# tanderson92/Fast_solver_Lippmann_Schwinger

Measured on AMD Instinct MI355X. Metric: fastconv applies/sec, 3D n=512^3 fp64 (FastM3D apply), higher is better.
Workload: dtype f64; 1 GPU; 3D n=512^3 complex fp64 operator apply y = x + w^2 G*(nu.*x), Greengard-Vico truncated-kernel symbol, omega=1/h=512, sum-of-8-Gaussians contrast, vectors resident in HBM; n=512, pipeline=pruned-hip, parallelism=single GPU

## Files before the change

fast_solver_lippmann_schwinger_amd/_lib.py:

```python
from __future__ import annotations

import ctypes as C
import os

_HERE = os.path.dirname(os.path.abspath(__file__))
LIB_PATH = os.environ.get("LSFC_LIBRARY") or os.path.join(_HERE, "liblsfc.so")

LSFC_QUAD_TRAPEZOIDAL, LSFC_QUAD_GREENGARD_VICO = 0, 1
LSFC_MEM_HOST, LSFC_MEM_DEVICE = 0, 1
LSFC_PRECOND_INV_F64, LSFC_PRECOND_INV_F32 = 0, 1
LSFC_PRECOND_PIVOT_NONE, LSFC_PRECOND_PIVOT_PARTIAL, LSFC_PRECOND_PIVOT_AUTO = 0, 1, 2
LSFC_FLAG_DEFAULT, LSFC_FLAG_LITERAL_PAD, LSFC_FLAG_FORCE_ROCFFT, LSFC_FLAG_PATCH_SINGULAR = 0, 1, 2, 4
LSFC_ORTH_MGS, LSFC_ORTH_CGS, LSFC_ORTH_DGKS = 0, 1, 2
LSFC_EINVAL, LSFC_ENODEV, LSFC_ENOMEM, LSFC_ENOTCONV = -1, -2, -3, -5
LSFC_UNIQUE_ID_BYTES = 128

PRECOND_FN = C.CFUNCTYPE(C.c_int, C.c_void_p, C.POINTER(C.c_double), C.c_int64)


class GmresOpts(C.Structure):
    _fields_ = [("restart", C.c_int), ("maxiter", C.c_int64), ("reltol", C.c_double), ("abstol", C.c_double),
                ("orth", C.c_int), ("initially_zero", C.c_int), ("precond", PRECOND_FN), ("precond_user", C.c_void_p),
                ("precond_on_device", C.c_int)]


class GmresResult(C.Structure):
    _fields_ = [("iters", C.c_int64), ("mvps", C.c_int64), ("converged", C.c_int), ("final_resnorm", C.c_double)]


class BicgstablOpts(C.Structure):
    _fields_ = [("l", C.c_int), ("max_mv_products", C.c_int64), ("reltol", C.c_double), ("abstol", C.c_double),
                ("initially_zero", C.c_int), ("precond", PRECOND_FN), ("precond_user", C.c_void_p),
                ("precond_on_device", C.c_int), ("r_shadow", C.c_void_p), ("reserved", C.c_int * 4)]


class BlocktriOpts(C.Structure):
    _fields_ = [("inverse_precision", C.c_int), ("pivoting", C.c_int), ("reserved", C.c_int * 6)]


class LsfcError(RuntimeError):
    def __init__(self, code, msg):
        super().__init__(f"lsfc error {code}: {msg}")
        self.code = code


_P, _I, _L, _D, _U = C.c_void_p, C.c_int, C.c_int64, C.c_double, C.c_uint
_PP = C.POINTER(C.c_void_p)
SIGNATURES = {
    "lsfc_plan_create_2d": (_I, [_PP, _L, _L, _L, _L, _P, _P, _D, _I, _U, _I]),
    "lsfc_plan_create_3d": (_I, [_PP, _L, _L, _L, _L, _L, _L, _P, _P, _D, _I, _U, _I]),
    "lsfc_plan_create_gv2d": (_I, [_PP, _L, _L, _D, _D, _P, _U, _I]),
    "lsfc_plan_create_trap2d": (_I, [_PP, _L, _L, _D, _D, _D, _D, _D, _D, _P, _U, _I]),
    "lsfc_plan_create_gv3d": (_I, [_PP, _L, _L, _L, _D, _D, _P, _U, _I]),
    "lsfc_plan_destroy": (_I, [_P]),
    "lsfc_plan_size": (_L, [_P]),
    "lsfc_plan_dims": (_I, [_P, C.POINTER(_L), C.POINTER(_L)]),
    "lsfc_plan_pipeline": (C.c_char_p, [_P]),
    "lsfc_plan_set_nu": (_I, [_P, _P, _I]),
    "lsfc_plan_get_symbol": (_I, [_P, _P, _L, C.POINTER(_L)]),
    "lsfc_apply": (_I, [_P, _P, _P, _I]),
    "lsfc_convolve": (_I, [_P, _P, _P, _I, _I]),
    "lsfc_apply_batch": (_I, [_P, _P, _P, _L, _I, _I]),
    "lsfc_sample_sources": (_I, [_P, _P, _L, _P, _I]),
    "lsfc_gmres": (_I, [_P, _P, _P, C.POINTER(GmresOpts), _P, _L, C.POINTER(GmresResult), _I]),
    "lsfc_gmres_batch": (_I, [_P, _P, _P, _L, C.POINTER(GmresOpts), _P, _L, C.POINTER(GmresResult), _I]),
    "lsfc_bicgstabl": (_I, [_P, _P, _P, C.POINTER(BicgstablOpts), _P, _L, C.POINTER(GmresResult), _I]),
    "lsfc_precond_create": (_I, [_PP, _L, _P, _P, _P, _P, _P, _P, _P, _P, _P, _P, _P, _P, _I]),
    "lsfc_precond_destroy": (_I, [_P]),
    "lsfc_precond_set_stream": (_I, [_P, _P]),
    "lsfc_precond_apply": (_I, [_P, _P, _I]),
    "lsfc_precond_apply_batch": (_I, [_P, _P, _L, _I]),
    "lsfc_precond_batch_info": (_I, [_P, C.POINTER(_L)]),
    "lsfc_precond_callback": (_I, [_P, _P, _L]),
    "lsfc_precond_stats": (_I, [_P, C.POINTER(_L), C.POINTER(_L), C.POINTER(_L)]),
    "lsfc_precond_schedule": (_I, [_P, _I, C.POINTER(_L)]),
    "lsfc_precond_create_blocktri": (_I, [_PP, _L, _L, _P, _P, _P, _P, _I, _I]),
    "lsfc_precond_create_from_plan": (_I, [_PP, _P]),
    "lsfc_precond_create_blocktri_prec": (_I, [_PP, _L, _L, _P, _P, _P, _P, _I, _I, _I]),
    "lsfc_precond_create_from_plan_prec": (_I, [_PP, _P, _I]),
    "lsfc_precond_create_blocktri_opts": (_I, [_PP, _L, _L, _P, _P, _P, _P, _I, _I, _P]),
    "lsfc_precond_create_from_plan_opts": (_I, [_PP, _P, _P]),
    "lsfc_precond_blocktri_get_pivots": (_I, [_P, _L, _P, _L]),
    "lsfc_precond_inverse_precision": (_I, [_P, C.POINTER(_I)]),
    "lsfc_precond_blocktri_info": (_I, [_P, C.POINTER(_L), C.POINTER(_D)]),
    "lsfc_precond_blocktri_get_block": (_I, [_P, _L, _P, _L]),
    "lsfc_sparsify_pattern": (_I, [_L, _L, _L, C.POINTER(_L), _P, _P, _P]),
    "lsfc_sparsify_build": (_I, [_P, _P, _P, _P, _P, _P, _P, _I]),
    "lsfc_plan_set_stream": (_I, [_P, _P]),
    "lsfc_plan_synchronize": (_I, [_P]),
    "lsfc_plan_set_tuning": (_I, [_P, C.c_char_p, _I]),
    "lsfc_time_apply": (_I, [_P, _P, _P, _I, C.POINTER(_D)]),
    "lsfc_profile_apply": (_I, [_P, _P, _P, _I, _I, C.POINTER(C.c_char_p), C.POINTER(_D), C.POINTER(_D), C.POINTER(_I)]),
    "lsfc_device_count": (_I, [C.POINTER(_I)]),
    "lsfc_malloc": (_I, [_PP, C.c_size_t, _I]),
    "lsfc_free": (_I, [_P]),
    "lsfc_memcpy_h2d": (_I, [_P, _P, C.c_size_t]),
    "lsfc_memcpy_d2h": (_I, [_P, _P, C.c_size_t]),
    "lsfc_host_register": (_I, [_P, C.c_size_t]),
    "lsfc_host_unregister": (_I, [_P]),
    "lsfc_host_alloc": (_I, [_PP, C.c_size_t]),
    "lsfc_host_free": (_I, [_P]),
    "lsfc_dist_unique_id": (_I, [_P]),
    "lsfc_dist_plan_create_gv3d": (_I, [_PP, _L, _L, _L, _D, _D, _P, _U, _I, _I, _I, _P]),
    "lsfc_dist_sim_plan_create_gv3d": (_I, [_PP, _L, _L, _L, _D, _D, _P, _U, _I, _I, _I]),
    "lsfc_dist_sim_apply": (_I, [_PP, _I, _PP, _PP, _I]),
    "lsfc_plan_create_gv3d_multi": (_I, [_PP, _L, _L, _L, _D, _D, _P, _U, C.POINTER(_I), _I]),
    "lsfc_multi_info": (_I, [_P, C.POINTER(_I), C.POINTER(_I), C.POINTER(_L), C.POINTER(C.c_char_p)]),
    "lsfc_multi_apply_dev": (_I, [_P, _PP, _PP, _I]),
    "lsfc_last_error": (C.c_char_p, []),
    "lsfc_padded_length": (_I, [C.c_int64]),
    "lsfc_version": (C.c_char_p, []),
}

_lib = None


def load():
    global _lib
    if _lib is None:
        if not os.path.exists(LIB_PATH):
            raise ImportError(f"{LIB_PATH} is missing: build it with `make -C {os.path.join(_HERE, 'csrc')}` "
                              "(hipcc --offload-arch=gfx950); there is no CPU fallback for the lsfc operator")
        try:
            import torch
        except ImportError:
            pass
        lib = C.CDLL(LIB_PATH)
        for name, (res, args) in SIGNATURES.items():
            fn = getattr(lib, name)
            fn.restype, fn.argtypes = res, args
        _lib = lib
    return _lib


def check(rc):
    if rc != 0:
        raise LsfcError(rc, load().lsfc_last_error().decode(errors="replace"))
    return rc


def host_register(a):
    check(load().lsfc_host_register(a.ctypes.data_as(C.c_void_p), a.nbytes))


def host_unregister(a):
    check(load().lsfc_host_unregister(a.ctypes.data_as(C.c_void_p)))


class _PinnedBlock:

    def __init__(self, nbytes):
        self.ptr = C.c_void_p()
        check(load().lsfc_host_alloc(C.byref(self.ptr), max(int(nbytes), 1)))
        self.nbytes = int(nbytes)

    def __del__(self):
        try:
            if self.ptr:
                load().lsfc_host_free(self.ptr)
                self.ptr = C.c_void_p()
        except Exception:
            pass


def host_empty(shape, dtype="complex128"):
    import numpy as np
    dt = np.dtype(dtype)
    count = int(np.prod(shape)) if np.ndim(shape) else int(shape)
    blk = _PinnedBlock(count * dt.itemsize)
    buf = (C.c_char * max(blk.nbytes, 1)).from_address(blk.ptr.value)
    buf._owner = blk
    return np.frombuffer(buf, dtype=dt, count=count).reshape(shape)


def device_count():
    n = C.c_int(0)
    load().lsfc_device_count(C.byref(n))
    return n.value
```

fast_solver_lippmann_schwinger_amd/csrc/fft_kernels.hip:

```cpp
#include "common.hpp"
#include "fft_configs.hpp"
#include "pruned.hpp"
#include <cstdlib>
#include <mutex>
#include <set>
#include <map>
#include <utility>

#ifndef LSFC_FAMILY
#error "compile with -DLSFC_FAMILY=2, 3 or 5"
#endif
#define LSFC_CAT2(a, b) a##b
#define LSFC_CAT(a, b) LSFC_CAT2(a, b)
#define FAM(name) LSFC_CAT(LSFC_CAT(name, _f), LSFC_FAMILY)

namespace lsfc {
using namespace fft;

static constexpr int XB = 8;

template <class C, int LPW, bool SPLIT, bool EXACT>
__global__ __launch_bounds__(C::T * LPW)
void k_xfwd(const VecBatch vb, int64_t obatch, const double* __restrict__ nu, cplx* __restrict__ out,
            const cplx* __restrict__ tw, int64_t nlines, int wmagic, int W, int Wp, int n, int64_t bstride) {
    const cplx* __restrict__ x = vb.x[blockIdx.y];
    out += (int64_t)blockIdx.y * obatch;
    using LL = LdsLayout<1, 3, SPLIT>;
    extern __shared__ __attribute__((aligned(16))) char smem[];
    constexpr int T = C::T, E = C::E;
    const int t = threadIdx.x % T, ll = threadIdx.x / T;
    const int64_t line = (int64_t)blockIdx.x * LPW + ll;
    const bool valid = line < nlines;
    const int64_t lc = valid ? line : nlines - 1;
    const cplx* xin = x + lc * n;
    cplx v[E];
#pragma unroll
    for (int e = 0; e < E / 2; ++e) v[e] = (EXACT || t + T * e < n) ? xin[t + T * e] : make_double2(0.0, 0.0);
    if (nu) {
        const double* nin = nu + lc * n;
#pragma unroll
        for (int e = 0; e < E / 2; ++e) { const double s = (EXACT || t + T * e < n) ? nin[t + T * e] : 0.0; v[e].x *= s; v[e].y *= s; }
    }
#pragma unroll
    for (int e = E / 2; e < E; ++e) v[e] = make_double2(0.0, 0.0);
    fft_forward<C, LL, true>(v, t, tw, smem, ll * LL::line_elems(C::L), 0);
    if (valid) {
#pragma unroll
        for (int e = 0; e < E; ++e) {
            const int s = t + T * e;
            const int c = (int)(((unsigned)s * (unsigned)wmagic) >> 22);
            out[(int64_t)c * bstride + line * Wp + (s - c * W)] = v[e];
        }
    }
}

template <class C, int LPW, bool SPLIT, bool EXACT>
__global__ __launch_bounds__(C::T * LPW)
void k_xinv(const cplx* __restrict__ in, const VecBatch vb, int64_t ibatch, double alpha, double beta,
            const cplx* __restrict__ tw, int64_t nlines, int wmagic, int W, int Wp, int n, int64_t bstride) {
    const cplx* xorig = vb.x[blockIdx.y];
    cplx* y = vb.y[blockIdx.y];
    in += (int64_t)blockIdx.y * ibatch;
    using LL = LdsLayout<1, 3, SPLIT>;
    extern __shared__ __attribute__((aligned(16))) char smem[];
    constexpr int T = C::T, E = C::E;
    const int t = threadIdx.x % T, ll = threadIdx.x / T;
    const int64_t line = (int64_t)blockIdx.x * LPW + ll;
    const bool valid = line < nlines;
    const int64_t lc = valid ? line : nlines - 1;
    cplx v[E];
#pragma unroll
    for (int e = 0; e < E; ++e) {
        const int s = t + T * e;
        const int c = (int)(((unsigned)s * (unsigned)wmagic) >> 22);
        v[e] = in[(int64_t)c * bstride + lc * Wp + (s - c * W)];
    }
    fft_inverse<C, LL, true>(v, t, tw, smem, ll * LL::line_elems(C::L), 0);
    if (valid) {
#pragma unroll
        for (int e = 0; e < E / 2; ++e) {
            if (EXACT || t + T * e < n) {
                const int64_t idx = line * n + t + T * e;
                cplx r = make_double2(beta * v[e].x, beta * v[e].y);
                if (alpha != 0.0) { const cplx xo = xorig[idx]; r.x = fma(alpha, xo.x, r.x); r.y = fma(alpha, xo.y, r.y); }
                y[idx] = r;
            }
        }
    }
}

template <class C, int LINES, bool SPLIT, int WPE, bool EXACT>
__global__ __launch_bounds__(C::T * LINES, WPE)
void k_yfwd(const cplx* __restrict__ a1, cplx* __restrict__ a2, const cplx* __restrict__ tw, int Lx, int m, int l, int TG, int TZ, int p1, int p2,
            int64_t batch1, int64_t batch2) {
    using LL = LdsLayout<LINES, 3, SPLIT>;
    a1 += (int64_t)blockIdx.y * batch1; a2 += (int64_t)blockIdx.y * batch2;
    extern __shared__ __attribute__((aligned(16))) char smem[];
    constexpr int T = C::T, E = C::E, Ly = C::L;
    const int xi = threadIdx.x % LINES, t = threadIdx.x / LINES;
    const int ngrp = Lx / LINES;
    const int within = blockIdx.x % (TG * TZ), tile = blockIdx.x / (TG * TZ);
    const int ntg = ngrp / TG;
    const int g = (tile % ntg) * TG + within % TG, z = (tile / ntg) * TZ + within / TG;
    const int xp = g * LINES + xi;
    const cplx* src = a1 + xp + (int64_t)p1 * m * z;
    cplx v[E];
#pragma unroll
    for (int e = 0; e < E / 2; ++e) v[e] = (EXACT || t + T * e < m) ? src[(int64_t)p1 * (t + T * e)] : make_double2(0.0, 0.0);
#pragma unroll
    for (int e = E / 2; e < E; ++e) v[e] = make_double2(0.0, 0.0);
    fft_forward<C, LL, true, false, (C::T * LINES > 512)>(v, t, tw, smem, 0, xi);
    const int xb = xp / XB, xq = xp % XB;
    cplx* dst = a2 + xq + (int64_t)XB * z + (int64_t)p2 * ((int64_t)Ly * xb);
#pragma unroll
    for (int e = 0; e < E; ++e) dst[(int64_t)p2 * (t + T * e)] = v[e];
}

template <class C, int LINES, bool SPLIT, int WPE, bool EXACT>
__global__ __launch_bounds__(C::T * LINES, WPE)
void k_yinv(const cplx* __restrict__ a2, cplx* __restrict__ a1, const cplx* __restrict__ tw, int Lx, int m, int l, int TG, int TZ, int p1, int p2,
            int64_t batch1, int64_t batch2) {
    using LL = LdsLayout<LINES, 3, SPLIT>;
    a1 += (int64_t)blockIdx.y * batch1; a2 += (int64_t)blockIdx.y * batch2;
    extern __shared__ __attribute__((aligned(16))) char smem[];
    constexpr int T = C::T, E = C::E, Ly = C::L;
    const int xi = threadIdx.x % LINES, t = threadIdx.x / LINES;
    const int ngrp = Lx / LINES;
    const int within = blockIdx.x % (TG * TZ), tile = blockIdx.x / (TG * TZ);
    const int ntg = ngrp / TG;
    const int g = (tile % ntg) * TG + within % TG, z = (tile / ntg) * TZ + within / TG;
    const int xp = g * LINES + xi;
    const int xb = xp / XB, xq = xp % XB;
    const cplx* src = a2 + xq + (int64_t)XB * z + (int64_t)p2 * ((int64_t)Ly * xb);
    cplx v[E];
#pragma unroll
    for (int e = 0; e < E; ++e) v[e] = src[(int64_t)p2 * (t + T * e)];
    fft_inverse<C, LL, true, false, (C::T * LINES > 512)>(v, t, tw, smem, 0, xi);
    cplx* dst = a1 + xp + (int64_t)p1 * m * z;
#pragma unroll
    for (int e = 0; e < E / 2; ++e) if (EXACT || t + T * e < m) dst[(int64_t)p1 * (t + T * e)] = v[e];
}

template <class C, int LINES, bool SPLIT, bool PREFETCH, int WPE, bool HALF, bool ZE, bool EXACT, bool TWL, bool MULTI = false>
__global__ __launch_bounds__(C::T * LINES, WPE)
void k_zfused(cplx* __restrict__ data, const cplx* __restrict__ sym, const cplx* __restrict__ tw,
              int nouter, int64_t dGrp, int64_t dOuter, int64_t dLine, int64_t sGrp, int64_t sOuter, int64_t sLine,
              const int2* __restrict__ ytab, const int* __restrict__ zm, int nin, int nrhs, int64_t dBatch, int sibling_pairs) {
    using LL = LdsLayout<LINES, 3, SPLIT>;
    extern __shared__ __attribute__((aligned(16))) char smem[];
    constexpr int T = C::T, E = C::E;
    int xi = threadIdx.x % LINES; const int t = threadIdx.x / LINES;
    unsigned tile = blockIdx.x;
    if constexpr (HALF) {
        constexpr int PARTS = XB / LINES, SH = PARTS == 4 ? 5 : 4;
        const unsigned b = blockIdx.x;
        tile = (b >> SH) * 8 + (b & 7);
        xi += (int)((b >> 3) & (PARTS - 1)) * LINES;
    } else if (sibling_pairs) {
        const unsigned b = blockIdx.x;
        tile = (((b >> 4) * 8 + (b & 7)) << 1) | ((b >> 3) & 1);
    }
    const int o = tile % nouter, g = tile / nouter;
    int outer = o, srow = o;
    if (ytab) { const int2 e = ytab[o]; outer = e.x; srow = e.y; }
    cplx* d = data + g * dGrp + outer * dOuter + xi;
    const cplx* s = sym + g * sGrp + srow * sOuter + xi;
    const int li = threadIdx.x % LINES;
    if constexpr (TWL) {
        cplx* tl = reinterpret_cast<cplx*>(smem + (size_t)LL::line_elems(C::L) * LINES * LL::elem_bytes());
        for (int i = threadIdx.x; i < C::TWLEN; i += C::T * LINES) tl[i] = tw[i];
        __syncthreads();
        tw = tl;
    }
#ifdef LSFC_NO_XLANE_ONE_TILE
    constexpr bool XL1 = false;
#else
    constexpr bool XL1 = !SPLIT && xlane_ok<C, LL>() && (C::T * LINES) % 64 == 0;
#endif
    auto fwd = [&](cplx (&w)[E]) {
        if constexpr (!SPLIT) fft_forward_ws<C, LL, true, TWL, false, XL1>(w, t, tw, smem, 0, li, [] {});
        else fft_forward<C, LL, true, TWL>(w, t, tw, smem, 0, li);
    };
    auto inv = [&](cplx (&w)[E]) {
        if constexpr (!SPLIT) fft_inverse_ws<C, LL, true, TWL, false, XL1>(w, t, tw, smem, 0, li);
        else fft_inverse<C, LL, true, TWL>(w, t, tw, smem, 0, li);
    };
    cplx v[E];
    if constexpr (MULTI) {
        constexpr int H = ZE ? E / 2 : E;
        cplx sv[H];
#pragma unroll
        for (int e = 0; e < H; ++e) sv[e] = s[sLine * (t + T * e)];
        int part[ZE ? H : 1];
        cplx smid = make_double2(0.0, 0.0);
        if constexpr (ZE) {
#pragma unroll
            for (int e = 0; e < H; ++e) part[e] = zm[t + T * e];
            if (t == 0) smid = s[sLine * (C::L / 2)];
        }
        for (int r = 0; r < nrhs; ++r) {
            cplx* dr = d + (int64_t)r * dBatch;
#pragma unroll
            for (int e = 0; e < E / 2; ++e) v[e] = (EXACT || t + T * e < nin) ? dr[dLine * (t + T * e)] : make_double2(0.0, 0.0);
#pragma unroll
            for (int e = E / 2; e < E; ++e) v[e] = make_double2(0.0, 0.0);
            fwd(v);
            if constexpr (ZE) {
                cplx* stage = reinterpret_cast<cplx*>(smem);
                if constexpr (forward_ends_local<C, LL>()) LSFC_BARRIER();
#pragma unroll
                for (int e = 0; e < H; ++e) stage[(t + T * e) * LINES + li] = sv[e];
                if (t == 0) stage[(C::L / 2) * LINES + li] = smid;
                LSFC_BARRIER();
#pragma unroll
                for (int e = 0; e < H; ++e) {
                    v[e] = cmul(v[e], sv[e]);
                    v[e + H] = cmul(v[e + H], stage[part[e] * LINES + li]);
                }
                LSFC_BARRIER();
            } else {
#pragma unroll
                for (int e = 0; e < E; ++e) v[e] = cmul(v[e], sv[e]);
            }
            inv(v);
#pragma unroll
            for (int e = 0; e < E / 2; ++e) if (EXACT || t + T * e < nin) dr[dLine * (t + T * e)] = v[e];
        }
        return;
    }
#pragma unroll
    for (int e = 0; e < E / 2; ++e) v[e] = (EXACT || t + T * e < nin) ? d[dLine * (t + T * e)] : make_double2(0.0, 0.0);
#pragma unroll
    for (int e = E / 2; e < E; ++e) v[e] = make_double2(0.0, 0.0);
    if constexpr (ZE) {
        constexpr int H = E / 2;
        int part[H];
#pragma unroll
        for (int e = 0; e < H; ++e) part[e] = zm[t + T * e];
        cplx sv[H];
        if constexpr (PREFETCH) {
#pragma unroll
            for (int e = 0; e < H; ++e) sv[e] = s[sLine * (t + T * e)];
        }
        fwd(v);
        if constexpr (!PREFETCH) {
#pragma unroll
            for (int e = 0; e < H; ++e) sv[e] = s[sLine * (t + T * e)];
        }
        cplx* stage = reinterpret_cast<cplx*>(smem);
        if constexpr (forward_ends_local<C, LL>()) LSFC_BARRIER();
#pragma unroll
        for (int e = 0; e < H; ++e) stage[(t + T * e) * LINES + li] = sv[e];
        if (t == 0) stage[(C::L / 2) * LINES + li] = s[sLine * (C::L / 2)];
        LSFC_BARRIER();
#pragma unroll
        for (int e = 0; e < H; ++e) {
            v[e] = cmul(v[e], sv[e]);
            v[e + H] = cmul(v[e + H], stage[part[e] * LINES + li]);
        }
        LSFC_BARRIER();
    } else if constexpr (PREFETCH) {
        cplx sv[E];
#pragma unroll
        for (int e = 0; e < E; ++e) sv[e] = s[sLine * (t + T * e)];
        fwd(v);
#pragma unroll
        for (int e = 0; e < E; ++e) v[e] = cmul(v[e], sv[e]);
    } else {
        fwd(v);
#pragma unroll
        for (int e = 0; e < E; ++e) v[e] = cmul(v[e], s[sLine * (t + T * e)]);
    }
    inv(v);
#pragma unroll
    for (int e = 0; e < E / 2; ++e) if (EXACT || t + T * e < nin) d[dLine * (t + T * e)] = v[e];
}

__device__ __forceinline__ unsigned xcc_id() {
    unsigned v;
    asm volatile("s_getreg_b32 %0, hwreg(HW_REG_XCC_ID, 0, 4)" : "=s"(v));
    return v & 7u;
}
template <class V> __device__ __forceinline__ V launder_v(V x) { asm volatile("" : "+v"(x)); return x; }
template <class P> __device__ __forceinline__ P launder_s(P x) { asm volatile("" : "+s"(x)); return x; }

template <class C, int LINES, bool SPLIT, bool HALF> constexpr size_t persist_xbuf_bytes() {
    using LL = LdsLayout<LINES, HALF ? -1 : 3, SPLIT>;
    constexpr size_t ex = (size_t)LL::line_elems(C::L) * LINES * LL::elem_bytes(), stg = (size_t)(C::L / 2 + 1) * LINES * sizeof(cplx);
    return ex > stg ? ex : stg;
}
template <class C, int LINES, bool SPLIT, bool TWL, bool HALF> constexpr size_t persist_lds_bytes() {
    return persist_xbuf_bytes<C, LINES, SPLIT, HALF>() + (TWL ? (size_t)C::TWLEN * sizeof(cplx) : 0);
}
template <class C, int LINES, bool SPLIT, bool EXACT, bool TWL, bool LATE_SYM = false, bool HALF = false, bool TICKETS = HALF, int XL = 0>
__global__ __launch_bounds__(C::T * LINES, (HALF && 2 * persist_lds_bytes<C, LINES, SPLIT, TWL, HALF>() <= (size_t)160 * 1024) ? 2 : 1)
void k_zfused_persist(cplx* __restrict__ data, const cplx* __restrict__ sym, const cplx* __restrict__ tw,
                      int nouter, int64_t dGrp, int64_t dOuter, int64_t dLine, int64_t sGrp, int64_t sOuter, int64_t sLine,
                      const int2* __restrict__ ytab, const int* __restrict__ zm, int nin, unsigned ntiles, unsigned* __restrict__ tickets) {
    using LL = LdsLayout<LINES, HALF ? -1 : 3, SPLIT>;
    extern __shared__ __attribute__((aligned(16))) char smem[];
    constexpr int T = C::T, E = C::E, H = E / 2;
#ifdef LSFC_NO_STAGE_STORES
    constexpr bool WS = false;
#else
    constexpr bool WS = true;
#endif
#ifdef LSFC_DEFERRED_BARRIERS
    constexpr bool DEFER = true;
#else
    constexpr bool DEFER = false;
#endif
    const int li = threadIdx.x % LINES, t = threadIdx.x / LINES;
    constexpr bool PAIR = (XL & 4) != 0 && TICKETS && !HALF;
    constexpr unsigned DONE = 0xFFFFFFFFu;
    unsigned cur = blockIdx.x, nwork = ntiles;
    unsigned* slot = nullptr;
    unsigned queue = 0, queues_left = 8;
    [[maybe_unused]] unsigned parity = 1u;
    auto draw = [&]() -> unsigned {
        while (queues_left > 0) {
            const unsigned c = atomicAdd(tickets + queue, 1u);
            if (c < nwork) return (c << 3) | queue;
            queue = (queue + 1) & 7u; --queues_left;
        }
        return DONE;
    };
    if constexpr (TICKETS) {
        queue = xcc_id();
        nwork = HALF ? ntiles / 4 : (PAIR ? ntiles / 16 : ntiles / 8);
        slot = reinterpret_cast<unsigned*>(smem + persist_lds_bytes<C, LINES, SPLIT, TWL, HALF>());
        if (threadIdx.x == 0) *slot = draw();
        __syncthreads();
        cur = __builtin_amdgcn_readfirstlane(*slot);
        __syncthreads();
        if (cur == DONE) return;
    } else if (cur >= nwork) return;
    if constexpr (TWL) {
        cplx* tl = reinterpret_cast<cplx*>(smem + persist_xbuf_bytes<C, LINES, SPLIT, HALF>());
        for (int i = threadIdx.x; i < C::TWLEN; i += C::T * LINES) tl[i] = tw[i];
        __syncthreads();
        tw = tl;
    }
    auto locate = [&](unsigned w, cplx*& dbase, const cplx*& sbase, unsigned sub = 0) {
        unsigned tl_ = w; int half = 0;
        if constexpr (PAIR) tl_ = ticket_decode_pair(w, sub);
        else if constexpr (TICKETS) { unsigned hf; ticket_decode<HALF>(w, tl_, hf); half = (int)hf * LINES; }
        const int o = (int)(tl_ % (unsigned)nouter), g = (int)(tl_ / (unsigned)nouter);
        int outer = o, srow = o;
        if (ytab) { const int2 e2 = ytab[o]; outer = e2.x; srow = e2.y; }
        dbase = data + g * dGrp + outer * dOuter + half;
        sbase = sym + g * sGrp + srow * sOuter + half;
    };
    const unsigned doff = (unsigned)(li + (int)dLine * t), dstep = (unsigned)((int)dLine * T);
    const unsigned soff = (unsigned)(li + (int)sLine * t), sstep = (unsigned)((int)sLine * T);
    constexpr bool MIRG = (XL & 2) != 0;
    [[maybe_unused]] unsigned moff[MIRG ? H : 1];
    if constexpr (MIRG) {
#pragma unroll
        for (int e = 0; e < H; ++e) moff[e] = (unsigned)(li + (int)sLine * zm[t + T * e]);
    }
    cplx nd[H];
    {
        cplx* d; const cplx* s;
        locate(cur, d, s);
#pragma unroll
        for (int e = 0; e < H; ++e) nd[e] = (EXACT || t + T * e < nin) ? d[doff + dstep * e] : make_double2(0.0, 0.0);
    }
    [[maybe_unused]] unsigned sub = 0;
    [[maybe_unused]] const cplx* sheld = nullptr;
    [[maybe_unused]] cplx sv_pair[PAIR ? H : 1];
    [[maybe_unused]] cplx smid_pair = make_double2(0.0, 0.0);
    for (;;) {
        unsigned drawn = 0;
        if constexpr (TICKETS) { if (threadIdx.x == 0 && (!PAIR || sub == 0)) drawn = draw(); }
        cplx v[E];
#pragma unroll
        for (int e = 0; e < H; ++e) { v[e] = nd[e]; v[e + H] = make_double2(0.0, 0.0); }
        cplx sv_tile[PAIR ? 1 : H];
        cplx (&sv)[H] = *reinterpret_cast<cplx (*)[H]>(PAIR ? &sv_pair[0] : &sv_tile[0]);
        [[maybe_unused]] cplx smr[MIRG ? H : 1];
        cplx smid_tile = make_double2(0.0, 0.0);
        cplx& smid = PAIR ? smid_pair : smid_tile;
        auto load_symbol = [&] {
            cplx* d; const cplx* s;
            locate(cur, d, s, sub);
            if constexpr (PAIR) {
                if (s == sheld) return;
                sheld = s;
            }
            const unsigned so = launder_v(soff);
#pragma unroll
            for (int e = 0; e < H; ++e) sv[e] = s[so + sstep * e];
            if constexpr (MIRG) {
#pragma unroll
                for (int e = 0; e < H; ++e) smr[e] = s[moff[e]];
            } else {
                if (t == 0) smid = s[so - (unsigned)((int)sLine * t) + (unsigned)((int)sLine * (C::L / 2))];
            }
        };
        if constexpr (!SPLIT && WS) {
            if constexpr (!LATE_SYM) load_symbol();
            fft_forward_ws<C, LL, true, TWL, DEFER, (XL > 0)>(v, t, tw, smem, 0, li, [&] { if constexpr (LATE_SYM) load_symbol(); });
        } else if constexpr (LATE_SYM) {
            stage<C, 0, +1, 1, TWL>(v, t, tw);
            load_symbol();
            exchange<C, 0, 1, LL>(v, t, smem, 0, li);
            stage<C, 1, +1, 0, TWL>(v, t, tw);
            if constexpr (C::NS >= 3) { exchange<C, 1, 2, LL>(v, t, smem, 0, li); stage<C, 2, +1, 0, TWL>(v, t, tw); }
            if constexpr (C::NS >= 4) { exchange<C, 2, 3, LL>(v, t, smem, 0, li); stage<C, 3, +1, 0, TWL>(v, t, tw); }
        } else {
            load_symbol();
            fft_forward<C, LL, true, TWL>(v, t, tw, smem, 0, li);
        }
        cplx* stage = reinterpret_cast<cplx*>(smem);
        unsigned next = cur + gridDim.x;
        if constexpr (MIRG) {
#pragma unroll
            for (int e = 0; e < H; ++e) { v[e] = cmul(v[e], sv[e]); v[e + H] = cmul(v[e + H], smr[e]); }
            if constexpr (TICKETS) {
                if (threadIdx.x == 0) slot[parity] = drawn;
                LSFC_BARRIER();
                next = __builtin_amdgcn_readfirstlane(slot[parity]);
                parity ^= 1u;
            }
        } else {
        if constexpr (forward_ends_local<C, LL>() || (!SPLIT && WS && DEFER)) LSFC_BARRIER();
#pragma unroll
        for (int e = 0; e < H; ++e) stage[(t + T * e) * LINES + li] = sv[e];
        if (t == 0) stage[(C::L / 2) * LINES + li] = smid;
        if constexpr (TICKETS) { if (threadIdx.x == 0 && (!PAIR || sub == 0)) *slot = drawn; }
        LSFC_BARRIER();
        {
            const int* zmt = launder_s(zm) + t;
#pragma unroll
            for (int e = 0; e < H; ++e) {
                v[e] = cmul(v[e], sv[e]);
                v[e + H] = cmul(v[e + H], stage[zmt[T * e] * LINES + li]);
            }
        }
        if constexpr (TICKETS) next = __builtin_amdgcn_readfirstlane(*slot);
        LSFC_BARRIER();
        }
        const bool more = PAIR ? (sub == 0 || next != DONE) : (TICKETS ? next != DONE : next < nwork);
        if (more) {
            cplx* dn; const cplx* sn;
            if (PAIR && sub == 0) locate(cur, dn, sn, 1u); else locate(next, dn, sn, 0u);
            const unsigned dof = launder_v(doff);
#pragma unroll
            for (int e = 0; e < H; ++e) nd[e] = (EXACT || t + T * e < nin) ? dn[dof + dstep * e] : make_double2(0.0, 0.0);
        }
        if constexpr (!SPLIT && WS) fft_inverse_ws<C, LL, true, TWL, DEFER, (XL > 0)>(v, t, tw, smem, 0, li);
        else fft_inverse<C, LL, true, TWL>(v, t, tw, smem, 0, li);
        {
            cplx* d; const cplx* s;
            locate(cur, d, s, sub);
            const unsigned dof = launder_v(doff);
#pragma unroll
            for (int e = 0; e < H; ++e) if (EXACT || t + T * e < nin) d[dof + dstep * e] = v[e];
        }
        if (!more) break;
        if constexpr (PAIR) { if (sub == 0) sub = 1; else { sub = 0; cur = next; } }
        else cur = next;
    }
}

template <class K> static void allow_lds(K kernel, size_t bytes) {
    if (bytes <= 48 * 1024) return;
    static std::mutex mu;
    static std::set<std::pair<const void*, int>> done;
    int dev = 0; LSFC_HIP(hipGetDevice(&dev));
    const std::pair<const void*, int> key(reinterpret_cast<const void*>(kernel), dev);
    std::lock_guard<std::mutex> lock(mu);
    if (done.count(key)) return;
    LSFC_HIP(hipFuncSetAttribute(key.first, hipFuncAttributeMaxDynamicSharedMemorySize, (int)bytes));
    done.insert(key);
}

static bool env_flag_no_sibling_pairs() { static const bool v = getenv("LSFC_NO_SIBLING_PAIRS") != nullptr; return v; }
static bool env_flag_z_quarter() { static const bool v = [] { const char* e = getenv("LSFC_Z_QUARTER"); return e && e[0] == '1'; }(); return v; }

template <class C> struct Tune {
    static constexpr int LPW = (256 / C::T) > 0 ? (256 / C::T) : 1;
    static constexpr int LINES = (C::T * XB <= 512 || (C::E <= 8 && C::T * XB <= 1024)) ? XB : 512 / C::T;
#ifdef LSFC_Y2048_HALF
    static constexpr int YLINES = LINES;
#else
    static constexpr int YLINES = (C::L == 2048 && C::T * XB <= 1024) ? XB : LINES;
#endif
};

template <class C, bool SPLIT> static void xfwd_t(const VecBatch& vb, int nrhs, int64_t obatch, const double* nu, cplx* out, const cplx* tw, int64_t nlines, int wmagic, int W, int Wp, int n, int64_t bstride, hipStream_t st) {
    constexpr int LPW = Tune<C>::LPW;
    using LL = LdsLayout<1, 3, SPLIT>;
    const size_t lds = (size_t)LL::line_elems(C::L) * LPW * LL::elem_bytes();
    auto k = (n == C::L / 2) ? k_xfwd<C, LPW, SPLIT, true> : k_xfwd<C, LPW, SPLIT, false>;
    allow_lds(k, lds);
    hipLaunchKernelGGL(k, dim3((unsigned)((nlines + LPW - 1) / LPW), (unsigned)nrhs), dim3(C::T * LPW), lds, st, vb, obatch, nu, out, tw, nlines, wmagic, W, Wp, n, bstride);
}
template <class C, bool SPLIT> static void xinv_t(const cplx* in, const VecBatch& vb, int nrhs, int64_t ibatch, double alpha, double beta, const cplx* tw, int64_t nlines, int wmagic, int W, int Wp, int n, int64_t bstride, hipStream_t st) {
    constexpr int LPW = Tune<C>::LPW;
    using LL = LdsLayout<1, 3, SPLIT>;
    const size_t lds = (size_t)LL::line_elems(C::L) * LPW * LL::elem_bytes();
    auto k = (n == C::L / 2) ? k_xinv<C, LPW, SPLIT, true> : k_xinv<C, LPW, SPLIT, false>;
    allow_lds(k, lds);
    hipLaunchKernelGGL(k, dim3((unsigned)((nlines + LPW - 1) / LPW), (unsigned)nrhs), dim3(C::T * LPW), lds, st, in, vb, ibatch, alpha, beta, tw, nlines, wmagic, W, Wp, n, bstride);
}
static void ytile(const PrunedTuning& tn, int L, int ngrp, int l, int& TG, int& TZ) {
    const int ag = (L >= 1024) ? 32 : ngrp, az = (L >= 1024) ? 8 : 1;
    TG = tn.ytile_g > 0 ? tn.ytile_g : ag; if (TG > ngrp) TG = ngrp; while (ngrp % TG) --TG;
    TZ = tn.ytile_z > 0 ? tn.ytile_z : az; if (TZ > l) TZ = l;       while (l % TZ) --TZ;
}
template <class C, bool SPLIT, int WPE> static void yfwd_t(const PrunedTuning& tn, const cplx* a1, cplx* a2, const cplx* tw, int Lx, int m, int l, int p1, int p2, hipStream_t st, int nrhs, int64_t b1, int64_t b2) {
    constexpr int LINES = Tune<C>::YLINES;
    using LL = LdsLayout<LINES, 3, SPLIT>;
    const size_t lds = (size_t)LL::line_elems(C::L) * LINES * LL::elem_bytes();
    auto k = (m == C::L / 2) ? k_yfwd<C, LINES, SPLIT, WPE, true> : k_yfwd<C, LINES, SPLIT, WPE, false>;
    allow_lds(k, lds);
    int TG, TZ; ytile(tn, C::L, Lx / LINES, l, TG, TZ);
    hipLaunchKernelGGL(k, dim3((unsigned)((Lx / LINES) * l), (unsigned)nrhs), dim3(C::T * LINES), lds, st, a1, a2, tw, Lx, m, l, TG, TZ, p1, p2, b1, b2);
}
template <class C, bool SPLIT, int WPE> static void yinv_t(const PrunedTuning& tn, const cplx* a2, cplx* a1, const cplx* tw, int Lx, int m, int l, int p1, int p2, hipStream_t st, int nrhs, int64_t b1, int64_t b2) {
    constexpr int LINES = Tune<C>::YLINES;
    using LL = LdsLayout<LINES, 3, SPLIT>;
    const size_t lds = (size_t)LL::line_elems(C::L) * LINES * LL::elem_bytes();
    auto k = (m == C::L / 2) ? k_yinv<C, LINES, SPLIT, WPE, true> : k_yinv<C, LINES, SPLIT, WPE, false>;
    allow_lds(k, lds);
    int TG, TZ; ytile(tn, C::L, Lx / LINES, l, TG, TZ);
    hipLaunchKernelGGL(k, dim3((unsigned)((Lx / LINES) * l), (unsigned)nrhs), dim3(C::T * LINES), lds, st, a2, a1, tw, Lx, m, l, TG, TZ, p1, p2, b1, b2);
}
template <class C, bool SPLIT, bool PREFETCH, int WPE, bool ZE = false> static void zfused_t(cplx* data, const cplx* sym, const cplx* tw, const cplx* twl,
                                                    const FusedGeom& g, hipStream_t st, int nrhs, int64_t dBatch) {
    constexpr int LINES = Tune<C>::LINES;
    static_assert(XB % LINES == 0, "LINES must divide XB");
    using LL = LdsLayout<LINES, 3, SPLIT>;
    size_t lds = (size_t)LL::line_elems(C::L) * LINES * LL::elem_bytes();
    auto k = (g.nin == C::L / 2) ? k_zfused<C, LINES, SPLIT, PREFETCH, WPE, false, ZE, true, false> : k_zfused<C, LINES, SPLIT, PREFETCH, WPE, false, ZE, false, false>;
    if (twl && lds + (size_t)C::TWLEN * sizeof(cplx) > (size_t)160 * 1024) twl = nullptr;
    if (twl) {
        k = (g.nin == C::L / 2) ? k_zfused<C, LINES, SPLIT, PREFETCH, WPE, false, ZE, true, true> : k_zfused<C, LINES, SPLIT, PREFETCH, WPE, false, ZE, false, true>;
        lds += (size_t)C::TWLEN * sizeof(cplx);
        tw = twl;
    }
    if (nrhs > 1) {
        if (twl) k = (g.nin == C::L / 2) ? k_zfused<C, LINES, SPLIT, false, WPE, false, ZE, true, true, true> : k_zfused<C, LINES, SPLIT, false, WPE, false, ZE, false, true, true>;
        else     k = (g.nin == C::L / 2) ? k_zfused<C, LINES, SPLIT, false, WPE, false, ZE, true, false, true> : k_zfused<C, LINES, SPLIT, false, WPE, false, ZE, false, false, true>;
    }
    allow_lds(k, lds);
    if (LINES == XB) {
        hipLaunchKernelGGL(k, dim3((unsigned)((g.Lx / XB) * g.nouter)), dim3(C::T * LINES), lds, st, data, sym, tw, g.nouter,
                           g.dTile, g.dOuter, g.dLine, g.sTile, g.sOuter, g.sLine, g.ytab, g.zm, g.nin, nrhs, dBatch,
                           0);
    } else {
        LSFC_REQUIRE(g.dTile == XB && g.sTile == XB, "sub-tile groups need the natural (2D) layout");
        hipLaunchKernelGGL(k, dim3((unsigned)((g.Lx / LINES) * g.nouter)), dim3(C::T * LINES), lds, st, data, sym, tw, g.nouter,
                           (int64_t)LINES, g.dOuter, g.dLine, (int64_t)LINES, g.sOuter, g.sLine, g.ytab, g.zm, g.nin, nrhs, dBatch,
                           (XB / LINES == 2 && g.nouter == 1 && (g.Lx / LINES) % 16 == 0 && !env_flag_no_sibling_pairs()) ? 1 : 0);
    }
}

static int cu_count() {
    static int cus = 0;
    if (!cus) { int dev = 0; LSFC_HIP(hipGetDevice(&dev)); hipDeviceProp_t pr; LSFC_HIP(hipGetDeviceProperties(&pr, dev)); cus = pr.multiProcessorCount > 0 ? pr.multiProcessorCount : 256; }
    return cus;
}
static unsigned* ticket_set(hipStream_t st);
template <class C, bool SPLIT, bool LATE_SYM = false, bool TICKETS = false> static void zfused_persist_t(cplx* data, const cplx* sym, const cplx* tw, const cplx* twl,
                                                            const FusedGeom& g, hipStream_t st, int xl = 0) {
    constexpr int LINES = XB;
    using LL = LdsLayout<LINES, 3, SPLIT>;
    size_t lds = persist_xbuf_bytes<C, LINES, SPLIT, false>();
    if (twl && lds + (size_t)C::TWLEN * sizeof(cplx) > (size_t)160 * 1024) twl = nullptr;
    auto k = (g.nin == C::L / 2) ? k_zfused_persist<C, LINES, SPLIT, true, false, LATE_SYM, false, TICKETS> : k_zfused_persist<C, LINES, SPLIT, false, false, LATE_SYM, false, TICKETS>;
    if (twl) {
        k = (g.nin == C::L / 2) ? k_zfused_persist<C, LINES, SPLIT, true, true, LATE_SYM, false, TICKETS> : k_zfused_persist<C, LINES, SPLIT, false, true, LATE_SYM, false, TICKETS>;
        lds += (size_t)C::TWLEN * sizeof(cplx);
        tw = twl;
    }
    if constexpr (xlane_ok<C, LL>() && !SPLIT && LATE_SYM) {
        if (xl == 1) {
            if (twl) k = (g.nin == C::L / 2) ? k_zfused_persist<C, LINES, SPLIT, true, true, LATE_SYM, false, TICKETS, 1> : k_zfused_persist<C, LINES, SPLIT, false, true, LATE_SYM, false, TICKETS, 1>;
            else     k = (g.nin == C::L / 2) ? k_zfused_persist<C, LINES, SPLIT, true, false, LATE_SYM, false, TICKETS, 1> : k_zfused_persist<C, LINES, SPLIT, false, false, LATE_SYM, false, TICKETS, 1>;
        } else if (xl >= 2 && twl) {
            if (xl == 5 && TICKETS) k = (g.nin == C::L / 2) ? k_zfused_persist<C, LINES, SPLIT, true, true, LATE_SYM, false, TICKETS, 5> : k_zfused_persist<C, LINES, SPLIT, false, true, LATE_SYM, false, TICKETS, 5>;
            else if (xl == 3) k = (g.nin == C::L / 2) ? k_zfused_persist<C, LINES, SPLIT, true, true, LATE_SYM, false, TICKETS, 3> : k_zfused_persist<C, LINES, SPLIT, false, true, LATE_SYM, false, TICKETS, 3>;
            else k = (g.nin == C::L / 2) ? k_zfused_persist<C, LINES, SPLIT, true, true, LATE_SYM, false, TICKETS, 1> : k_zfused_persist<C, LINES, SPLIT, false, true, LATE_SYM, false, TICKETS, 1>;
        }
    }
    if (TICKETS) lds += 16;
    allow_lds(k, lds);
    const int cus = cu_count();
    const unsigned ntiles = (unsigned)((g.Lx / XB) * g.nouter);
    const int per_cu = (int)std::max<size_t>(1, std::min<size_t>(4, ((size_t)160 * 1024) / lds));
    const unsigned grid = std::min<unsigned>(ntiles, (unsigned)(cus * per_cu));
    hipLaunchKernelGGL(k, dim3(grid), dim3(C::T * LINES), lds, st, data, sym, tw, g.nouter,
                       g.dTile, g.dOuter, g.dLine, g.sTile, g.sOuter, g.sLine, g.ytab, g.zm, g.nin, ntiles, TICKETS ? ticket_set(st) : (unsigned*)nullptr);
}
static unsigned* ticket_set(hipStream_t st) {
    static std::mutex mu;
    static std::map<int, std::pair<unsigned*, unsigned>> ring;
    int dev = 0; LSFC_HIP(hipGetDevice(&dev));
    unsigned* base; unsigned idx;
    {
        std::lock_guard<std::mutex> lock(mu);
        auto it = ring.find(dev);
        if (it == ring.end()) {
            unsigned* p = nullptr;
            LSFC_HIP(hipMalloc(&p, 64 * 8 * sizeof(unsigned)));
            it = ring.emplace(dev, std::make_pair(p, 0u)).first;
        }
        base = it->second.first; idx = it->second.second++ % 64u;
    }
    unsigned* set = base + 8 * idx;
    LSFC_HIP(hipMemsetAsync(set, 0, 8 * sizeof(unsigned), st));
    return set;
}
template <class C> static void zfused_persist_half_t(cplx* data, const cplx* sym, const cplx* twl, const FusedGeom& g, hipStream_t st, int xl = 0) {
    if constexpr (C::L >= 1024) {
        constexpr int LINES = XB / 2;
        constexpr size_t lds = persist_lds_bytes<C, LINES, false, true, true>() + 16;
        static_assert(lds <= (size_t)160 * 1024, "half-tile persistent pass: exchange buffer exceeds the LDS");
        auto k = (g.nin == C::L / 2) ? k_zfused_persist<C, LINES, false, true, true, true, true> : k_zfused_persist<C, LINES, false, false, true, true, true>;
        if constexpr (xlane_ok<C, LdsLayout<LINES, -1, false>>()) {
            if (xl) k = (g.nin == C::L / 2) ? k_zfused_persist<C, LINES, false, true, true, true, true, true, 1> : k_zfused_persist<C, LINES, false, false, true, true, true, true, 1>;
        }
        LSFC_REQUIRE(twl != nullptr, "half-tile persistent pass: twiddle table missing");
        allow_lds(k, lds);
        const unsigned ntiles = (unsigned)((g.Lx / XB) * g.nouter);
        LSFC_REQUIRE(ntiles % 16 == 0 && (g.nouter % 2 == 0 || !g.ytab), "ticketed half-tile z pass needs a multiple of 16 tiles in row pairs");
        const int per_cu = (int)std::max<size_t>(1, std::min<size_t>(2, ((size_t)160 * 1024) / lds));
        const unsigned grid = std::min<unsigned>(2 * ntiles, (unsigned)(cu_count() * per_cu));
        unsigned* tickets = ticket_set(st);
        hipLaunchKernelGGL(k, dim3(grid), dim3(C::T * LINES), lds, st, data, sym, twl, g.nouter,
                           g.dTile, g.dOuter, g.dLine, g.sTile, g.sOuter, g.sLine, g.ytab, g.zm, g.nin, ntiles, tickets);
    } else {
        fail(LSFC_EINVAL, "half-tile persistent pass: lines of %d points run as whole tiles", (int)C::L);
    }
}

template <class C, bool SPLIT, bool PREFETCH, int WPE, bool ZE = false, int LINES = 4> static void zfused_half_t(cplx* data, const cplx* sym, const cplx* tw,
                                                         const FusedGeom& g, hipStream_t st) {
    using LL = LdsLayout<LINES, 3, SPLIT>;
    const size_t lds = (size_t)LL::line_elems(C::L) * LINES * LL::elem_bytes();
    auto k = (g.nin == C::L / 2) ? k_zfused<C, LINES, SPLIT, PREFETCH, WPE, true, ZE, true, false> : k_zfused<C, LINES, SPLIT, PREFETCH, WPE, true, ZE, false, false>;
    allow_lds(k, lds);
    const int64_t ntiles = (int64_t)(g.Lx / XB) * g.nouter;
    LSFC_REQUIRE(ntiles % 8 == 0, "half-tile z pass needs a multiple of 8 tiles");
    hipLaunchKernelGGL(k, dim3((unsigned)((XB / LINES) * ntiles)), dim3(C::T * LINES), lds, st, data, sym, tw, g.nouter,
                       g.dTile, g.dOuter, g.dLine, g.sTile, g.sOuter, g.sLine, g.ytab, g.zm, g.nin, 1, (int64_t)0, 0);
}

#if LSFC_FAMILY == 2
#define LSFC_DISPATCH_L(L, CALL)                                           \
    switch (L) {                                                           \
    case 32:   { using C = Cfg32;   CALL; } break;                         \
    case 64:   { using C = Cfg64;   CALL; } break;                         \
    case 128:  { using C = Cfg128;  CALL; } break;                         \
    case 256:  { using C = Cfg256;  CALL; } break;                         \
    case 512:  { using C = Cfg512;  CALL; } break;                         \
    case 1024: { using C = Cfg1024; CALL; } break;                         \
    case 2048: { using C = Cfg2048; CALL; } break;                         \
    default: fail(LSFC_EINVAL, "pruned pipeline: unsupported padded length %d", (int)(L)); }
#elif LSFC_FAMILY == 3
#define LSFC_DISPATCH_L(L, CALL)                                           \
    switch (L) {                                                           \
    case 48:   { using C = Cfg48;   CALL; } break;                         \
    case 96:   { using C = Cfg96;   CALL; } break;                         \
    case 192:  { using C = Cfg192;  CALL; } break;                         \
    case 384:  { using C = Cfg384;  CALL; } break;                         \
    case 768:  { using C = Cfg768;  CALL; } break;                         \
    case 1536: { using C = Cfg1536; CALL; } break;                         \
    default: fail(LSFC_EINVAL, "pruned pipeline: unsupported padded length %d", (int)(L)); }
#else
#define LSFC_DISPATCH_L(L, CALL)                                           \
    switch (L) {                                                           \
    case 80:   { using C = Cfg80;   CALL; } break;                         \
    case 160:  { using C = Cfg160;  CALL; } break;                         \
    case 320:  { using C = Cfg320;  CALL; } break;                         \
    case 640:  { using C = Cfg640;  CALL; } break;                         \
    case 1280: { using C = Cfg1280; CALL; } break;                         \
    default: fail(LSFC_EINVAL, "pruned pipeline: unsupported padded length %d", (int)(L)); }
#endif

__global__ void FAM(k_warmup)(int* p) { if (p) *p = 0; }
void FAM(pruned_warmup)() {
    hipLaunchKernelGGL(FAM(k_warmup), dim3(1), dim3(64), 0, 0, (int*)nullptr);
    LSFC_HIP(hipGetLastError());
}

void FAM(pruned_perm)(int L, int* freq_of_storage) {
    LSFC_DISPATCH_L(L, perm_table<C>(freq_of_storage));
}

static int chunk_magic(int L, int W) {
    LSFC_REQUIRE(W >= 8 && W <= L && L % W == 0 && L <= 2048, "chunk width %d does not divide the line length %d", W, L);
    return (1 << 22) / W + 1;
}
void FAM(pruned_xfwd)(int L, const PrunedTuning& tn, const VecBatch& vb, int nrhs, int64_t obatch, const double* nu, cplx* out, const cplx* tw, int64_t nlines, int W, int Wp, int n, hipStream_t st, int64_t bstride) {
    const int wmagic = chunk_magic(L, W);
    if (bstride <= 0) bstride = (int64_t)Wp * nlines;
    if (tn.split_x) { LSFC_DISPATCH_L(L, (xfwd_t<C, true>(vb, nrhs, obatch, nu, out, tw, nlines, wmagic, W, Wp, n, bstride, st))); }
    else            { LSFC_DISPATCH_L(L, (xfwd_t<C, false>(vb, nrhs, obatch, nu, out, tw, nlines, wmagic, W, Wp, n, bstride, st))); }
    LSFC_HIP(hipGetLastError());
}
void FAM(pruned_xinv)(int L, const PrunedTuning& tn, const cplx* in, const VecBatch& vb, int nrhs, int64_t ibatch, double alpha, double beta, const cplx* tw, int64_t nlines, int W, int Wp, int n, hipStream_t st, int64_t bstride) {
    const int wmagic = chunk_magic(L, W);
    if (bstride <= 0) bstride = (int64_t)Wp * nlines;
    if (tn.split_x) { LSFC_DISPATCH_L(L, (xinv_t<C, true>(in, vb, nrhs, ibatch, alpha, beta, tw, nlines, wmagic, W, Wp, n, bstride, st))); }
    else            { LSFC_DISPATCH_L(L, (xinv_t<C, false>(in, vb, nrhs, ibatch, alpha, beta, tw, nlines, wmagic, W, Wp, n, bstride, st))); }
    LSFC_HIP(hipGetLastError());
}
void FAM(pruned_yfwd)(int L, const PrunedTuning& tn, const cplx* a1, cplx* a2, const cplx* tw, int Lx, int m, int l, int p1, int p2, hipStream_t st, int nrhs, int64_t b1, int64_t b2) {
    size_t full_lds = 0;
    LSFC_DISPATCH_L(L, (full_lds = (size_t)LdsLayout<Tune<C>::YLINES, 3, false>::line_elems(C::L) * Tune<C>::YLINES * 16));
    if (tn.split_s || full_lds > (size_t)160 * 1024) { LSFC_DISPATCH_L(L, (yfwd_t<C, true, 1>(tn, a1, a2, tw, Lx, m, l, p1, p2, st, nrhs, b1, b2))); }
    else            { LSFC_DISPATCH_L(L, (yfwd_t<C, false, 1>(tn, a1, a2, tw, Lx, m, l, p1, p2, st, nrhs, b1, b2))); }
    LSFC_HIP(hipGetLastError());
}
void FAM(pruned_yinv)(int L, const PrunedTuning& tn, const cplx* a2, cplx* a1, const cplx* tw, int Lx, int m, int l, int p1, int p2, hipStream_t st, int nrhs, int64_t b1, int64_t b2) {
    size_t full_lds = 0;
    LSFC_DISPATCH_L(L, (full_lds = (size_t)LdsLayout<Tune<C>::YLINES, 3, false>::line_elems(C::L) * Tune<C>::YLINES * 16));
    if (tn.split_s || full_lds > (size_t)160 * 1024) { LSFC_DISPATCH_L(L, (yinv_t<C, true, 1>(tn, a2, a1, tw, Lx, m, l, p1, p2, st, nrhs, b1, b2))); }
    else            { LSFC_DISPATCH_L(L, (yinv_t<C, false, 1>(tn, a2, a1, tw, Lx, m, l, p1, p2, st, nrhs, b1, b2))); }
    LSFC_HIP(hipGetLastError());
}
int FAM(pruned_twfull_len)(int L) {
    int len = 0;
    LSFC_DISPATCH_L(L, len = C::TWLEN);
    return len;
}
void FAM(pruned_twfull)(int L, const cplx* tw, cplx* out) {
    LSFC_DISPATCH_L(L, twfull_table<C>(out, tw));
}

void FAM(pruned_zfused)(int L, const PrunedTuning& tn, cplx* data, const cplx* sym, const cplx* tw, const cplx* twl, const FusedGeom& g, hipStream_t st,
                        int nrhs, int64_t dBatch) {
    const bool tiled = g.dLine == 8 && ((int64_t)(g.Lx / XB) * g.nouter) % 8 == 0;
    const bool half_form = (LSFC_FAMILY == 2 && ((L == 1024 && (tn.z_half >= 0 ? tn.z_half : (g.zm ? 0 : 2)) > 0 && tiled) || (L == 2048 && g.dLine == 8)))
                        || (LSFC_FAMILY == 3 && L == 1536 && (tn.z_half >= 0 ? tn.z_half : 1) > 0 && tiled);
    {
        const int zp = tn.z_persist >= 0 ? tn.z_persist : ((L == 1536 || L == 1280 || L == 2048) ? 5 : (L >= 1024 ? 6 : 3));
        bool eight_lines = false;
        LSFC_DISPATCH_L(L, (eight_lines = Tune<C>::LINES == XB));
        const bool enough_tiles = tn.z_persist > 0 || (int64_t)(g.Lx / XB) * g.nouter >= (int64_t)4096;
        const bool half5 = zp == 5 && tiled && twl && L >= 1024 && ((int64_t)(g.Lx / XB) * g.nouter) % 16 == 0 && (g.nouter % 2 == 0 || !g.ytab);
        if (zp > 0 && g.zm && g.dLine == 8 && nrhs == 1 && (eight_lines || half5) && (!half_form || half5) && enough_tiles) {
            size_t full_lds = 0;
            LSFC_DISPATCH_L(L, (full_lds = (size_t)LdsLayout<XB, 3, false>::line_elems(C::L) * XB * 16));
            const bool split = zp == 2 || zp == 4 || full_lds > (size_t)160 * 1024;
            if (half5) {
                LSFC_DISPATCH_L(L, (zfused_persist_half_t<C>(data, sym, twl, g, st, tn.xlane != 0 ? 1 : 0)));
                LSFC_HIP(hipGetLastError());
                return;
            }
            if (zp == 6 && !split && ((int64_t)(g.Lx / XB) * g.nouter) % 16 == 0 && g.nouter % 2 == 0) {
                LSFC_DISPATCH_L(L, (zfused_persist_t<C, false, true, true>(data, sym, tw, tn.tw_lds ? twl : nullptr, g, st, tn.xlane < 0 ? 5 : tn.xlane)));
                LSFC_HIP(hipGetLastError());
                return;
            }
            if ((zp == 3 || zp == 6) && !split) { LSFC_DISPATCH_L(L, (zfused_persist_t<C, false, true>(data, sym, tw, tn.tw_lds ? twl : nullptr, g, st, tn.xlane < 0 ? 1 : tn.xlane))); }
            else if (zp >= 3) { LSFC_DISPATCH_L(L, (zfused_persist_t<C, true, true>(data, sym, tw, tn.tw_lds ? twl : nullptr, g, st))); }
            else if (split) { LSFC_DISPATCH_L(L, (zfused_persist_t<C, true>(data, sym, tw, tn.tw_lds ? twl : nullptr, g, st))); }
            else       { LSFC_DISPATCH_L(L, (zfused_persist_t<C, false>(data, sym, tw, tn.tw_lds ? twl : nullptr, g, st))); }
            LSFC_HIP(hipGetLastError());
            return;
        }
    }
    if (nrhs > 1 && half_form) {
        for (int r = 0; r < nrhs; ++r)
            FAM(pruned_zfused)(L, tn, data + (int64_t)r * dBatch, sym, tw, twl, g, st, 1, 0);
        return;
    }
#define LSFC_ZF(SP, PF) do { if (g.zm) { LSFC_DISPATCH_L(L, (zfused_t<C, SP, PF, 1, true>(data, sym, tw, tn.tw_lds ? twl : nullptr, g, st, nrhs, dBatch))); } \
                             else    { LSFC_DISPATCH_L(L, (zfused_t<C, SP, PF, 1, false>(data, sym, tw, tn.tw_lds ? twl : nullptr, g, st, nrhs, dBatch))); } } while (0)
#if LSFC_FAMILY == 2
    const int zh = tn.z_half >= 0 ? tn.z_half : (g.zm ? 0 : 2);
    if (L == 1024 && zh > 0 && g.dLine == 8 && ((int64_t)(g.Lx / XB) * g.nouter) % 8 == 0) {
        using C = Cfg1024;
#define LSFC_ZH(SP, PF, W) do { if (g.zm) zfused_half_t<C, SP, PF, W, true>(data, sym, tw, g, st); \
                                else zfused_half_t<C, SP, PF, W, false>(data, sym, tw, g, st); } while (0)
        switch (zh) {
        case 1: LSFC_ZH(false, true, 2); break;
        case 2: LSFC_ZH(true, true, 2); break;
        case 3: LSFC_ZH(true, false, 3); break;
        default: LSFC_ZH(false, false, 2); break;
        }
#undef LSFC_ZH
        LSFC_HIP(hipGetLastError());
        return;
    }
    if (L == 2048 && g.dLine == 8) {
        LSFC_REQUIRE(((int64_t)(g.Lx / XB) * g.nouter) % 8 == 0, "half-tile z pass needs a multiple of 8 tiles");
        using C = Cfg2048;
        const bool quarter = g.zm && env_flag_z_quarter();
        if (quarter) zfused_half_t<C, false, false, 2, true, 2>(data, sym, tw, g, st);
        else if (g.zm) zfused_half_t<C, false, false, 2, true>(data, sym, tw, g, st);
        else zfused_half_t<C, false, false, 2, false>(data, sym, tw, g, st);
        LSFC_HIP(hipGetLastError());
        return;
    }
#elif LSFC_FAMILY == 3
    const int zh = tn.z_half >= 0 ? tn.z_half : 1;
    if (L == 1536 && zh > 0 && g.dLine == 8 && ((int64_t)(g.Lx / XB) * g.nouter) % 8 == 0) {
        using C = Cfg1536;
#define LSFC_ZH(SP, PF) do { if (g.zm) zfused_half_t<C, SP, PF, 1, true>(data, sym, tw, g, st); \
                             else zfused_half_t<C, SP, PF, 1, false>(data, sym, tw, g, st); } while (0)
        switch (zh) {
        case 1: LSFC_ZH(false, true); break;
        case 2: LSFC_ZH(true, true); break;
        case 3: LSFC_ZH(true, false); break;
        default: LSFC_ZH(false, false); break;
        }
#undef LSFC_ZH
        LSFC_HIP(hipGetLastError());
        return;
    }
#endif
#if LSFC_FAMILY == 2
    const bool e16 = L == 1024, full = L >= 1024;
#elif LSFC_FAMILY == 3
    const bool e16 = L >= 384 && L < 1536, full = L >= 384;
#else
    const bool e16 = L >= 320, full = false;
#endif
    bool sp = tn.split_z >= 0 ? tn.split_z != 0 : !full;
    const bool pf = tn.sym_prefetch >= 0 ? tn.sym_prefetch != 0 : e16;
    size_t full_lds = 0;
    LSFC_DISPATCH_L(L, (full_lds = (size_t)LdsLayout<Tune<C>::LINES, 3, false>::line_elems(C::L) * Tune<C>::LINES * 16));
    if (full_lds > (size_t)160 * 1024) sp = true;
    if (sp) { if (pf) { LSFC_ZF(true, true); } else { LSFC_ZF(true, false); } }
    else    { if (pf) { LSFC_ZF(false, true); } else { LSFC_ZF(false, false); } }
#undef LSFC_ZF
    LSFC_HIP(hipGetLastError());
}

}
```

fast_solver_lippmann_schwinger_amd/csrc/plan.hip:

```cpp
#include "plan.hpp"
#include "pointwise.hpp"
#include <cmath>
#include <cstring>
#include <condition_variable>
#include <deque>
#include <thread>
#include <functional>
#include <mutex>

namespace lsfc {

static thread_local char g_last_error[1024] = "";
void set_last_error(const char* fmt, ...) {
    va_list ap; va_start(ap, fmt); vsnprintf(g_last_error, sizeof g_last_error, fmt, ap); va_end(ap);
}

#define LSFC_ROCFFT(expr) do { rocfft_status s_ = (expr); if (s_ != rocfft_status_success) \
    ::lsfc::fail(LSFC_EHIP, "%s failed with rocfft_status %d (%s:%d)", #expr, (int)s_, __FILE__, __LINE__); } while (0)

void rocfft_global_setup() {
    static std::once_flag once;
    std::call_once(once, [] { rocfft_setup(); });
}

RocFft::~RocFft() { release(); }
void RocFft::release() {
    if (info) { rocfft_execution_info_destroy(info); info = nullptr; }
    if (plan) { rocfft_plan_destroy(plan); plan = nullptr; }
    work.release();
}
void RocFft::finish_create() {
    size_t wsz = 0;
    LSFC_ROCFFT(rocfft_plan_get_work_buffer_size(plan, &wsz));
    LSFC_ROCFFT(rocfft_execution_info_create(&info));
    if (wsz) { work.alloc(wsz); LSFC_ROCFFT(rocfft_execution_info_set_work_buffer(info, work.p, wsz)); }
}
void RocFft::create(int ndim, const size_t* lengths, bool forward, size_t batch, bool lazy_work) {
    rocfft_global_setup();
    size_t len[3]; int nd = 0;
    for (int d = 0; d < ndim; ++d) if (lengths[d] > 1) len[nd++] = lengths[d];
    if (nd == 0) { len[0] = 1; nd = 1; }
    LSFC_ROCFFT(rocfft_plan_create(&plan, rocfft_placement_inplace,
                                   forward ? rocfft_transform_type_complex_forward : rocfft_transform_type_complex_inverse,
                                   rocfft_precision_double, nd, len, batch, nullptr));
    if (!lazy_work) finish_create();
}
void RocFft::create_strided_1d(size_t length, size_t stride, size_t dist, size_t batch, bool forward, bool lazy_work) {
    rocfft_global_setup();
    rocfft_plan_description desc = nullptr;
    LSFC_ROCFFT(rocfft_plan_description_create(&desc));
    const size_t strides[1] = { stride };
    rocfft_status s = rocfft_plan_description_set_data_layout(desc, rocfft_array_type_complex_interleaved, rocfft_array_type_complex_interleaved,
                                                              nullptr, nullptr, 1, strides, dist, 1, strides, dist);
    if (s == rocfft_status_success)
        s = rocfft_plan_create(&plan, rocfft_placement_inplace,
                               forward ? rocfft_transform_type_complex_forward : rocfft_transform_type_complex_inverse,
                               rocfft_precision_double, 1, &length, batch, desc);
    rocfft_plan_description_destroy(desc);
    LSFC_ROCFFT(s);
    if (!lazy_work) finish_create();
}
void RocFft::exec(void* buf, hipStream_t stream) {
    if (!info) finish_create();
    LSFC_ROCFFT(rocfft_execution_info_set_stream(info, stream));
    void* in[1] = { buf };
    LSFC_ROCFFT(rocfft_execute(plan, in, nullptr, info));
}

static int env_switch(const char* name) { const char* e = getenv(name); return e ? (unsigned char)e[0] : -1; }
static bool sym_even_y_enabled() { return env_switch("LSFC_SYM_EVEN_Y") != '0'; }
static bool sym_even_z_enabled() { return env_switch("LSFC_SYM_EVEN_Z") != '0'; }

static void select_device(int device) {
    int count = 0;
    hipError_t e = hipGetDeviceCount(&count);
    if (e != hipSuccess || count <= 0) fail(LSFC_ENODEV, "no HIP device available (%s): the lsfc operator has no CPU fallback",
                                            e == hipSuccess ? "device count is 0" : hipGetErrorString(e));
    LSFC_REQUIRE(device >= 0 && device < count, "device %d out of range (have %d)", device, count);
    LSFC_HIP(hipSetDevice(device));
}

void plan_common_init(lsfc_plan* p, int ndim, int64_t n, int64_t m, int64_t l, const double* nu_host, double omega,
                      int quad_rule, unsigned flags, int device) {
    LSFC_REQUIRE(n >= 1 && m >= 1 && l >= 1 && n <= 8192 && m <= 8192 && l <= 8192, "grid size out of range");
    LSFC_REQUIRE(quad_rule == LSFC_QUAD_TRAPEZOIDAL || quad_rule == LSFC_QUAD_GREENGARD_VICO,
                 "unknown quadRule %d (the reference leaves B undefined, src/FastConvolution.jl:106)", quad_rule);
    LSFC_REQUIRE(nu_host != nullptr, "nu is NULL");
    select_device(device);
    pruned_warmup(device);
    p->device = device; p->ndim = ndim;
    p->dims[0] = (int)n; p->dims[1] = (int)m; p->dims[2] = (int)l;
    p->N = n * m * l; p->omega = omega; p->quad_rule = quad_rule; p->flags = flags;
    p->nu.alloc((size_t)p->N);
    LSFC_HIP(hipMemcpy(p->nu.p, nu_host, p->N * sizeof(double), hipMemcpyHostToDevice));
    p->tuning = pruned_default_tuning();
}

void plan_make_twiddles(lsfc_plan* p, int axis, int L) {
    std::vector<cplx> tw((size_t)L);
    for (int j = 0; j < L; ++j) {
        const long double a = -2.0L * 3.14159265358979323846264338327950288L * (long double)j / (long double)L;
        tw[j] = make_double2((double)cosl(a), (double)sinl(a));
    }
    p->tw[axis].alloc((size_t)L);
    LSFC_HIP(hipMemcpy(p->tw[axis].p, tw.data(), (size_t)L * sizeof(cplx), hipMemcpyHostToDevice));
    std::vector<cplx> full((size_t)pruned_twfull_len(L) + 1);
    pruned_twfull(L, tw.data(), full.data());
    p->twl[axis].alloc(full.size());
    LSFC_HIP(hipMemcpy(p->twl[axis].p, full.data(), full.size() * sizeof(cplx), hipMemcpyHostToDevice));
}

static bool pruned_eligible(const lsfc_plan* p) {
    if (p->flags & (LSFC_FLAG_FORCE_ROCFFT | LSFC_FLAG_LITERAL_PAD)) return false;
    double ratio = 1.0;
    for (int d = 0; d < p->ndim; ++d) {
        const int L = pruned_best_length(p->dims[d]);
        if (L == 0) return false;
        if (p->ndim == 3 && L > 4 * p->dims[d]) return false;
        ratio *= (double)L / (2.0 * (double)p->dims[d]);
    }
    return ratio <= 4.0;
}

static void plan_choose_reduced_grid(lsfc_plan* p) {
    const bool pr = pruned_eligible(p);
    for (int d = 0; d < 3; ++d) {
        p->crop[d] = 0;
        if (d >= p->ndim) p->pads[d] = 1;
        else p->pads[d] = pr ? pruned_best_length(p->dims[d]) : 2 * p->dims[d];
    }
    p->pipeline = pr ? lsfc_plan::PRUNED : lsfc_plan::ROCFFT_REDUCED;
}

static void setup_rocfft_pipeline(lsfc_plan* p) {
    const size_t len[3] = { (size_t)p->pads[0], (size_t)p->pads[1], (size_t)p->pads[2] };
    p->fwd.reset(new RocFft()); p->fwd->create(3, len, true);
    p->inv.reset(new RocFft()); p->inv->create(3, len, false);
    p->W.alloc(len[0] * len[1] * len[2]);
}

static void plan_finish_literal(lsfc_plan* p, const cplx* Gd, bool centred) {
    const int64_t total = (int64_t)p->pads[0] * p->pads[1] * p->pads[2];
    p->sym.alloc((size_t)total);
    int shift[3];
    for (int d = 0; d < 3; ++d) shift[d] = centred ? p->pads[d] / 2 : 0;
    pw_roll_scale(Gd, p->sym.p, p->pads, shift, 1.0 / (double)total, p->stream);
    p->pipeline = lsfc_plan::ROCFFT_LITERAL;
    setup_rocfft_pipeline(p);
    LSFC_HIP(hipStreamSynchronize(p->stream));
}

static bool mirror_slots(const std::vector<int>& perm, std::vector<int>* zm) {
    const int L = (int)perm.size();
    for (int s = 0; s < L; ++s) if ((perm[(size_t)s] < L / 2) != (s < L / 2)) return false;
    if (!zm) return true;
    std::vector<int> inv((size_t)L);
    for (int s = 0; s < L; ++s) inv[(size_t)perm[(size_t)s]] = s;
    zm->resize((size_t)L / 2);
    for (int s = L / 2; s < L; ++s) {
        const int km = (L - perm[(size_t)s]) % L;
        (*zm)[(size_t)(s - L / 2)] = (km == L / 2) ? L / 2 : inv[(size_t)km];
    }
    return true;
}
static void upload_mirror_slots(lsfc_plan* p, const std::vector<int>& zm) {
    p->zmirror.alloc(zm.size());
    LSFC_HIP(hipMemcpy(p->zmirror.p, zm.data(), zm.size() * sizeof(int), hipMemcpyHostToDevice));
}

void plan_setup_symbol_rows(lsfc_plan* p, const cplx* G2, const std::vector<int>& perm_y, const std::vector<int>& perm_z, DevBuf<int>& pyrow) {
    const int Ly = p->pads[1], Lz = p->pads[2];
    bool even = false;
    if (sym_even_y_enabled() && p->ndim == 3 && Ly >= 4) even = !G2 || pw_mirror_deviation(G2, p->pads, 1, p->stream) < 1e-13;
    std::vector<int> inv((size_t)Ly), rowky;
    for (int s = 0; s < Ly; ++s) inv[perm_y[s]] = s;
    std::vector<int2> tab;
    if (even) {
        std::vector<int> rowof((size_t)Ly, -1);
        for (int s = 0; s < Ly; ++s) if (perm_y[s] <= Ly / 2) { rowof[s] = (int)rowky.size(); rowky.push_back(perm_y[s]); }
        for (int s = 0; s < Ly; ++s)
            if (rowof[s] >= 0 && inv[(Ly - perm_y[s]) % Ly] == s) tab.push_back(make_int2(s, rowof[s]));
        for (int s = 0; s < Ly; ++s) {
            if (rowof[s] < 0) continue;
            const int mirror = inv[(Ly - perm_y[s]) % Ly];
            if (mirror == s) continue;
            tab.push_back(make_int2(s, rowof[s]));
            tab.push_back(make_int2(mirror, rowof[s]));
        }
    } else {
        for (int s = 0; s < Ly; ++s) { rowky.push_back(perm_y[s]); tab.push_back(make_int2(s, s)); }
    }
    LSFC_REQUIRE((int)tab.size() == Ly, "internal: row table has %d entries for %d rows", (int)tab.size(), Ly);
    p->sym_rows = (int)rowky.size();
    p->ytab.alloc(tab.size());
    LSFC_HIP(hipMemcpy(p->ytab.p, tab.data(), tab.size() * sizeof(int2), hipMemcpyHostToDevice));
    pyrow.alloc(rowky.size());
    LSFC_HIP(hipMemcpy(pyrow.p, rowky.data(), rowky.size() * sizeof(int), hipMemcpyHostToDevice));

    std::vector<int> zm;
    bool zeven = false;
    if (sym_even_z_enabled() && p->ndim == 3 && Lz >= 32 && mirror_slots(perm_z, &zm))
        zeven = !G2 || pw_mirror_deviation(G2, p->pads, 2, p->stream) < 1e-13;
    if (zeven) {
        p->sym_hz = Lz / 2 + 8;
        upload_mirror_slots(p, zm);
    } else {
        p->sym_hz = Lz;
        p->zmirror.release();
    }
}

bool plan_quarter_symbol_ok(const lsfc_plan* p) {
    if (p->ndim != 3) return false;
    if (!sym_even_y_enabled() || !sym_even_z_enabled() || env_switch("LSFC_SYMBOL_FULL") == '1') return false;
    const int Ly = p->pads[1], Lz = p->pads[2];
    if (Ly < 4 || Lz < 32 || p->pads[0] % 2 || Ly % 2 || Lz % 2) return false;
    std::vector<int> pz((size_t)Lz);
    pruned_perm(Lz, pz.data());
    return mirror_slots(pz, nullptr);
}

static void plan_finish_symbol(lsfc_plan* p, DevBuf<cplx>& G2, bool quarter) {
    const int64_t total = (int64_t)p->pads[0] * p->pads[1] * p->pads[2];
    const int64_t have = quarter ? (int64_t)p->pads[0] * (p->pads[1] / 2 + 1) * (p->pads[2] / 2 + 1) : total;
    LSFC_REQUIRE((int64_t)G2.n == have, "internal: reduced symbol has %lld entries, expected %lld", (long long)G2.n, (long long)have);
    LSFC_REQUIRE(!quarter || (p->pipeline == lsfc_plan::PRUNED && p->ndim == 3), "internal: quarter symbol outside the 3D pruned pipeline");
    const double scale = 1.0 / (double)total;
    if (p->pipeline == lsfc_plan::PRUNED) {
        std::vector<int> perm[3];
        DevBuf<int> dperm[3], pyrow, zero, drow;
        for (int d = 0; d < p->ndim; ++d) {
            perm[d].resize((size_t)p->pads[d]);
            pruned_perm(p->pads[d], perm[d].data());
            dperm[d].alloc(perm[d].size());
            LSFC_HIP(hipMemcpy(dperm[d].p, perm[d].data(), perm[d].size() * sizeof(int), hipMemcpyHostToDevice));
            plan_make_twiddles(p, d, p->pads[d]);
        }
        if (p->ndim == 3) {
            plan_setup_symbol_rows(p, quarter ? nullptr : G2.p, perm[1], perm[2], pyrow);
            LSFC_REQUIRE(!quarter || (p->sym_rows == p->pads[1] / 2 + 1 && p->sym_hz == p->pads[2] / 2 + 8), "internal: quarter symbol but full storage");
            p->sym.alloc((size_t)p->pads[0] * p->sym_rows * p->sym_hz);
            pw_permute_symbol(G2.p, p->sym.p, dperm[0].p, pyrow.p, dperm[2].p, p->pads, p->sym_rows, p->sym_hz, 0, p->pads[0] / 8, scale, p->stream,
                              quarter ? p->pads[1] / 2 + 1 : 0);
        } else {
            const int Ly = p->pads[1];
            std::vector<int> zm;
            bool even = false;
            if (sym_even_z_enabled() && Ly >= 32 && mirror_slots(perm[1], &zm)) even = pw_mirror_deviation(G2.p, p->pads, 1, p->stream) < 1e-13;
            if (even) {
                upload_mirror_slots(p, zm);
                const int t2 = env_switch("LSFC_2D_TILED");
                const bool tiled = t2 >= 0 ? t2 == '1' : Ly >= 2048;
                if (tiled && p->pads[0] % 8 == 0 && (p->pads[0] / 8) % 8 == 0 && p->pads[0] <= 2048) {
                    p->sym_hz = Ly / 2 + 8; p->sym_rows = 1;
                    zero.alloc(1);
                    LSFC_HIP(hipMemset(zero.p, 0, sizeof(int)));
                    const int L3[3] = { p->pads[0], 1, Ly };
                    p->sym.alloc((size_t)p->pads[0] * p->sym_hz);
                    pw_permute_symbol(G2.p, p->sym.p, dperm[0].p, zero.p, dperm[1].p, L3, 1, p->sym_hz, 0, p->pads[0] / 8, scale, p->stream);
                    p->tile2d = (int64_t)8 * p->dims[1] + (Ly >= 1024 ? 72 : 0);
                } else {
                    std::vector<int> rowk(perm[1].begin(), perm[1].begin() + Ly / 2);
                    rowk.push_back(Ly / 2);
                    drow.alloc(rowk.size());
                    LSFC_HIP(hipMemcpy(drow.p, rowk.data(), rowk.size() * sizeof(int), hipMemcpyHostToDevice));
                    p->sym.alloc((size_t)p->pads[0] * rowk.size());
                    pw_permute_symbol(G2.p, p->sym.p, dperm[0].p, drow.p, dperm[2].p, p->pads, (int)rowk.size(), 1, 0, p->pads[0] / 8, scale, p->stream);
                }
            } else {
                p->zmirror.release();
                p->sym.alloc((size_t)total);
                pw_permute_symbol(G2.p, p->sym.p, dperm[0].p, dperm[1].p, dperm[2].p, p->pads, p->pads[1], 1, 0, p->pads[0] / 8, scale, p->stream);
            }
        }
        LSFC_HIP(hipStreamSynchronize(p->stream));
        G2.release();
        const bool big = p->ndim == 3 && p->pads[1] >= 1024;
        const int pad1 = p->tuning.pad1 >= 0 ? p->tuning.pad1 : (big ? 40 : 0);
        const int pad2 = p->tuning.pad2 >= 0 ? p->tuning.pad2 : (big ? 72 : 0);
        p->pitch1 = p->pads[0] + ((p->ndim == 3) ? pad1 / 8 * 8 : 0);
        p->pitch2 = 8 * p->dims[2] + pad2 / 8 * 8;
        p->a1_elems = (int64_t)p->pitch1 * p->dims[1] * p->dims[2];
        if (p->tile2d) p->a1_elems = std::max<int64_t>(p->a1_elems, p->tile2d * (p->pads[0] / 8));
        p->a2_elems = (p->ndim == 3) ? (int64_t)p->pitch2 * p->pads[1] * (p->pads[0] / 8) : 0;
        p->A1.alloc((size_t)p->a1_elems);
        if (p->ndim == 3) p->A2.alloc((size_t)p->a2_elems);
        p->batch_cap = 1;
    } else {
        pw_scale(G2.p, scale, total, p->stream);
        LSFC_HIP(hipStreamSynchronize(p->stream));
        p->sym = std::move(G2);
        setup_rocfft_pipeline(p);
    }
}

static void plan_finish_reduce(lsfc_plan* p, DevBuf<cplx>& Gd, const int lit[3], bool centred, const int kernel_origin[3]) {
    plan_choose_reduced_grid(p);
    const int* q = p->pads;
    for (int d = 0; d < p->ndim; ++d)
        LSFC_REQUIRE(lit[d] >= 2 * p->dims[d] - 1, "padded size %d along axis %d is smaller than 2n-1=%d", lit[d], d, 2 * p->dims[d] - 1);
    const int64_t ltotal = (int64_t)lit[0] * lit[1] * lit[2];
    const int64_t qtotal = (int64_t)q[0] * q[1] * q[2];
    {
        DevBuf<cplx> tmp; tmp.alloc((size_t)ltotal);
        int shift[3]; for (int d = 0; d < 3; ++d) shift[d] = centred ? lit[d] / 2 : 0;
        pw_roll_scale(Gd.p, tmp.p, lit, shift, 1.0, p->stream);
        LSFC_HIP(hipStreamSynchronize(p->stream));
        Gd.release();
        const size_t len[3] = { (size_t)lit[0], (size_t)lit[1], (size_t)lit[2] };
        RocFft inv; inv.create(3, len, false);
        inv.exec(tmp.p, p->stream);
        Gd.alloc((size_t)qtotal);
        int nmax[3]; for (int d = 0; d < 3; ++d) nmax[d] = (d < p->ndim) ? p->dims[d] - 1 : 0;
        pw_resample_kernel(tmp.p, Gd.p, lit, q, kernel_origin, nmax, 1.0 / (double)ltotal, p->stream);
        LSFC_HIP(hipStreamSynchronize(p->stream));
    }
    {
        const size_t len[3] = { (size_t)q[0], (size_t)q[1], (size_t)q[2] };
        RocFft fwd; fwd.create(3, len, true);
        fwd.exec(Gd.p, p->stream);
        LSFC_HIP(hipStreamSynchronize(p->stream));
    }
    plan_finish_symbol(p, Gd, false);
}

struct Slab { int z0, nz; };
static Slab whole_grid(const lsfc_plan* p) { return Slab{0, p->dims[2]}; }
static VecBatch slab_vectors(const lsfc_plan* p, const VecBatch& vb, int nrhs, Slab s) {
    const int64_t off = (int64_t)s.z0 * p->dims[0] * p->dims[1];
    VecBatch v = vb;
    for (int j = 0; j < nrhs; ++j) { v.x[j] += off; v.y[j] += off; }
    return v;
}
static cplx* slab_a1(const lsfc_plan* p, Slab s) { return p->A1.p + (int64_t)s.z0 * p->dims[1] * p->pitch1; }
static cplx* slab_a2(const lsfc_plan* p, Slab s) { return p->A2.p + (int64_t)8 * s.z0; }

static void pass_xfwd(lsfc_plan* p, const VecBatch& vb, int nrhs, const double* nu, Slab s, hipStream_t st) {
    const int Lx = p->pads[0], n = p->dims[0];
    const int64_t nlines = (int64_t)p->dims[1] * s.nz;
    const VecBatch v = slab_vectors(p, vb, nrhs, s);
    if (nu) nu += (int64_t)s.z0 * n * p->dims[1];
    if (p->tile2d) pruned_xfwd(Lx, p->tuning, v, nrhs, p->a1_elems, nu, p->A1.p, p->tw[0].p, nlines, 8, 8, n, st, p->tile2d);
    else pruned_xfwd(Lx, p->tuning, v, nrhs, p->a1_elems, nu, slab_a1(p, s), p->tw[0].p, nlines, Lx, p->pitch1, n, st);
}
static void pass_yfwd(lsfc_plan* p, int nrhs, Slab s, hipStream_t st) {
    pruned_yfwd(p->pads[1], p->tuning, slab_a1(p, s), slab_a2(p, s), p->tw[1].p, p->pads[0], p->dims[1], s.nz, p->pitch1, p->pitch2, st,
                nrhs, p->a1_elems, p->a2_elems);
}
static void pass_yinv(lsfc_plan* p, int nrhs, Slab s, hipStream_t st) {
    pruned_yinv(p->pads[1], p->tuning, slab_a2(p, s), slab_a1(p, s), p->tw[1].p, p->pads[0], p->dims[1], s.nz, p->pitch1, p->pitch2, st,
                nrhs, p->a1_elems, p->a2_elems);
}
static void pass_xinv(lsfc_plan* p, const VecBatch& vb, int nrhs, double alpha, double beta, Slab s, hipStream_t st) {
    const int Lx = p->pads[0], n = p->dims[0];
    const int64_t nlines = (int64_t)p->dims[1] * s.nz;
    const VecBatch v = slab_vectors(p, vb, nrhs, s);
    if (p->tile2d) pruned_xinv(Lx, p->tuning, p->A1.p, v, nrhs, p->a1_elems, alpha, beta, p->tw[0].p, nlines, 8, 8, n, st, p->tile2d);
    else pruned_xinv(Lx, p->tuning, slab_a1(p, s), v, nrhs, p->a1_elems, alpha, beta, p->tw[0].p, nlines, Lx, p->pitch1, n, st);
}

void plan_zfused_3d(lsfc_plan* p, int Wc, int64_t a2_off, int64_t sym_off, int nrhs, hipStream_t st) {
    const int Ly = p->pads[1];
    const FusedGeom g{Wc, Ly, (int64_t)p->pitch2 * Ly, (int64_t)p->pitch2, 8, (int64_t)8 * p->sym_hz * p->sym_rows, (int64_t)8 * p->sym_hz, 8,
                      p->ytab.p, p->zmirror.p, p->dims[2]};
    pruned_zfused(p->pads[2], p->tuning, p->A2.p + a2_off, p->sym.p + sym_off, p->tw[2].p, p->twl[2].p, g, st, nrhs, p->a2_elems);
}
static FusedGeom geom_2d_rows(const lsfc_plan* p) {
    return FusedGeom{p->pads[0], 1, 8, 0, (int64_t)p->pitch1, 8, 0, (int64_t)p->pads[0], nullptr, p->zmirror.p, p->dims[1]};
}
static FusedGeom geom_2d_tiles(const lsfc_plan* p) {
    return FusedGeom{p->pads[0], 1, p->tile2d, 0, 8, (int64_t)8 * p->sym_hz, 0, 8, nullptr, p->zmirror.p, p->dims[1]};
}
static void pass_fused(lsfc_plan* p, int nrhs, hipStream_t st) {
    if (p->ndim == 3) { plan_zfused_3d(p, p->pads[0], 0, 0, nrhs, st); return; }
    pruned_zfused(p->pads[1], p->tuning, p->A1.p, p->sym.p, p->tw[1].p, p->twl[1].p, p->tile2d ? geom_2d_tiles(p) : geom_2d_rows(p), st, nrhs, p->a1_elems);
}

static void pruned_convolve(lsfc_plan* p, int nrhs, const VecBatch& vb, bool use_nu, double alpha, double beta) {
    hipStream_t st = p->stream;
    const Slab all = whole_grid(p);
    pass_xfwd(p, vb, nrhs, use_nu ? p->nu.p : nullptr, all, st);
    if (p->ndim == 3) pass_yfwd(p, nrhs, all, st);
    pass_fused(p, nrhs, st);
    if (p->ndim == 3) pass_yinv(p, nrhs, all, st);
    pass_xinv(p, vb, nrhs, alpha, beta, all, st);
}

void plan_convolve_dev(lsfc_plan* p, const cplx* x, cplx* y, bool use_nu, double alpha, double beta) {
    if (p->dist) { dist_convolve_dev(p, x, y, use_nu, alpha, beta); return; }
    if (p->pipeline == lsfc_plan::PRUNED) {
        VecBatch vb{}; vb.x[0] = x; vb.y[0] = y;
        pruned_convolve(p, 1, vb, use_nu, alpha, beta);
    } else {
        const double* nu = use_nu ? p->nu.p : nullptr;
        hipStream_t st = p->stream;
        const int64_t total = (int64_t)p->pads[0] * p->pads[1] * p->pads[2];
        pw_embed(x, nu, p->W.p, p->dims, p->pads, st);
        p->fwd->exec(p->W.p, st);
        pw_mul_inplace(p->W.p, p->sym.p, total, st);
        p->inv->exec(p->W.p, st);
        pw_crop_axpy(p->W.p, x, y, alpha, beta, p->dims, p->pads, p->crop, st);
    }
}

void plan_convolve_batch_dev(lsfc_plan* p, int nrhs, const VecBatch& vb, bool use_nu, double alpha, double beta) {
    LSFC_REQUIRE(nrhs >= 1 && nrhs <= LSFC_MAX_BATCH, "batch of %d right-hand sides (1..%d per pass)", nrhs, LSFC_MAX_BATCH);
    const bool fuse = p->tuning.batch_fuse > 0 ||
                      (p->tuning.batch_fuse < 0 && (int64_t)p->pads[0] * p->pads[1] * p->pads[2] <= ((int64_t)1 << 24));
    if (nrhs == 1 || p->dist || p->multi || p->pipeline != lsfc_plan::PRUNED || !fuse) {
        for (int j = 0; j < nrhs; ++j) plan_convolve_dev(p, vb.x[j], vb.y[j], use_nu, alpha, beta);
        return;
    }
    if (nrhs > p->batch_cap) {
        LSFC_HIP(hipStreamSynchronize(p->stream));
        p->A1.alloc((size_t)(p->a1_elems * nrhs));
        if (p->ndim == 3) p->A2.alloc((size_t)(p->a2_elems * nrhs));
        p->batch_cap = nrhs;
    }
    pruned_convolve(p, nrhs, vb, use_nu, alpha, beta);
}

static void ensure_staging(lsfc_plan* p, int64_t count) {
    if (p->xs.n < (size_t)count) { p->xs.alloc((size_t)count); p->ys.alloc((size_t)count); }
}

HostPipe::~HostPipe() {
    for (hipEvent_t e : ev_up) (void)hipEventDestroy(e);
    for (hipEvent_t e : ev_down) (void)hipEventDestroy(e);
    if (ev_free) (void)hipEventDestroy(ev_free);
    for (hipEvent_t e : { ev_xfree[0], ev_xfree[1], ev_yfree[0], ev_yfree[1] }) if (e) (void)hipEventDestroy(e);
    if (up) (void)hipStreamDestroy(up);
    if (down) (void)hipStreamDestroy(down);
}

static int host_pipeline_chunks(const lsfc_plan* p) {
    const char* e = getenv("LSFC_HOST_PIPELINE");
    const int forced = e ? atoi(e) : -1;
    if (forced == 0 || forced == 1) return 1;
    if (p->pipeline != lsfc_plan::PRUNED || p->ndim != 3 || p->dist || p->multi) return 1;
    if (forced < 0 && p->N * (int64_t)sizeof(cplx) < ((int64_t)64 << 20)) return 1;
    const int l = p->dims[2];
    for (int K = forced > 1 ? forced : 8; K >= 2; --K) if (l % K == 0) return K;
    return 1;
}

static void host_pipelined_convolve(lsfc_plan* p, const cplx* x, cplx* y, int64_t nrhs, bool use_nu, double alpha, double beta, int K) {
    if (!p->hostpipe) {
        std::unique_ptr<HostPipe> hp(new HostPipe());
        LSFC_HIP(hipStreamCreateWithFlags(&hp->up, hipStreamNonBlocking));
        LSFC_HIP(hipStreamCreateWithFlags(&hp->down, hipStreamNonBlocking));
        LSFC_HIP(hipEventCreateWithFlags(&hp->ev_free, hipEventDisableTiming));
        for (hipEvent_t* e : { &hp->ev_xfree[0], &hp->ev_xfree[1], &hp->ev_yfree[0], &hp->ev_yfree[1] }) LSFC_HIP(hipEventCreateWithFlags(e, hipEventDisableTiming));
        p->hostpipe = std::move(hp);
    }
    HostPipe* hp = p->hostpipe.get();
    while ((int)hp->ev_up.size() < 2 * K) {
        hipEvent_t a, b;
        LSFC_HIP(hipEventCreateWithFlags(&a, hipEventDisableTiming)); hp->ev_up.push_back(a);
        LSFC_HIP(hipEventCreateWithFlags(&b, hipEventDisableTiming)); hp->ev_down.push_back(b);
    }
    const int slots = nrhs > 1 ? 2 : 1;
    if (p->xs.n < (size_t)(slots * p->N)) { LSFC_HIP(hipStreamSynchronize(p->stream)); p->xs.alloc((size_t)(slots * p->N)); p->ys.alloc((size_t)(slots * p->N)); }
    const double* nu = use_nu ? p->nu.p : nullptr;
    hipStream_t st = p->stream;
    const int lz = p->dims[2] / K;
    const int64_t chunk = (int64_t)p->dims[0] * p->dims[1] * lz;
    LSFC_HIP(hipEventRecord(hp->ev_free, st));
    LSFC_HIP(hipStreamWaitEvent(hp->up, hp->ev_free, 0));
    struct Down { hipEvent_t ev; cplx* dst; const cplx* src; int slot; bool last; int64_t rhs; };
    std::mutex dmu; std::condition_variable dcv; std::deque<Down> dq; bool ddone = false; std::exception_ptr derr;
    int64_t yfree_recorded[2] = { 0, 0 };
    std::thread dthread;
    const bool helper = nrhs > 1;
    if (helper) dthread = std::thread([&] {
        try {
            LSFC_HIP(hipSetDevice(p->device));
            for (;;) {
                Down d;
                { std::unique_lock<std::mutex> lk(dmu); dcv.wait(lk, [&] { return !dq.empty() || ddone; }); if (dq.empty()) return; d = dq.front(); dq.pop_front(); }
                LSFC_HIP(hipStreamWaitEvent(hp->down, d.ev, 0));
                LSFC_HIP(hipMemcpyAsync(d.dst, d.src, (size_t)chunk * sizeof(cplx), hipMemcpyDeviceToHost, hp->down));
                if (d.last) {
                    LSFC_HIP(hipEventRecord(hp->ev_yfree[d.slot], hp->down));
                    { std::lock_guard<std::mutex> lk(dmu); yfree_recorded[d.slot] = d.rhs + 1; }
                    dcv.notify_all();
                }
            }
        } catch (...) { { std::lock_guard<std::mutex> lk(dmu); derr = std::current_exception(); } dcv.notify_all(); }
    });
    struct Join { std::thread& t; std::mutex& mu; std::condition_variable& cv; bool& done;
                  ~Join() { if (t.joinable()) { { std::lock_guard<std::mutex> lk(mu); done = true; } cv.notify_all(); t.join(); } } } join{dthread, dmu, dcv, ddone};
    for (int64_t j = 0; j < nrhs; ++j) {
        const int sl = (int)(j % slots);
        const cplx* xj = x + j * p->N; cplx* yj = y + j * p->N;
        cplx* xs = p->xs.p + (int64_t)sl * p->N; cplx* ys = p->ys.p + (int64_t)sl * p->N;
        VecBatch sv{}; sv.x[0] = xs; sv.y[0] = ys;
        if (j >= slots) {
            LSFC_HIP(hipStreamWaitEvent(hp->up, hp->ev_xfree[sl], 0));
            if (helper) {
                std::unique_lock<std::mutex> lk(dmu);
                dcv.wait(lk, [&] { return yfree_recorded[sl] >= j - slots + 1 || derr; });
                if (derr) std::rethrow_exception(derr);
            }
            LSFC_HIP(hipStreamWaitEvent(st, hp->ev_yfree[sl], 0));
        }
        for (int c = 0; c < K; ++c) {
            const int64_t off = c * chunk;
            hipEvent_t ev = hp->ev_up[(size_t)(sl * K + c)];
            LSFC_HIP(hipMemcpyAsync(xs + off, xj + off, (size_t)chunk * sizeof(cplx), hipMemcpyHostToDevice, hp->up));
            LSFC_HIP(hipEventRecord(ev, hp->up));
            LSFC_HIP(hipStreamWaitEvent(st, ev, 0));
            pass_xfwd(p, sv, 1, nu, Slab{c * lz, lz}, st);
            pass_yfwd(p, 1, Slab{c * lz, lz}, st);
        }
        pass_fused(p, 1, st);
        for (int c = 0; c < K; ++c) {
            const int64_t off = c * chunk;
            hipEvent_t ev = hp->ev_down[(size_t)(sl * K + c)];
            pass_yinv(p, 1, Slab{c * lz, lz}, st);
            pass_xinv(p, sv, 1, alpha, beta, Slab{c * lz, lz}, st);
            LSFC_HIP(hipEventRecord(ev, st));
            if (helper) {
                { std::lock_guard<std::mutex> lk(dmu); dq.push_back(Down{ev, yj + off, ys + off, sl, c == K - 1, j}); }
                dcv.notify_all();
            } else {
                LSFC_HIP(hipStreamWaitEvent(hp->down, ev, 0));
                LSFC_HIP(hipMemcpyAsync(yj + off, ys + off, (size_t)chunk * sizeof(cplx), hipMemcpyDeviceToHost, hp->down));
            }
        }
        LSFC_HIP(hipEventRecord(hp->ev_xfree[sl], st));
        if (!helper) LSFC_HIP(hipEventRecord(hp->ev_yfree[sl], hp->down));
    }
    if (helper) {
        { std::lock_guard<std::mutex> lk(dmu); ddone = true; }
        dcv.notify_all();
        dthread.join();
        if (derr) std::rethrow_exception(derr);
    }
    LSFC_HIP(hipStreamSynchronize(hp->down));
    LSFC_HIP(hipStreamSynchronize(st));
}

static void convolve_any(lsfc_plan* p, const double* x, double* y, int64_t nrhs, bool use_nu, double alpha, double beta, int memspace) {
    LSFC_REQUIRE(p && x && y, "NULL argument");
    LSFC_REQUIRE(nrhs >= 1, "nrhs must be >= 1");
    if (p->multi) {
        LSFC_REQUIRE(memspace == LSFC_MEM_HOST, "a multi-device plan takes host vectors here; per-device slabs go through lsfc_multi_apply_dev");
        for (int64_t j = 0; j < nrhs; ++j) multi_convolve_host(p, (const cplx*)x + j * p->N, (cplx*)y + j * p->N, use_nu, alpha, beta);
        return;
    }
    LSFC_HIP(hipSetDevice(p->device));
    if (memspace == LSFC_MEM_DEVICE) {
        for (int64_t j0 = 0; j0 < nrhs; j0 += LSFC_MAX_BATCH) {
            const int cnt = (int)std::min<int64_t>(LSFC_MAX_BATCH, nrhs - j0);
            VecBatch vb{};
            for (int j = 0; j < cnt; ++j) { vb.x[j] = (const cplx*)x + (j0 + j) * p->N; vb.y[j] = (cplx*)y + (j0 + j) * p->N; }
            plan_convolve_batch_dev(p, cnt, vb, use_nu, alpha, beta);
        }
        return;
    }
    LSFC_REQUIRE(memspace == LSFC_MEM_HOST, "unknown memspace %d", memspace);
    const int group = (int)std::min<int64_t>(LSFC_MAX_BATCH, nrhs);
    const int K = host_pipeline_chunks(p);
    if (K <= 1) ensure_staging(p, p->N * group);
    if (K > 1) {
        host_pipelined_convolve(p, (const cplx*)x, (cplx*)y, nrhs, use_nu, alpha, beta, K);
        return;
    }
    static const bool sync_copy = env_switch("LSFC_HOST_COPY") == 's';
    for (int64_t j0 = 0; j0 < nrhs; j0 += group) {
        const int cnt = (int)std::min<int64_t>(group, nrhs - j0);
        const size_t bytes = (size_t)cnt * p->N * sizeof(cplx);
        if (sync_copy) {
            LSFC_HIP(hipStreamSynchronize(p->stream));
            LSFC_HIP(hipMemcpy(p->xs.p, (const cplx*)x + j0 * p->N, bytes, hipMemcpyHostToDevice));
        } else LSFC_HIP(hipMemcpyAsync(p->xs.p, (const cplx*)x + j0 * p->N, bytes, hipMemcpyHostToDevice, p->stream));
        VecBatch vb{};
        for (int j = 0; j < cnt; ++j) { vb.x[j] = p->xs.p + (int64_t)j * p->N; vb.y[j] = p->ys.p + (int64_t)j * p->N; }
        plan_convolve_batch_dev(p, cnt, vb, use_nu, alpha, beta);
        LSFC_HIP(hipMemcpyAsync((cplx*)y + j0 * p->N, p->ys.p, bytes, hipMemcpyDeviceToHost, p->stream));
        LSFC_HIP(hipStreamSynchronize(p->stream));
    }
}

void plan_kernel0(lsfc_plan* p) {
    const int64_t N = p->N;
    if (p->kernel0.n == (size_t)N) return;
    p->kernel0.alloc((size_t)N);
    DevBuf<cplx> e; e.alloc((size_t)N);
    LSFC_HIP(hipMemsetAsync(e.p, 0, (size_t)N * sizeof(cplx), p->stream));
    const cplx one = make_double2(1.0, 0.0);
    LSFC_HIP(hipMemcpyAsync(e.p, &one, sizeof one, hipMemcpyHostToDevice, p->stream));
    plan_convolve_dev(p, e.p, p->kernel0.p, false, 0.0, 1.0);
    LSFC_HIP(hipStreamSynchronize(p->stream));
}
}

using namespace lsfc;

lsfc_plan::lsfc_plan() {}
lsfc_plan::~lsfc_plan() {}

extern "C" {

const char* lsfc_last_error(void) { return g_last_error; }
int lsfc_padded_length(int64_t n) { return (n >= 1 && n <= 1024) ? lsfc::pruned_best_length(n) : 0; }

const char* lsfc_version(void) { return "lsfc 0.1 (gfx950, rocFFT + hand-written pruned FFT passes)"; }

static int create_from_literal(lsfc_plan** out, int ndim, int64_t n, int64_t m, int64_t l, int64_t ne, int64_t me, int64_t le,
                               const double* nu, const double* gfft, double omega, int quad_rule, unsigned flags, int device) {
    return guarded([&] {
        LSFC_REQUIRE(out && gfft, "NULL argument");
        *out = nullptr;
        std::unique_ptr<lsfc_plan> p(new lsfc_plan());
        plan_common_init(p.get(), ndim, n, m, l, nu, omega, quad_rule, flags, device);
        LSFC_REQUIRE(ne >= 1 && me >= 1 && le >= 1 && ne <= 16384 && me <= 16384 && le <= 16384, "padded size out of range");
        const int lit[3] = { (int)ne, (int)me, (int)le };
        const int64_t ltotal = ne * me * le;
        DevBuf<cplx> Gd; Gd.alloc((size_t)ltotal);
        LSFC_HIP(hipMemcpy(Gd.p, gfft, (size_t)ltotal * sizeof(cplx), hipMemcpyHostToDevice));
        const bool trap = quad_rule == LSFC_QUAD_TRAPEZOIDAL;
        for (int d = 0; d < ndim; ++d)
            LSFC_REQUIRE(lit[d] >= (trap ? 2 * p->dims[d] - 1 : p->dims[d]), "padded size %d too small along axis %d", lit[d], d);
        int origin[3]; for (int d = 0; d < 3; ++d) origin[d] = (trap && d < ndim) ? p->dims[d] - 1 : 0;
        if (flags & LSFC_FLAG_LITERAL_PAD) {
            for (int d = 0; d < 3; ++d) { p->pads[d] = lit[d]; p->crop[d] = origin[d]; }
            plan_finish_literal(p.get(), Gd.p, !trap);
        } else {
            plan_finish_reduce(p.get(), Gd, lit, !trap, origin);
        }
        *out = p.release();
    });
}

int lsfc_plan_create_2d(lsfc_plan** out, int64_t n, int64_t m, int64_t ne, int64_t me, const double* nu, const double* gfft,
                        double omega, int quad_rule, unsigned flags, int device) {
    return create_from_literal(out, 2, n, m, 1, ne, me, 1, nu, gfft, omega, quad_rule, flags, device);
}
int lsfc_plan_create_3d(lsfc_plan** out, int64_t n, int64_t m, int64_t l, int64_t ne, int64_t me, int64_t le, const double* nu,
                        const double* gfft, double omega, int quad_rule, unsigned flags, int device) {
    return create_from_literal(out, 3, n, m, l, ne, me, le, nu, gfft, omega, quad_rule, flags, device);
}

int lsfc_plan_create_gv3d(lsfc_plan** out, int64_t n, int64_t m, int64_t l, double box, double omega, const double* nu,
                          unsigned flags, int device) {
    return guarded([&] {
        LSFC_REQUIRE(out, "NULL argument"); *out = nullptr;
        LSFC_REQUIRE(n % 2 == 0 && m % 2 == 0 && l % 2 == 0, "buildFastConvolution3D: even n only (the reference's odd branch is broken)");
        LSFC_REQUIRE(box > 0, "box must be positive");
        PhaseTimer pt;
        std::unique_ptr<lsfc_plan> p(new lsfc_plan());
        plan_common_init(p.get(), 3, n, m, l, nu, omega, LSFC_QUAD_GREENGARD_VICO, flags & ~LSFC_FLAG_LITERAL_PAD, device);
        pt.mark("init + nu upload");
        DevBuf<cplx> G2;
        plan_choose_reduced_grid(p.get());
        if (p->pipeline == lsfc_plan::PRUNED && plan_quarter_symbol_ok(p.get())) {
            symbol_gv3d_quarter(p.get(), box, G2);
            pt.mark("symbol (total; through its symmetry)");
            plan_finish_symbol(p.get(), G2, true);
        } else {
            symbol_gv3d_reduced(p.get(), box, G2);
            pt.mark("symbol (total)");
            plan_finish_symbol(p.get(), G2, false);
        }
        pt.mark("tables, symbol permutation, work arrays");
        *out = p.release();
    });
}

int lsfc_plan_create_gv2d(lsfc_plan** out, int64_t n, int64_t m, double box, double omega, const double* nu, unsigned flags, int device) {
    return guarded([&] {
        LSFC_REQUIRE(out, "NULL argument"); *out = nullptr;
        LSFC_REQUIRE(box > 0, "box must be positive");
        std::unique_ptr<lsfc_plan> p(new lsfc_plan());
        plan_common_init(p.get(), 2, n, m, 1, nu, omega, LSFC_QUAD_GREENGARD_VICO, flags, device);
        DevBuf<cplx> G; int lit[3];
        symbol_gv2d_literal(p.get(), box, G, lit);
        const int origin[3] = { 0, 0, 0 };
        if (flags & LSFC_FLAG_LITERAL_PAD) {
            for (int d = 0; d < 3; ++d) { p->pads[d] = lit[d]; p->crop[d] = 0; }
            plan_finish_literal(p.get(), G.p, true);
        } else plan_finish_reduce(p.get(), G, lit, true, origin);
        *out = p.release();
    });
}

int lsfc_plan_create_trap2d(lsfc_plan** out, int64_t n, int64_t m, double x0, double y0, double h, double omega,
                            double d0_re, double d0_im, const double* nu, unsigned flags, int device) {
    return guarded([&] {
        LSFC_REQUIRE(out, "NULL argument"); *out = nullptr;
        LSFC_REQUIRE(n % 2 == 1 && m % 2 == 1, "so far only works for n odd (src/FastConvolution.jl:455)");
        std::unique_ptr<lsfc_plan> p(new lsfc_plan());
        plan_common_init(p.get(), 2, n, m, 1, nu, omega, LSFC_QUAD_TRAPEZOIDAL, flags, device);
        DevBuf<cplx> G;
        symbol_trap2d_literal(p.get(), x0, y0, h, make_double2(d0_re, d0_im), G);
        const int lit[3] = { 2 * (int)n - 1, 2 * (int)m - 1, 1 };
        const int origin[3] = { (int)n - 1, (int)m - 1, 0 };
        if (flags & LSFC_FLAG_LITERAL_PAD) {
            for (int d = 0; d < 3; ++d) { p->pads[d] = lit[d]; p->crop[d] = origin[d]; }
            plan_finish_literal(p.get(), G.p, false);
        } else plan_finish_reduce(p.get(), G, lit, false, origin);
        *out = p.release();
    });
}

int lsfc_plan_destroy(lsfc_plan* plan) {
    return guarded([&] {
        if (!plan) return;
        if (plan->multi) multi_synchronize(plan);
        else { (void)hipSetDevice(plan->device); (void)hipStreamSynchronize(plan->stream); }
        delete plan;
    });
}

int64_t lsfc_plan_size(const lsfc_plan* plan) { return plan ? plan->N : -1; }

int lsfc_plan_dims(const lsfc_plan* plan, int64_t dims[3], int64_t pads[3]) {
    return guarded([&] {
        LSFC_REQUIRE(plan, "NULL plan");
        for (int d = 0; d < 3; ++d) { if (dims) dims[d] = plan->dims[d]; if (pads) pads[d] = plan->pads[d]; }
    });
}

const char* lsfc_plan_pipeline(const lsfc_plan* plan) {
    if (!plan) return "";
    switch (plan->pipeline) {
    case lsfc_plan::PRUNED: return "pruned-hip";
    case lsfc_plan::ROCFFT_REDUCED: return "rocfft-reduced";
    default: return "rocfft-literal";
    }
}

int lsfc_plan_set_nu(lsfc_plan* plan, const double* nu, int memspace) {
    return guarded([&] {
        LSFC_REQUIRE(plan && nu, "NULL argument");
        if (plan->multi) {
            LSFC_REQUIRE(memspace == LSFC_MEM_HOST, "a multi-device plan takes nu from the host");
            int64_t off = 0;
            for (auto& sp : plan->multi->sub) {
                LSFC_HIP(hipSetDevice(sp->device));
                LSFC_HIP(hipMemcpy(sp->nu.p, nu + off, sp->N * sizeof(double), hipMemcpyHostToDevice));
                off += sp->N;
            }
            return;
        }
        LSFC_HIP(hipSetDevice(plan->device));
        LSFC_HIP(hipMemcpyAsync(plan->nu.p, nu, plan->N * sizeof(double),
                                memspace == LSFC_MEM_DEVICE ? hipMemcpyDeviceToDevice : hipMemcpyHostToDevice, plan->stream));
        LSFC_HIP(hipStreamSynchronize(plan->stream));
    });
}

int lsfc_plan_get_symbol(const lsfc_plan* plan, double* out, int64_t capacity_complex, int64_t* count) {
    return guarded([&] {
        LSFC_REQUIRE(plan && count, "NULL argument");
        LSFC_REQUIRE(!plan->multi, "not available on a multi-device plan");
        *count = (int64_t)plan->sym.n;
        if (out) {
            LSFC_REQUIRE(capacity_complex >= (int64_t)plan->sym.n, "buffer too small");
            LSFC_HIP(hipMemcpy(out, plan->sym.p, plan->sym.bytes(), hipMemcpyDeviceToHost));
        }
    });
}

int lsfc_apply(lsfc_plan* plan, const double* x, double* y, int memspace) {
    return guarded([&] { LSFC_REQUIRE(plan, "NULL plan"); convolve_any(plan, x, y, 1, true, 1.0, plan->omega * plan->omega, memspace); });
}
int lsfc_convolve(lsfc_plan* plan, const double* x, double* y, int apply_nu, int memspace) {
    return guarded([&] { convolve_any(plan, x, y, 1, apply_nu != 0, 0.0, 1.0, memspace); });
}
int lsfc_apply_batch(lsfc_plan* plan, const double* x, double* y, int64_t nrhs, int mode, int memspace) {
    return guarded([&] {
        LSFC_REQUIRE(plan, "NULL plan");
        LSFC_REQUIRE(mode >= 0 && mode <= 2, "mode must be 0 (apply), 1 (convolve) or 2 (convolve with nu)");
        if (mode == 0) convolve_any(plan, x, y, nrhs, true, 1.0, plan->omega * plan->omega, memspace);
        else convolve_any(plan, x, y, nrhs, mode == 2, 0.0, 1.0, memspace);
    });
}

int lsfc_sample_sources(lsfc_plan* plan, const int64_t* sources, int64_t nsrc, double* out, int memspace) {
    return guarded([&] {
        LSFC_REQUIRE(plan && sources && out && nsrc >= 1, "bad argument");
        LSFC_REQUIRE(!plan->dist && !plan->multi, "not available on a distributed plan");
        LSFC_HIP(hipSetDevice(plan->device));
        lsfc_plan* p = plan;
        const int64_t N = p->N;
        for (int64_t s = 0; s < nsrc; ++s) LSFC_REQUIRE(sources[s] >= 0 && sources[s] < N, "source index %lld out of range", (long long)sources[s]);
        plan_kernel0(p);
        DevBuf<int64_t> dsrc; dsrc.alloc((size_t)nsrc);
        LSFC_HIP(hipMemcpyAsync(dsrc.p, sources, (size_t)nsrc * sizeof(int64_t), hipMemcpyHostToDevice, p->stream));
        if (memspace == LSFC_MEM_DEVICE) {
            pw_gather_sources(p->kernel0.p, (cplx*)out, dsrc.p, (int)nsrc, p->dims, p->stream);
            LSFC_HIP(hipStreamSynchronize(p->stream));
        } else {
            const int64_t per = std::max<int64_t>(1, ((int64_t)1 << 24) / N);
            DevBuf<cplx> buf; buf.alloc((size_t)(std::min(per, nsrc) * N));
            for (int64_t s0 = 0; s0 < nsrc; s0 += per) {
                const int64_t cnt = std::min(per, nsrc - s0);
                pw_gather_sources(p->kernel0.p, buf.p, dsrc.p + s0, (int)cnt, p->dims, p->stream);
                LSFC_HIP(hipMemcpyAsync((cplx*)out + s0 * N, buf.p, (size_t)(cnt * N) * sizeof(cplx), hipMemcpyDeviceToHost, p->stream));
                LSFC_HIP(hipStreamSynchronize(p->stream));
            }
        }
    });
}

int lsfc_gmres(lsfc_plan* plan, double* x, const double* b, const lsfc_gmres_opts* opts, double* resnorm, int64_t resnorm_cap,
               lsfc_gmres_result* result, int memspace) {
    int conv_code = LSFC_OK;
    int rc = guarded([&] {
        LSFC_REQUIRE(plan && x && b, "NULL argument");
        LSFC_HIP(hipSetDevice(plan->device));
        lsfc_gmres_result local; lsfc_gmres_result* res = result ? result : &local;
        if (plan->multi) {
            LSFC_REQUIRE(memspace == LSFC_MEM_HOST, "a multi-device plan takes host vectors");
            gmres_run_multi(plan, (cplx*)x, (const cplx*)b, opts, resnorm, resnorm_cap, res);
        } else if (memspace == LSFC_MEM_DEVICE) {
            gmres_run(plan, (cplx*)x, (const cplx*)b, opts, resnorm, resnorm_cap, res);
        } else {
            LSFC_REQUIRE(memspace == LSFC_MEM_HOST, "unknown memspace %d", memspace);
            ensure_staging(plan, plan->N);
            LSFC_HIP(hipMemcpy(plan->xs.p, x, plan->N * sizeof(cplx), hipMemcpyHostToDevice));
            LSFC_HIP(hipMemcpy(plan->ys.p, b, plan->N * sizeof(cplx), hipMemcpyHostToDevice));
            gmres_run(plan, plan->xs.p, plan->ys.p, opts, resnorm, resnorm_cap, res);
            LSFC_HIP(hipMemcpy(x, plan->xs.p, plan->N * sizeof(cplx), hipMemcpyDeviceToHost));
        }
        if (!res->converged) conv_code = LSFC_ENOTCONV;
    });
    if (rc == LSFC_OK && conv_code != LSFC_OK) { set_last_error("gmres: maxiter reached without convergence"); return conv_code; }
    return rc;
}

int lsfc_gmres_batch(lsfc_plan* plan, double* x, const double* b, int64_t nrhs, const lsfc_gmres_opts* opts, double* resnorm,
                     int64_t resnorm_cap, lsfc_gmres_result* results, int memspace) {
    return guarded([&] {
        LSFC_REQUIRE(plan && x && b && results, "NULL argument");
        LSFC_REQUIRE(nrhs >= 1 && nrhs <= 64, "nrhs must be in 1..64");
        LSFC_REQUIRE(!plan->multi && !plan->dist, "batched GMRES runs on a single-device plan");
        LSFC_HIP(hipSetDevice(plan->device));
        if (memspace == LSFC_MEM_DEVICE) {
            gmres_run_batch(plan, (cplx*)x, (const cplx*)b, (int)nrhs, opts, resnorm, resnorm_cap, results);
        } else {
            LSFC_REQUIRE(memspace == LSFC_MEM_HOST, "unknown memspace %d", memspace);
            const size_t bytes = (size_t)nrhs * plan->N * sizeof(cplx);
            DevBuf<cplx> xd, bd; xd.alloc((size_t)nrhs * plan->N); bd.alloc((size_t)nrhs * plan->N);
            LSFC_HIP(hipMemcpy(xd.p, x, bytes, hipMemcpyHostToDevice));
            LSFC_HIP(hipMemcpy(bd.p, b, bytes, hipMemcpyHostToDevice));
            gmres_run_batch(plan, xd.p, bd.p, (int)nrhs, opts, resnorm, resnorm_cap, results);
            LSFC_HIP(hipMemcpy(x, xd.p, bytes, hipMemcpyDeviceToHost));
        }
    });
}

int lsfc_plan_set_stream(lsfc_plan* plan, void* hip_stream) {
    return guarded([&] {
        LSFC_REQUIRE(plan, "NULL plan");
        LSFC_REQUIRE(!plan->multi, "a multi-device plan runs on the streams of its ranks");
        plan->stream = (hipStream_t)hip_stream;
    });
}
int lsfc_plan_synchronize(lsfc_plan* plan) {
    return guarded([&] {
        LSFC_REQUIRE(plan, "NULL plan");
        if (plan->multi) { multi_synchronize(plan); return; }
        LSFC_HIP(hipSetDevice(plan->device)); LSFC_HIP(hipStreamSynchronize(plan->stream));
    });
}

int lsfc_plan_set_tuning(lsfc_plan* plan, const char* key, int value) {
    return guarded([&] {
        LSFC_REQUIRE(plan && key, "NULL argument");
        if (plan->multi) { for (auto& sp : plan->multi->sub) { const int rc = lsfc_plan_set_tuning(sp.get(), key, value); if (rc != LSFC_OK) fail(rc, "%s", lsfc_last_error()); } return; }
        const std::string k(key);
        if (k == "split_x") plan->tuning.split_x = value != 0;
        else if (k == "split_s") plan->tuning.split_s = value != 0;
        else if (k == "split_z") plan->tuning.split_z = value;
        else if (k == "z_half") plan->tuning.z_half = value;
        else if (k == "tw_lds") plan->tuning.tw_lds = value;
        else if (k == "sym_prefetch") plan->tuning.sym_prefetch = value;
        else if (k == "ytile_g") plan->tuning.ytile_g = value;
        else if (k == "ytile_z") plan->tuning.ytile_z = value;
        else if (k == "batch_fuse") plan->tuning.batch_fuse = value;
        else if (k == "z_persist") plan->tuning.z_persist = value;
        else if (k == "xlane") plan->tuning.xlane = value;
        else fail(LSFC_EINVAL, "unknown tuning key '%s'", key);
    });
}

int lsfc_time_apply(lsfc_plan* plan, const double* x_dev, double* y_dev, int reps, double* ms_total) {
    return guarded([&] {
        LSFC_REQUIRE(plan && x_dev && y_dev && ms_total && reps >= 1, "bad argument");
        LSFC_REQUIRE(!plan->multi, "time a multi-device plan from the host around lsfc_multi_apply_dev + lsfc_plan_synchronize");
        LSFC_HIP(hipSetDevice(plan->device));
        hipEvent_t e0, e1;
        LSFC_HIP(hipEventCreate(&e0)); LSFC_HIP(hipEventCreate(&e1));
        LSFC_HIP(hipEventRecord(e0, plan->stream));
        for (int r = 0; r < reps; ++r) plan_apply_dev(plan, (const cplx*)x_dev, (cplx*)y_dev);
        LSFC_HIP(hipEventRecord(e1, plan->stream));
        LSFC_HIP(hipEventSynchronize(e1));
        float ms = 0; LSFC_HIP(hipEventElapsedTime(&ms, e0, e1));
        *ms_total = ms;
        (void)hipEventDestroy(e0); (void)hipEventDestroy(e1);
    });
}

int lsfc_profile_apply(lsfc_plan* plan, const double* x_dev, double* y_dev, int reps, int max_stages, const char** names,
                       double* ms, double* bytes, int* nstages) {
    return guarded([&] {
        LSFC_REQUIRE(plan && names && ms && bytes && nstages && reps >= 1, "bad argument");
        if (plan->multi) { multi_profile(plan, reps, max_stages, names, ms, bytes, nstages); return; }
        LSFC_REQUIRE(x_dev && y_dev, "bad argument");
        LSFC_HIP(hipSetDevice(plan->device));
        lsfc_plan* p = plan;
        const cplx* x = (const cplx*)x_dev; cplx* y = (cplx*)y_dev;
        hipStream_t st = p->stream;
        const double N = (double)p->N, C = 16.0;
        struct Stage { const char* name; double bytes; std::function<void()> run; };
        std::vector<Stage> stages;
        auto stages_add_fn = [](std::vector<Stage>& v) {
            return [&v](const char* name, double bytes, std::function<void()> run) { v.push_back({name, bytes, std::move(run)}); };
        };
        const double om2 = p->omega * p->omega;
        if (p->dist) {
            dist_profile_stages(p, x, y, stages_add_fn(stages));
        } else if (p->pipeline == lsfc_plan::PRUNED) {
            VecBatch vb{}; vb.x[0] = x; vb.y[0] = y;
            const Slab all = whole_grid(p);
            const bool d3 = p->ndim == 3;
            stages.push_back({"xfwd", N * (C + 8) + 2 * N * C, [=] { pass_xfwd(p, vb, 1, p->nu.p, all, st); }});
            if (d3) stages.push_back({"yfwd", (2 + 4) * N * C, [=] { pass_yfwd(p, 1, all, st); }});
            stages.push_back({d3 ? "zfused" : "yfused", d3 ? (4 + 8 + 4) * N * C : (2 + 4 + 2) * N * C, [=] { pass_fused(p, 1, st); }});
            if (d3) stages.push_back({"yinv", (4 + 2) * N * C, [=] { pass_yinv(p, 1, all, st); }});
            stages.push_back({"xinv", (2 + 1 + 1) * N * C, [=] { pass_xinv(p, vb, 1, 1.0, om2, all, st); }});
        } else {
            const int64_t total = (int64_t)p->pads[0] * p->pads[1] * p->pads[2];
            const double P = (double)total;
            stages.push_back({"embed", N * (C + 8) + P * C, [=] { pw_embed(x, p->nu.p, p->W.p, p->dims, p->pads, st); }});
            stages.push_back({"rocfft_fwd", 2 * P * C, [=] { p->fwd->exec(p->W.p, st); }});
            stages.push_back({"symbol_mul", 3 * P * C, [=] { pw_mul_inplace(p->W.p, p->sym.p, total, st); }});
            stages.push_back({"rocfft_inv", 2 * P * C, [=] { p->inv->exec(p->W.p, st); }});
            stages.push_back({"crop_axpy", 3 * N * C, [=] { pw_crop_axpy(p->W.p, x, y, 1.0, om2, p->dims, p->pads, p->crop, st); }});
        }
        LSFC_REQUIRE((int)stages.size() <= max_stages, "max_stages too small (need %d)", (int)stages.size());
        *nstages = (int)stages.size();
        std::vector<hipEvent_t> ev(stages.size() + 1);
        for (auto& e : ev) LSFC_HIP(hipEventCreate(&e));
        for (size_t i = 0; i < stages.size(); ++i) { names[i] = stages[i].name; bytes[i] = stages[i].bytes; ms[i] = 0.0; }
        for (int r = 0; r < reps; ++r) {
            LSFC_HIP(hipEventRecord(ev[0], st));
            for (size_t i = 0; i < stages.size(); ++i) { stages[i].run(); LSFC_HIP(hipEventRecord(ev[i + 1], st)); }
            LSFC_HIP(hipEventSynchronize(ev[stages.size()]));
            for (size_t i = 0; i < stages.size(); ++i) { float t = 0; LSFC_HIP(hipEventElapsedTime(&t, ev[i], ev[i + 1])); ms[i] += t; }
        }
        for (size_t i = 0; i < stages.size(); ++i) ms[i] /= reps;
        for (auto& e : ev) (void)hipEventDestroy(e);
    });
}

int lsfc_device_count(int* count) {
    return guarded([&] { LSFC_REQUIRE(count, "NULL argument"); int c = 0; hipError_t e = hipGetDeviceCount(&c); *count = (e == hipSuccess) ? c : 0; });
}
int lsfc_malloc(void** dptr, size_t bytes, int device) {
    return guarded([&] { LSFC_REQUIRE(dptr, "NULL argument"); select_device(device); LSFC_HIP(hipMalloc(dptr, bytes)); });
}
int lsfc_free(void* dptr) { return guarded([&] { if (dptr) LSFC_HIP(hipFree(dptr)); }); }
int lsfc_memcpy_h2d(void* dst, const void* src, size_t bytes) { return guarded([&] { LSFC_HIP(hipMemcpy(dst, src, bytes, hipMemcpyHostToDevice)); }); }
int lsfc_memcpy_d2h(void* dst, const void* src, size_t bytes) { return guarded([&] { LSFC_HIP(hipMemcpy(dst, src, bytes, hipMemcpyDeviceToHost)); }); }
int lsfc_host_register(void* ptr, size_t bytes) {
    return guarded([&] { LSFC_REQUIRE(ptr && bytes, "NULL argument"); LSFC_HIP(hipHostRegister(ptr, bytes, hipHostRegisterDefault)); });
}
int lsfc_host_unregister(void* ptr) { return guarded([&] { LSFC_REQUIRE(ptr, "NULL argument"); LSFC_HIP(hipHostUnregister(ptr)); }); }
int lsfc_host_alloc(void** ptr, size_t bytes) {
    return guarded([&] { LSFC_REQUIRE(ptr && bytes, "NULL argument"); *ptr = nullptr; LSFC_HIP(hipHostMalloc(ptr, bytes, hipHostMallocDefault)); });
}
int lsfc_host_free(void* ptr) { return guarded([&] { if (ptr) LSFC_HIP(hipHostFree(ptr)); }); }

}
```

fast_solver_lippmann_schwinger_amd/csrc/plan.hpp:

```cpp
#pragma once
#include "common.hpp"
#include "pruned.hpp"
#include <rocfft/rocfft.h>
#include <functional>
#include <memory>
#include <vector>

namespace lsfc {

struct RocFft {
    rocfft_plan plan = nullptr;
    rocfft_execution_info info = nullptr;
    DevBuf<char> work;
    RocFft() = default;
    RocFft(const RocFft&) = delete; RocFft& operator=(const RocFft&) = delete;
    ~RocFft();
    void create(int ndim, const size_t* lengths, bool forward, size_t batch = 1, bool lazy_work = false);
    void create_strided_1d(size_t length, size_t stride, size_t dist, size_t batch, bool forward, bool lazy_work = false);
    void exec(void* buf, hipStream_t stream);
    void release();
private:
    void finish_create();
};

void rocfft_global_setup();

struct GmresWorkspace {
    int restart = 0;
    DevBuf<cplx> V;
    DevBuf<cplx> hdev;
    DevBuf<cplx> ydev;
    DevBuf<cplx> partial;
    DevBuf<cplx> ax;
    cplx* hpin = nullptr;
    cplx* vpin = nullptr;
    hipEvent_t fetched[2] = { nullptr, nullptr };
    ~GmresWorkspace();
};

struct HostPipe {
    hipStream_t up = nullptr, down = nullptr;
    std::vector<hipEvent_t> ev_up, ev_down;
    hipEvent_t ev_free = nullptr;
    hipEvent_t ev_xfree[2] = { nullptr, nullptr };
    hipEvent_t ev_yfree[2] = { nullptr, nullptr };
    ~HostPipe();
};

struct DistState {
    int rank = 0, nranks = 1;
    bool force_overlap = false, force_comm = false;
    bool no_overlap = false, split_edges = true;
    bool sim = false;
    bool member = false;
    void* comm = nullptr;
    void* comm2 = nullptr;
    int lz = 0;
    int W = 0;
    int K = 1;
    int Wc = 0;
    DevBuf<cplx> S1;
    DevBuf<cplx> R1;
    hipStream_t cs1 = nullptr, cs2 = nullptr;
    hipStream_t st2 = nullptr;
    std::vector<hipEvent_t> ev_in, ev_done, ev_back;
    hipEvent_t ev_p1 = nullptr, ev_p1a = nullptr, ev_backa = nullptr;
    ~DistState();
};

struct MultiState {
    int P = 0;
    std::vector<int> devices;
    std::vector<std::unique_ptr<lsfc_plan>> sub;
    bool rccl = false;
    std::vector<void*> comm, comm2;
    cplx* red_pin = nullptr;
    ~MultiState();
};

}

struct lsfc_plan {
    int device = 0;
    hipStream_t stream = nullptr;
    int ndim = 3;
    int dims[3] = {1, 1, 1};
    int pads[3] = {1, 1, 1};
    int crop[3] = {0, 0, 0};
    int64_t N = 0;
    double omega = 0.0;
    int quad_rule = LSFC_QUAD_GREENGARD_VICO;
    unsigned flags = 0;
    enum Pipeline { PRUNED = 0, ROCFFT_REDUCED = 1, ROCFFT_LITERAL = 2 } pipeline = PRUNED;

    lsfc::DevBuf<double> nu;
    lsfc::DevBuf<lsfc::cplx> sym;

    lsfc::PrunedTuning tuning;
    lsfc::DevBuf<lsfc::cplx> tw[3];
    lsfc::DevBuf<lsfc::cplx> twl[3];
    lsfc::DevBuf<lsfc::cplx> A1, A2;
    int sym_rows = 0;
    lsfc::DevBuf<int2> ytab;
    int sym_hz = 0;
    lsfc::DevBuf<int> zmirror;
    int pitch1 = 0, pitch2 = 0;
    int64_t tile2d = 0;
    int64_t a1_elems = 0, a2_elems = 0;
    int batch_cap = 1;

    std::unique_ptr<lsfc::RocFft> fwd, inv;
    lsfc::DevBuf<lsfc::cplx> W;

    lsfc::DevBuf<lsfc::cplx> kernel0;

    lsfc::DevBuf<lsfc::cplx> xs, ys;
    std::unique_ptr<lsfc::HostPipe> hostpipe;

    std::unique_ptr<lsfc::GmresWorkspace> gmres;
    std::vector<std::unique_ptr<lsfc::GmresWorkspace>> gmres_batch;
    std::unique_ptr<lsfc::DistState> dist;
    std::unique_ptr<lsfc::MultiState> multi;

    lsfc_plan();
    ~lsfc_plan();
};

namespace lsfc {

void plan_convolve_dev(lsfc_plan* p, const cplx* x, cplx* y, bool use_nu, double alpha, double beta);
void plan_convolve_batch_dev(lsfc_plan* p, int nrhs, const VecBatch& vb, bool use_nu, double alpha, double beta);
inline void plan_apply_dev(lsfc_plan* p, const cplx* x, cplx* y) { plan_convolve_dev(p, x, y, true, 1.0, p->omega * p->omega); }

void plan_zfused_3d(lsfc_plan* p, int Wc, int64_t a2_off, int64_t sym_off, int nrhs, hipStream_t st);

void plan_common_init(lsfc_plan* p, int ndim, int64_t n, int64_t m, int64_t l, const double* nu_host, double omega,
                      int quad_rule, unsigned flags, int device);

void symbol_gv3d_reduced(lsfc_plan* p, double box, DevBuf<cplx>& G2);
void symbol_gv3d_quarter(lsfc_plan* p, double box, DevBuf<cplx>& Gq);
bool plan_quarter_symbol_ok(const lsfc_plan* p);
void symbol_gv2d_literal(lsfc_plan* p, double box, DevBuf<cplx>& G, int lit[3]);
void symbol_trap2d_literal(lsfc_plan* p, double x0, double y0, double h, cplx d0, DevBuf<cplx>& G);

void dist_convolve_dev(lsfc_plan* p, const cplx* x, cplx* y, bool use_nu, double alpha, double beta);
void dist_allreduce_sum(lsfc_plan* p, cplx* dev, int count);
void dist_profile_stages(lsfc_plan* p, const cplx* x, cplx* y,
                         std::function<void(const char*, double, std::function<void()>)> add);

void plan_make_twiddles(lsfc_plan* p, int axis, int L);
void plan_setup_symbol_rows(lsfc_plan* p, const cplx* G2, const std::vector<int>& perm_y, const std::vector<int>& perm_z, DevBuf<int>& pyrow);

void multi_convolve_dev(lsfc_plan* root, const cplx* const* x, cplx* const* y, bool use_nu, double alpha, double beta);
void multi_convolve_host(lsfc_plan* root, const cplx* x, cplx* y, bool use_nu, double alpha, double beta);
void multi_allreduce_sum(lsfc_plan* root, cplx* const* dev, int count);
void multi_synchronize(lsfc_plan* root);
void multi_profile(lsfc_plan* root, int reps, int max_stages, const char** names, double* ms, double* bytes, int* nstages);

void plan_kernel0(lsfc_plan* p);

void gmres_run(lsfc_plan* p, cplx* x_dev, const cplx* b_dev, const lsfc_gmres_opts* opts, double* resnorm, int64_t cap,
               lsfc_gmres_result* res);
void gmres_run_batch(lsfc_plan* p, cplx* x_dev, const cplx* b_dev, int nrhs, const lsfc_gmres_opts* opts, double* resnorm, int64_t cap,
                     lsfc_gmres_result* res);
void gmres_run_multi(lsfc_plan* root, cplx* x_host, const cplx* b_host, const lsfc_gmres_opts* opts, double* resnorm, int64_t cap,
                     lsfc_gmres_result* res);

}
```

fast_solver_lippmann_schwinger_amd/csrc/pruned.hip:

```cpp
#include "pruned.hpp"
#include <cstdio>
#include <cstdlib>
#include <mutex>
#include <set>

namespace lsfc {

#define LSFC_FAMILY_DECLS(F)                                                                                                   \
    void pruned_xfwd_f##F(int, const PrunedTuning&, const VecBatch&, int, int64_t, const double*, cplx*, const cplx*, int64_t, int, int, int, hipStream_t, int64_t); \
    void pruned_xinv_f##F(int, const PrunedTuning&, const cplx*, const VecBatch&, int, int64_t, double, double, const cplx*, int64_t, int, int, int, hipStream_t, int64_t); \
    void pruned_yfwd_f##F(int, const PrunedTuning&, const cplx*, cplx*, const cplx*, int, int, int, int, int, hipStream_t, int, int64_t, int64_t);     \
    void pruned_yinv_f##F(int, const PrunedTuning&, const cplx*, cplx*, const cplx*, int, int, int, int, int, hipStream_t, int, int64_t, int64_t);     \
    void pruned_zfused_f##F(int, const PrunedTuning&, cplx*, const cplx*, const cplx*, const cplx*, const FusedGeom&, hipStream_t, int, int64_t); \
    void pruned_perm_f##F(int, int*);                                                                                     \
    void pruned_warmup_f##F();                                                                                         \
    int pruned_twfull_len_f##F(int);                                                                                            \
    void pruned_twfull_f##F(int, const cplx*, cplx*);
void warmup_pointwise(); void warmup_symbol(); void warmup_precond(); void warmup_blocktri();
LSFC_FAMILY_DECLS(2)
LSFC_FAMILY_DECLS(3)
LSFC_FAMILY_DECLS(5)

static int family(int64_t L) {
    if (L < 32 || L > 2048) return 0;
    int64_t v = L; while (v % 2 == 0) v /= 2;
    if (v == 1) return 2;
    if (v == 3) return L >= 48 && L <= 1536 ? 3 : 0;
    if (v == 5) return L >= 80 && L <= 1280 ? 5 : 0;
    return 0;
}
bool pruned_length_supported(int64_t L) { return family(L) != 0; }

void pruned_warmup(int device) {
    static std::mutex mu;
    static std::set<int> done;
    std::lock_guard<std::mutex> lock(mu);
    if (done.count(device)) return;
    if (const char* e = getenv("LSFC_EAGER_LOAD")) if (e[0] == '0') return;
    pruned_warmup_f2(); pruned_warmup_f3(); pruned_warmup_f5();
    warmup_pointwise(); warmup_symbol(); warmup_precond(); warmup_blocktri();
    LSFC_HIP(hipDeviceSynchronize());
    done.insert(device);
}

int pruned_best_length(int64_t n) {
    const char* e = getenv("LSFC_POW2_ONLY");
    const bool pow2_only = e && e[0] == '1';
    for (int64_t L = (2 * n > 32 ? 2 * n : 32); L <= 2048; ++L) if (family(L) && (!pow2_only || family(L) == 2)) return (int)L;
    return 0;
}

static bool debug_sync() { static const bool on = getenv("LSFC_DEBUG_SYNC") && getenv("LSFC_DEBUG_SYNC")[0] == '1'; return on; }
static void debug_check(const char* pass, int L) {
    if (!debug_sync()) return;
    const hipError_t e = hipDeviceSynchronize();
    if (e != hipSuccess) { (void)hipGetLastError(); fail(LSFC_EHIP, "%s (line length %d) failed: %s", pass, L, hipGetErrorString(e)); }
    fprintf(stderr, "[lsfc debug] %s L=%d ok\n", pass, L);
}
#define LSFC_ROUTE(L, NAME, ...)                                            \
    switch (family(L)) {                                                    \
    case 2: NAME##_f2(__VA_ARGS__); break;                                  \
    case 3: NAME##_f3(__VA_ARGS__); break;                                  \
    case 5: NAME##_f5(__VA_ARGS__); break;                                  \
    default: fail(LSFC_EINVAL, "pruned pipeline: unsupported padded length %d", (int)(L)); } \
    debug_check(#NAME, (int)(L));

void pruned_xfwd(int L, const PrunedTuning& tn, const VecBatch& vb, int nrhs, int64_t obatch, const double* nu, cplx* out, const cplx* tw, int64_t nlines, int W, int Wp, int n, hipStream_t st, int64_t bstride) {
    LSFC_REQUIRE(nrhs >= 1 && nrhs <= LSFC_MAX_BATCH, "batch of %d right-hand sides (1..%d per launch)", nrhs, LSFC_MAX_BATCH);
    LSFC_ROUTE(L, pruned_xfwd, L, tn, vb, nrhs, obatch, nu, out, tw, nlines, W, Wp, n, st, bstride);
}
void pruned_xinv(int L, const PrunedTuning& tn, const cplx* in, const VecBatch& vb, int nrhs, int64_t ibatch, double alpha, double beta, const cplx* tw, int64_t nlines, int W, int Wp, int n, hipStream_t st, int64_t bstride) {
    LSFC_REQUIRE(nrhs >= 1 && nrhs <= LSFC_MAX_BATCH, "batch of %d right-hand sides (1..%d per launch)", nrhs, LSFC_MAX_BATCH);
    LSFC_ROUTE(L, pruned_xinv, L, tn, in, vb, nrhs, ibatch, alpha, beta, tw, nlines, W, Wp, n, st, bstride);
}
void pruned_yfwd(int L, const PrunedTuning& tn, const cplx* a1, cplx* a2, const cplx* tw, int Lx, int m, int l, int p1, int p2, hipStream_t st, int nrhs, int64_t b1, int64_t b2) {
    LSFC_ROUTE(L, pruned_yfwd, L, tn, a1, a2, tw, Lx, m, l, p1, p2, st, nrhs, b1, b2);
}
void pruned_yinv(int L, const PrunedTuning& tn, const cplx* a2, cplx* a1, const cplx* tw, int Lx, int m, int l, int p1, int p2, hipStream_t st, int nrhs, int64_t b1, int64_t b2) {
    LSFC_ROUTE(L, pruned_yinv, L, tn, a2, a1, tw, Lx, m, l, p1, p2, st, nrhs, b1, b2);
}
void pruned_zfused(int L, const PrunedTuning& tn, cplx* data, const cplx* sym, const cplx* tw, const cplx* twl, const FusedGeom& g, hipStream_t st, int nrhs, int64_t dBatch) {
    LSFC_ROUTE(L, pruned_zfused, L, tn, data, sym, tw, twl, g, st, nrhs, dBatch);
}
void pruned_perm(int L, int* freq_of_storage) {
    switch (family(L)) {
    case 2: pruned_perm_f2(L, freq_of_storage); break;
    case 3: pruned_perm_f3(L, freq_of_storage); break;
    case 5: pruned_perm_f5(L, freq_of_storage); break;
    default: fail(LSFC_EINVAL, "pruned pipeline: unsupported padded length %d", L); }
}
int pruned_twfull_len(int L) {
    switch (family(L)) {
    case 2: return pruned_twfull_len_f2(L);
    case 3: return pruned_twfull_len_f3(L);
    case 5: return pruned_twfull_len_f5(L);
    default: fail(LSFC_EINVAL, "pruned pipeline: unsupported padded length %d", L);
    }
}
void pruned_twfull(int L, const cplx* tw, cplx* out) {
    switch (family(L)) {
    case 2: pruned_twfull_f2(L, tw, out); break;
    case 3: pruned_twfull_f3(L, tw, out); break;
    case 5: pruned_twfull_f5(L, tw, out); break;
    default: fail(LSFC_EINVAL, "pruned pipeline: unsupported padded length %d", L); }
}

static bool env_flag(const char* name, bool dflt) {
    const char* v = getenv(name);
    if (!v || !*v) return dflt;
    return v[0] == '1' || v[0] == 'y' || v[0] == 't';
}

PrunedTuning pruned_default_tuning() {
    PrunedTuning t;
    t.split_x = env_flag("LSFC_SPLIT_X", true);
    t.split_s = env_flag("LSFC_SPLIT_S", true);
    if (const char* v = getenv("LSFC_SPLIT_Z")) t.split_z = atoi(v);
    if (const char* v = getenv("LSFC_PAD1")) t.pad1 = atoi(v);
    if (const char* v = getenv("LSFC_PAD2")) t.pad2 = atoi(v);
    if (const char* v = getenv("LSFC_Z_HALF")) t.z_half = atoi(v);
    if (const char* v = getenv("LSFC_TW_LDS")) t.tw_lds = atoi(v);
    if (const char* v = getenv("LSFC_SYM_PREFETCH")) t.sym_prefetch = atoi(v);
    if (const char* v = getenv("LSFC_YTILE_G")) t.ytile_g = atoi(v);
    if (const char* v = getenv("LSFC_YTILE_Z")) t.ytile_z = atoi(v);
    if (const char* v = getenv("LSFC_BATCH_FUSE")) t.batch_fuse = atoi(v);
    if (const char* v = getenv("LSFC_Z_PERSIST")) t.z_persist = atoi(v);
    if (const char* v = getenv("LSFC_XLANE")) t.xlane = atoi(v);
    return t;
}

}
```

fast_solver_lippmann_schwinger_amd/csrc/pruned.hpp:

```cpp
#pragma once
#include "common.hpp"

namespace lsfc {

static constexpr int LSFC_MAX_BATCH = 8;
struct VecBatch {
    const cplx* x[LSFC_MAX_BATCH];
    cplx* y[LSFC_MAX_BATCH];
};

struct PrunedTuning {
    bool split_x = true;
    bool split_s = true;
    int split_z = -1;
    int sym_prefetch = -1;
    int pad1 = -1, pad2 = -1;
    int tw_lds = 1;
    int z_half = -1;
    int z_persist = -1;
    int xlane = -1;
    int ytile_g = 0, ytile_z = 0;
    int batch_fuse = -1;
};

bool pruned_length_supported(int64_t L);
void pruned_warmup(int device);
int pruned_best_length(int64_t n);
void pruned_perm(int L, int* freq_of_storage);
PrunedTuning pruned_default_tuning();

void pruned_xfwd(int L, const PrunedTuning&, const VecBatch& vb, int nrhs, int64_t obatch, const double* nu, cplx* out, const cplx* tw, int64_t nlines, int W, int Wp, int n, hipStream_t,
                 int64_t bstride = 0);
void pruned_xinv(int L, const PrunedTuning&, const cplx* in, const VecBatch& vb, int nrhs, int64_t ibatch, double alpha, double beta,
                 const cplx* tw, int64_t nlines, int W, int Wp, int n, hipStream_t, int64_t bstride = 0);
void pruned_yfwd(int L, const PrunedTuning&, const cplx* a1, cplx* a2, const cplx* tw, int Lx, int m, int l, int p1, int p2, hipStream_t,
                 int nrhs = 1, int64_t batch1 = 0, int64_t batch2 = 0);
void pruned_yinv(int L, const PrunedTuning&, const cplx* a2, cplx* a1, const cplx* tw, int Lx, int m, int l, int p1, int p2, hipStream_t,
                 int nrhs = 1, int64_t batch1 = 0, int64_t batch2 = 0);
int pruned_twfull_len(int L);
void pruned_twfull(int L, const cplx* tw, cplx* out);
struct FusedGeom {
    int Lx;
    int nouter;
    int64_t dTile, dOuter, dLine;
    int64_t sTile, sOuter, sLine;
    const int2* ytab;
    const int* zm;
    int nin;
};
void pruned_zfused(int L, const PrunedTuning&, cplx* data, const cplx* sym, const cplx* tw, const cplx* twl, const FusedGeom&, hipStream_t,
                   int nrhs = 1, int64_t dBatch = 0);

}
```

fast_solver_lippmann_schwinger_amd/operators.py:

```python
from __future__ import annotations

import ctypes as C

import numpy as np

from . import _lib as L


def _is_torch(a):
    return type(a).__module__.split(".")[0] == "torch"


def _vec(a, N, name, count=1, plan=None):
    if _is_torch(a):
        import torch
        if a.dtype != torch.complex128 or not a.is_contiguous() or a.numel() != N * count:
            raise TypeError(f"{name}: need a contiguous complex128 tensor with {N * count} entries")
        if a.is_cuda and plan is not None:
            L.check(L.load().lsfc_plan_set_stream(plan, C.c_void_p(torch.cuda.current_stream(a.device).cuda_stream)))
        return C.c_void_p(a.data_ptr()), (L.LSFC_MEM_DEVICE if a.is_cuda else L.LSFC_MEM_HOST), a
    arr = np.ascontiguousarray(a, dtype=np.complex128)
    if arr.size != N * count:
        raise ValueError(f"DimensionMismatch: {name} has {arr.size} entries, operator needs {N * count}")
    return arr.ctypes.data_as(C.c_void_p), L.LSFC_MEM_HOST, arr


_QUAD = {"trapezoidal": L.LSFC_QUAD_TRAPEZOIDAL, "Greengard_Vico": L.LSFC_QUAD_GREENGARD_VICO}


class _Operator:
    _plan = None

    def size(self, dim=None):
        N = int(self.nu.shape[0])
        return N if dim is not None else ((N,), (N,))

    @property
    def shape(self):
        N = int(self.nu.shape[0])
        return (N, N)

    def eltype(self):
        return np.complex128

    dtype = np.complex128

    @property
    def N(self):
        return int(L.load().lsfc_plan_size(self._plan))

    @property
    def pipeline(self):
        return L.load().lsfc_plan_pipeline(self._plan).decode()

    @property
    def padded_dims(self):
        d, p = (C.c_int64 * 3)(), (C.c_int64 * 3)()
        L.check(L.load().lsfc_plan_dims(self._plan, d, p))
        return tuple(p)

    def _out_like(self, b, count=1):
        if _is_torch(b):
            import torch
            return torch.empty(self.N * count, dtype=torch.complex128, device=b.device)
        return np.empty(self.N * count, dtype=np.complex128)

    def __mul__(self, b):
        return fastconvolution(self, b)

    __matmul__ = __mul__
    matvec = __mul__

    def mul_(self, Y, b):
        px, sx, kx = _vec(b, self.N, "b", plan=self._plan)
        if _is_torch(Y):
            py, sy, _ = _vec(Y, self.N, "Y")
            if sy != sx:
                raise TypeError("Y and b must live in the same memory space")
            L.check(L.load().lsfc_apply(self._plan, px, py, sx))
            return Y
        if not (isinstance(Y, np.ndarray) and Y.dtype == np.complex128 and Y.flags.c_contiguous and Y.size == self.N):
            raise TypeError("Y: need a contiguous complex128 array of the operator size")
        if sx != L.LSFC_MEM_HOST:
            raise TypeError("Y and b must live in the same memory space")
        L.check(L.load().lsfc_apply(self._plan, px, Y.ctypes.data_as(C.c_void_p), sx))
        return Y

    def set_nu(self, nu):
        nu = np.ascontiguousarray(nu, dtype=np.float64)
        if nu.size != self.N:
            raise ValueError("DimensionMismatch: nu")
        L.check(L.load().lsfc_plan_set_nu(self._plan, nu.ctypes.data_as(C.c_void_p), L.LSFC_MEM_HOST))
        self.nu = nu

    def working_symbol(self):
        cnt = C.c_int64(0)
        L.check(L.load().lsfc_plan_get_symbol(self._plan, None, 0, C.byref(cnt)))
        out = np.empty(cnt.value, dtype=np.complex128)
        L.check(L.load().lsfc_plan_get_symbol(self._plan, out.ctypes.data_as(C.c_void_p), cnt.value, C.byref(cnt)))
        return out

    def set_tuning(self, **knobs):
        for key, value in knobs.items():
            L.check(L.load().lsfc_plan_set_tuning(self._plan, key.encode(), int(value)))

    def synchronize(self):
        L.check(L.load().lsfc_plan_synchronize(self._plan))

    def close(self):
        if self._plan is not None:
            L.load().lsfc_plan_destroy(self._plan)
            self._plan = None

    def __del__(self):
        try:
            self.close()
        except Exception:
            pass


class FastM(_Operator):

    def __init__(self, GFFT, nu, ne, me, n, m, k, quadRule="trapezoidal", flags=0, device=0, _plan=None):
        self.GFFT, self.ne, self.me, self.n, self.m = GFFT, int(ne), int(me), int(n), int(m)
        self.omega, self.quadRule = float(k), quadRule
        self.nu = np.ascontiguousarray(nu, dtype=np.float64).reshape(-1)
        if _plan is not None:
            self._plan = _plan
            return
        if quadRule not in _QUAD:
            raise NameError(f"UndefVarError: B not defined (unknown quadRule {quadRule!r})")
        G = np.asarray(GFFT, dtype=np.complex128)
        if G.shape != (self.ne, self.me):
            raise ValueError(f"DimensionMismatch: GFFT has shape {G.shape}, expected {(self.ne, self.me)}")
        if self.nu.size != self.n * self.m:
            raise ValueError("DimensionMismatch: nu")
        Gf = np.asfortranarray(G)
        plan = C.c_void_p()
        L.check(L.load().lsfc_plan_create_2d(C.byref(plan), self.n, self.m, self.ne, self.me,
                                             self.nu.ctypes.data_as(C.c_void_p), Gf.ctypes.data_as(C.c_void_p),
                                             self.omega, _QUAD[quadRule], flags, device))
        self._plan = plan


class FastM3D(_Operator):

    def __init__(self, GFFT, nu, ne, me, le, n, m, l, k, quadRule="Greengard_Vico", flags=0, device=0, _plan=None):
        self.GFFT = GFFT
        self.ne, self.me, self.le, self.n, self.m, self.l = int(ne), int(me), int(le), int(n), int(m), int(l)
        self.omega, self.quadRule = float(k), quadRule
        self.nu = np.ascontiguousarray(nu, dtype=np.float64).reshape(-1)
        if _plan is not None:
            self._plan = _plan
            return
        if quadRule not in _QUAD:
            raise NameError(f"UndefVarError: B not defined (unknown quadRule {quadRule!r})")
        G = np.asarray(GFFT, dtype=np.complex128)
        if G.shape != (self.ne, self.me, self.le):
            raise ValueError(f"DimensionMismatch: GFFT has shape {G.shape}, expected {(self.ne, self.me, self.le)}")
        if self.nu.size != self.n * self.m * self.l:
            raise ValueError("DimensionMismatch: nu")
        Gf = np.asfortranarray(G)
        plan = C.c_void_p()
        L.check(L.load().lsfc_plan_create_3d(C.byref(plan), self.n, self.m, self.l, self.ne, self.me, self.le,
                                             self.nu.ctypes.data_as(C.c_void_p), Gf.ctypes.data_as(C.c_void_p),
                                             self.omega, _QUAD[quadRule], flags, device))
        self._plan = plan


def size(M, dim=None):
    return M.size(dim)


def eltype(M):
    return M.eltype()


def fastconvolution(M, b):
    px, sx, keep = _vec(b, M.N, "b", plan=M._plan)
    y = M._out_like(keep)
    py, _, _ = _vec(y, M.N, "y")
    L.check(L.load().lsfc_apply(M._plan, px, py, sx))
    return y


def mul_(Y, M, b):
    return M.mul_(Y, b)


def FFTconvolution(M, b):
    if isinstance(M, FastM) and M.n != M.m:
        raise ValueError("DimensionMismatch: FFTconvolution(::FastM) assumes n == m")
    apply_nu = 1 if (isinstance(M, FastM) and M.quadRule == "trapezoidal") else 0
    px, sx, keep = _vec(b, M.N, "b", plan=M._plan)
    y = M._out_like(keep)
    py, _, _ = _vec(y, M.N, "y")
    L.check(L.load().lsfc_convolve(M._plan, px, py, apply_nu, sx))
    return y


def referenceValsTrapRule():
    x = 2.0 ** (-np.arange(6.0))
    w = np.array([1 - 0.892j, 1 - 1.35j, 1 - 1.79j, 1 - 2.23j, 1 - 2.67j, 1 - 3.11j])
    return x, w


def _grid2d(x, y):
    n, m = len(x), len(y)
    X = np.repeat(np.asarray(x, float)[:, None], m, axis=1).reshape(-1, order="F")
    Y = np.repeat(np.asarray(y, float)[None, :], n, axis=0).reshape(-1, order="F")
    return X, Y


def buildFastConvolution(x, y, h, k, nu, quadRule="trapezoidal", flags=0, device=0):
    x, y = np.asarray(x, float), np.asarray(y, float)
    n, m = len(x), len(y)
    X, Y = _grid2d(x, y)
    nuv = np.ascontiguousarray(nu(X, Y), dtype=np.float64)
    plan = C.c_void_p()
    if quadRule == "trapezoidal":
        _, D = referenceValsTrapRule()
        idx = int(round(k * h))
        if not 1 <= idx <= len(D):
            raise IndexError(f"BoundsError: attempt to access {len(D)}-element Vector at index [{idx}] "
                             "(D[round(Int, k*h)], src/FastConvolution.jl:176)")
        D0 = D[idx - 1]
        L.check(L.load().lsfc_plan_create_trap2d(C.byref(plan), n, m, float(x[0]), float(y[0]), float(h), float(k),
                                                 float(D0.real), float(D0.imag), nuv.ctypes.data_as(C.c_void_p), flags, device))
        return FastM(None, nuv, 2 * n - 1, 2 * m - 1, n, m, k, quadRule="trapezoidal", _plan=plan)
    if quadRule == "Greengard_Vico":
        box = abs(x[-1] - x[0]) + h
        L.check(L.load().lsfc_plan_create_gv2d(C.byref(plan), n, m, float(box), float(k), nuv.ctypes.data_as(C.c_void_p), flags, device))
        return FastM(None, nuv, 4 * n, 4 * m, n, m, k, quadRule="Greengard_Vico", _plan=plan)
    raise NameError(f"UndefVarError: unknown quadRule {quadRule!r}")


def buildFastConvolution3D(x, y, z, X, Y, Z, h, k, nu, quadRule="Greengard_Vico", flags=0, device=0):
    if quadRule != "Greengard_Vico":
        raise NameError(f"UndefVarError: unknown quadRule {quadRule!r}")
    x = np.asarray(x, float)
    n, m, l = len(x), len(y), len(z)
    nuv = np.ascontiguousarray(nu(X, Y, Z) if callable(nu) else nu, dtype=np.float64).reshape(-1)
    box = abs(x[-1] - x[0]) + h
    plan = C.c_void_p()
    L.check(L.load().lsfc_plan_create_gv3d(C.byref(plan), n, m, l, float(box), float(k), nuv.ctypes.data_as(C.c_void_p), flags, device))
    return FastM3D(None, nuv, 4 * n, 4 * m, 4 * l, n, m, l, k, _plan=plan)


def sampleGConv(k, X, Y, indS, fastconv):
    return _sample(indS, fastconv)


def sampleG3D(k, X, Y, Z, indS, fastconv):
    return _sample(indS, fastconv)


def _sample(indS, M):
    N, ns = M.N, len(indS)
    out = np.empty((ns, N), dtype=np.complex128)
    if isinstance(M, FastM) and M.quadRule == "trapezoidal":
        R = np.zeros((ns, N), dtype=np.complex128)
        for i, ii in enumerate(indS):
            R[i, ii] = 1.0
        L.check(L.load().lsfc_apply_batch(M._plan, R.ctypes.data_as(C.c_void_p), out.ctypes.data_as(C.c_void_p), ns, 2, L.LSFC_MEM_HOST))
        return out
    src = np.ascontiguousarray(indS, dtype=np.int64)
    L.check(L.load().lsfc_sample_sources(M._plan, src.ctypes.data_as(C.c_void_p), ns, out.ctypes.data_as(C.c_void_p), L.LSFC_MEM_HOST))
    return out


class ConvergenceHistory:

    def __init__(self, resnorm, iters, mvps, isconverged):
        self.data = {"resnorm": resnorm}
        self.iters, self.mvps, self.isconverged = iters, mvps, isconverged

    def __getitem__(self, key):
        return self.data[key.lstrip(":")]


class _DevPtr:

    def __init__(self, ptr, n):
        self.__cuda_array_interface__ = {"shape": (n,), "typestr": "<c16", "data": (ptr, False), "version": 2}


def _device_view(ptr, n):
    import torch
    return torch.as_tensor(_DevPtr(ptr, n), device="cuda")


_ORTH = {"ModifiedGramSchmidt": L.LSFC_ORTH_MGS, "ClassicalGramSchmidt": L.LSFC_ORTH_CGS, "DGKS": L.LSFC_ORTH_DGKS}


def gmres_(x, A, b, Pl=None, abstol=0.0, reltol=None, restart=None, maxiter=None, log=False,
           initially_zero=False, orth_meth="ModifiedGramSchmidt", Pl_on_device=False):
    N = A.N
    px, sx, keepx = _vec(x, N, "x", plan=A._plan)
    pb, sb, keepb = _vec(b, N, "b")
    if sx != sb:
        raise TypeError("x and b must live in the same memory space")
    if not _is_torch(x) and keepx is not x:
        raise TypeError("x must be a contiguous complex128 array (it is updated in place)")
    opts = L.GmresOpts()
    opts.restart = int(restart) if restart is not None else 0
    opts.maxiter = int(maxiter) if maxiter is not None else 0
    opts.reltol = float(reltol) if reltol is not None else -1.0
    opts.abstol = float(abstol)
    opts.orth = _ORTH[orth_meth]
    opts.initially_zero = 1 if initially_zero else 0
    err = []
    native_pc = getattr(Pl, "_pc", None) if Pl is not None else None
    if native_pc is not None:
        if sx == L.LSFC_MEM_DEVICE:
            import torch
            Pl.set_stream(torch.cuda.current_stream(x.device).cuda_stream)
        else:
            L.check(L.load().lsfc_plan_set_stream(A._plan, None))
            Pl.set_stream(0)
        lib = L.load()
        opts.precond = C.cast(lib.lsfc_precond_callback, L.PRECOND_FN)
        opts.precond_user = native_pc
        opts.precond_on_device = 1
    elif Pl is not None:
        def _cb(user, v, n):
            try:
                if Pl_on_device:
                    Pl(_device_view(C.cast(v, C.c_void_p).value, n))
                    return 0
                arr = np.ctypeslib.as_array(C.cast(v, C.POINTER(C.c_double)), shape=(2 * n,)).view(np.complex128)
                Pl(arr)
                return 0
            except Exception as e:
                err.append(e)
                return 1
        cb = L.PRECOND_FN(_cb)
        opts.precond = cb
        opts.precond_on_device = 1 if Pl_on_device else 0
    cap = int(maxiter) if maxiter is not None else N
    cap = max(1, min(cap, 1 << 20))
    res = L.GmresResult()
    resnorm = np.zeros(cap, dtype=np.float64)
    rc = L.load().lsfc_gmres(A._plan, px, pb, C.byref(opts), resnorm.ctypes.data_as(C.c_void_p), cap, C.byref(res), sx)
    if err:
        raise err[0]
    if rc not in (0, L.LSFC_ENOTCONV):
        L.check(rc)
    if log:
        return x, ConvergenceHistory(resnorm[:min(res.iters, cap)].copy(), int(res.iters), int(res.mvps), bool(res.converged))
    return x


def _precond_opts(opts, Pl, Pl_on_device, A, x, sx, err):
    native_pc = getattr(Pl, "_pc", None) if Pl is not None else None
    if native_pc is not None:
        if sx == L.LSFC_MEM_DEVICE:
            import torch
            Pl.set_stream(torch.cuda.current_stream(x.device).cuda_stream)
        else:
            L.check(L.load().lsfc_plan_set_stream(A._plan, None))
            Pl.set_stream(0)
        opts.precond = C.cast(L.load().lsfc_precond_callback, L.PRECOND_FN)
        opts.precond_user = native_pc
        opts.precond_on_device = 1
        return None
    if Pl is None:
        return None

    def _cb(user, v, n):
        try:
            if Pl_on_device:
                Pl(_device_view(C.cast(v, C.c_void_p).value, n))
                return 0
            Pl(np.ctypeslib.as_array(C.cast(v, C.POINTER(C.c_double)), shape=(2 * n,)).view(np.complex128))
            return 0
        except Exception as e:
            err.append(e)
            return 1
    cb = L.PRECOND_FN(_cb)
    opts.precond = cb
    opts.precond_on_device = 1 if Pl_on_device else 0
    return cb


def bicgstabl_(x, A, b, l=2, Pl=None, max_mv_products=None, abstol=0.0, reltol=None, log=False, Pl_on_device=False,
               r_shadow=None, initially_zero=False):
    N = A.N
    px, sx, keepx = _vec(x, N, "x", plan=A._plan)
    pb, sb, keepb = _vec(b, N, "b")
    if sx != sb:
        raise TypeError("x and b must live in the same memory space")
    if not _is_torch(x) and keepx is not x:
        raise TypeError("x must be a contiguous complex128 array (it is updated in place)")
    opts = L.BicgstablOpts()
    opts.l = int(l)
    opts.max_mv_products = int(max_mv_products) if max_mv_products is not None else 0
    opts.reltol = float(reltol) if reltol is not None else -1.0
    opts.abstol = float(abstol)
    opts.initially_zero = 1 if initially_zero else 0
    keeps = None
    if r_shadow is not None:
        ps, ss, keeps = _vec(r_shadow, N, "r_shadow")
        if ss != sx:
            raise TypeError("r_shadow and x must live in the same memory space")
        opts.r_shadow = ps
    err = []
    cb = _precond_opts(opts, Pl, Pl_on_device, A, x, sx, err)
    cap = (opts.max_mv_products if opts.max_mv_products > 0 else N) // (2 * max(opts.l, 1)) + 2
    cap = max(1, min(cap, 1 << 20))
    res = L.GmresResult()
    resnorm = np.zeros(cap, dtype=np.float64)
    rc = L.load().lsfc_bicgstabl(A._plan, px, pb, C.byref(opts), resnorm.ctypes.data_as(C.c_void_p), cap, C.byref(res), sx)
    del cb, keeps, keepb
    if err:
        raise err[0]
    if rc not in (0, L.LSFC_ENOTCONV):
        L.check(rc)
    if log:
        hist = ConvergenceHistory(resnorm[:min(res.iters, cap)].copy(), int(res.iters), int(res.mvps), bool(res.converged))
        hist.message = L.load().lsfc_last_error().decode(errors="replace") if rc == L.LSFC_ENOTCONV else ""
        return x, hist
    return x


def apply_batch(M, B, mode=0):
    if _is_torch(B):
        nrhs = B.shape[0]
        pb, sb, keep = _vec(B.reshape(-1), M.N, "B", count=nrhs, plan=M._plan)
        import torch
        Y = torch.empty_like(keep)
        L.check(L.load().lsfc_apply_batch(M._plan, pb, C.c_void_p(Y.data_ptr()), nrhs, mode, sb))
        return Y.reshape(nrhs, M.N)
    B = np.ascontiguousarray(B, dtype=np.complex128)
    if B.ndim != 2 or B.shape[1] != M.N:
        raise ValueError(f"DimensionMismatch: B must be (nrhs, {M.N})")
    Y = np.empty_like(B)
    L.check(L.load().lsfc_apply_batch(M._plan, B.ctypes.data_as(C.c_void_p), Y.ctypes.data_as(C.c_void_p), B.shape[0], mode, L.LSFC_MEM_HOST))
    return Y


def gmres_batch_(X, A, B, Pl=None, abstol=0.0, reltol=None, restart=None, maxiter=None, log=False,
                 initially_zero=False, orth_meth="ModifiedGramSchmidt"):
    torch_in = _is_torch(X)
    if torch_in:
        nrhs = X.shape[0]
        px, sx, keepx = _vec(X.reshape(-1), A.N, "X", count=nrhs, plan=A._plan)
        pb, sb, keepb = _vec(B.reshape(-1), A.N, "B", count=nrhs)
        if keepx.data_ptr() != X.data_ptr():
            raise TypeError("X must be contiguous (it is updated in place)")
    else:
        if not (isinstance(X, np.ndarray) and X.dtype == np.complex128 and X.flags.c_contiguous and X.ndim == 2 and X.shape[1] == A.N):
            raise TypeError(f"X must be a C-contiguous complex128 array of shape (nrhs, {A.N}) (it is updated in place)")
        nrhs = X.shape[0]
        Bc = np.ascontiguousarray(B, dtype=np.complex128)
        if Bc.shape != X.shape:
            raise ValueError("DimensionMismatch: B")
        px, sx, pb, sb, keepb = X.ctypes.data_as(C.c_void_p), L.LSFC_MEM_HOST, Bc.ctypes.data_as(C.c_void_p), L.LSFC_MEM_HOST, Bc
    if sx != sb:
        raise TypeError("X and B must live in the same memory space")
    opts = L.GmresOpts()
    opts.restart = int(restart) if restart is not None else 0
    opts.maxiter = int(maxiter) if maxiter is not None else 0
    opts.reltol = float(reltol) if reltol is not None else -1.0
    opts.abstol = float(abstol)
    opts.orth = _ORTH[orth_meth]
    opts.initially_zero = 1 if initially_zero else 0
    err = []
    native_pc = getattr(Pl, "_pc", None) if Pl is not None else None
    if native_pc is not None:
        if sx == L.LSFC_MEM_DEVICE:
            import torch
            Pl.set_stream(torch.cuda.current_stream(X.device).cuda_stream)
        else:
            L.check(L.load().lsfc_plan_set_stream(A._plan, None))
            Pl.set_stream(0)
        opts.precond = C.cast(L.load().lsfc_precond_callback, L.PRECOND_FN)
        opts.precond_user = native_pc
        opts.precond_on_device = 1
    elif Pl is not None:
        def _cb(user, v, n):
            try:
                Pl(np.ctypeslib.as_array(C.cast(v, C.POINTER(C.c_double)), shape=(2 * n,)).view(np.complex128))
                return 0
            except Exception as e:
                err.append(e)
                return 1
        cb = L.PRECOND_FN(_cb)
        opts.precond = cb
    cap = max(1, min(int(maxiter) if maxiter is not None else A.N, 1 << 20))
    res = (L.GmresResult * nrhs)()
    resnorm = np.zeros((nrhs, cap), dtype=np.float64)
    rc = L.load().lsfc_gmres_batch(A._plan, px, pb, nrhs, C.byref(opts), resnorm.ctypes.data_as(C.c_void_p), cap, res, sx)
    if err:
        raise err[0]
    L.check(rc)
    if log:
        return X, [ConvergenceHistory(resnorm[j, :min(res[j].iters, cap)].copy(), int(res[j].iters), int(res[j].mvps), bool(res[j].converged))
                   for j in range(nrhs)]
    return X


def time_apply(M, x_dev, y_dev, reps):
    px, sx, _ = _vec(x_dev, M.N, "x")
    py, sy, _ = _vec(y_dev, M.N, "y")
    if sx != L.LSFC_MEM_DEVICE or sy != L.LSFC_MEM_DEVICE:
        raise TypeError("time_apply needs device tensors")
    ms = C.c_double(0)
    L.check(L.load().lsfc_time_apply(M._plan, px, py, int(reps), C.byref(ms)))
    return ms.value


def profile_apply(M, x_dev, y_dev, reps=3):
    px = _vec(x_dev, M.N, "x")[0] if x_dev is not None else None
    py = _vec(y_dev, M.N, "y")[0] if y_dev is not None else None
    names = (C.c_char_p * 16)()
    ms, nb, ns = (C.c_double * 16)(), (C.c_double * 16)(), C.c_int(0)
    L.check(L.load().lsfc_profile_apply(M._plan, px, py, int(reps), 16, names, ms, nb, C.byref(ns)))
    return [(names[i].decode(), ms[i], nb[i]) for i in range(ns.value)]
```

include/lsfc.h:

```cpp
#ifndef LSFC_H
#define LSFC_H

#include <stddef.h>
#include <stdint.h>

#ifdef __cplusplus
extern "C" {
#endif

typedef struct lsfc_plan lsfc_plan;

#define LSFC_OK        0
#define LSFC_EINVAL   -1
#define LSFC_ENODEV   -2
#define LSFC_ENOMEM   -3
#define LSFC_EHIP     -4
#define LSFC_ENOTCONV -5

#define LSFC_QUAD_TRAPEZOIDAL     0
#define LSFC_QUAD_GREENGARD_VICO  1

#define LSFC_MEM_HOST    0
#define LSFC_MEM_DEVICE  1

#define LSFC_FLAG_DEFAULT        0u
#define LSFC_FLAG_LITERAL_PAD    1u
#define LSFC_FLAG_FORCE_ROCFFT   2u
#define LSFC_FLAG_PATCH_SINGULAR 4u

#define LSFC_ORTH_MGS   0
#define LSFC_ORTH_CGS   1
#define LSFC_ORTH_DGKS  2


int lsfc_plan_create_2d(lsfc_plan** out, int64_t n, int64_t m, int64_t ne, int64_t me,
                        const double* nu, const double* gfft, double omega,
                        int quad_rule, unsigned flags, int device);

int lsfc_plan_create_3d(lsfc_plan** out, int64_t n, int64_t m, int64_t l,
                        int64_t ne, int64_t me, int64_t le,
                        const double* nu, const double* gfft, double omega,
                        int quad_rule, unsigned flags, int device);

int lsfc_plan_create_gv2d(lsfc_plan** out, int64_t n, int64_t m, double box, double omega,
                          const double* nu, unsigned flags, int device);

int lsfc_plan_create_trap2d(lsfc_plan** out, int64_t n, int64_t m, double x0, double y0, double h,
                            double omega, double d0_re, double d0_im,
                            const double* nu, unsigned flags, int device);

int lsfc_plan_create_gv3d(lsfc_plan** out, int64_t n, int64_t m, int64_t l, double box, double omega,
                          const double* nu, unsigned flags, int device);

int lsfc_plan_destroy(lsfc_plan* plan);


int64_t lsfc_plan_size(const lsfc_plan* plan);
int lsfc_plan_dims(const lsfc_plan* plan, int64_t dims[3], int64_t pads[3]);
const char* lsfc_plan_pipeline(const lsfc_plan* plan);
int lsfc_plan_set_nu(lsfc_plan* plan, const double* nu, int memspace);
int lsfc_plan_get_symbol(const lsfc_plan* plan, double* out, int64_t capacity_complex, int64_t* count);


int lsfc_apply(lsfc_plan* plan, const double* x, double* y, int memspace);

int lsfc_convolve(lsfc_plan* plan, const double* x, double* y, int apply_nu, int memspace);

int lsfc_apply_batch(lsfc_plan* plan, const double* x, double* y, int64_t nrhs, int mode , int memspace);

int lsfc_sample_sources(lsfc_plan* plan, const int64_t* sources, int64_t nsrc, double* out, int memspace);


typedef int (*lsfc_precond_fn)(void* user, double* v, int64_t n);

typedef struct lsfc_gmres_opts {
    int     restart;
    int64_t maxiter;
    double  reltol;
    double  abstol;
    int     orth;
    int     initially_zero;
    lsfc_precond_fn precond; void* precond_user;
    int     precond_on_device;
} lsfc_gmres_opts;

typedef struct lsfc_gmres_result {
    int64_t iters;
    int64_t mvps;
    int     converged;
    double  final_resnorm;
} lsfc_gmres_result;

int lsfc_gmres(lsfc_plan* plan, double* x, const double* b, const lsfc_gmres_opts* opts,
               double* resnorm, int64_t resnorm_cap, lsfc_gmres_result* result, int memspace);

int lsfc_gmres_batch(lsfc_plan* plan, double* x, const double* b, int64_t nrhs, const lsfc_gmres_opts* opts,
                     double* resnorm, int64_t resnorm_cap, lsfc_gmres_result* results, int memspace);


typedef struct lsfc_bicgstabl_opts {
    int     l;
    int64_t max_mv_products;
    double  reltol;
    double  abstol;
    int     initially_zero;
    lsfc_precond_fn precond; void* precond_user;
    int     precond_on_device;
    const double* r_shadow;
    int     reserved[4];
} lsfc_bicgstabl_opts;

int lsfc_bicgstabl(lsfc_plan* plan, double* x, const double* b, const lsfc_bicgstabl_opts* opts,
                   double* resnorm, int64_t resnorm_cap, lsfc_gmres_result* result, int memspace);


typedef struct lsfc_precond lsfc_precond;
int lsfc_precond_create(lsfc_precond** out, int64_t N,
                        const int64_t* As_rowptr, const int64_t* As_col, const double* As_val,
                        const int64_t* L_rowptr, const int64_t* L_col, const double* L_val,
                        const int64_t* U_rowptr, const int64_t* U_col, const double* U_val,
                        const int64_t* row_gather, const int64_t* col_scatter, const double* row_scale, int device);
int lsfc_precond_destroy(lsfc_precond* pc);
int lsfc_precond_set_stream(lsfc_precond* pc, void* stream);
int lsfc_precond_apply(lsfc_precond* pc, double* v, int memspace);
int lsfc_precond_apply_batch(lsfc_precond* pc, double* v, int64_t nrhs, int memspace);
int lsfc_precond_batch_info(const lsfc_precond* pc, int64_t out[4]);
int lsfc_precond_callback(void* user, double* v, int64_t n);
int lsfc_precond_stats(const lsfc_precond* pc, int64_t* levels_L, int64_t* levels_U, int64_t* launches);
int lsfc_precond_schedule(const lsfc_precond* pc, int factor, int64_t out[10]);

int lsfc_precond_create_blocktri(lsfc_precond** out, int64_t N, int64_t nblocks, const int64_t* rowptr, const int64_t* col,
                                 const double* As_val, const double* Msp_val, int memspace, int device);
int lsfc_precond_create_from_plan(lsfc_precond** out, lsfc_plan* plan);
#define LSFC_PRECOND_INV_F64 0
#define LSFC_PRECOND_INV_F32 1
int lsfc_precond_create_blocktri_prec(lsfc_precond** out, int64_t N, int64_t nblocks, const int64_t* rowptr, const int64_t* col,
                                      const double* As_val, const double* Msp_val, int memspace, int device, int inverse_precision);
int lsfc_precond_create_from_plan_prec(lsfc_precond** out, lsfc_plan* plan, int inverse_precision);
int lsfc_precond_inverse_precision(const lsfc_precond* pc, int* precision);
#define LSFC_PRECOND_PIVOT_NONE 0
#define LSFC_PRECOND_PIVOT_PARTIAL 1
#define LSFC_PRECOND_PIVOT_AUTO 2
typedef struct lsfc_blocktri_opts { int inverse_precision; int pivoting; int reserved[6]; } lsfc_blocktri_opts;
int lsfc_precond_create_blocktri_opts(lsfc_precond** out, int64_t N, int64_t nblocks, const int64_t* rowptr, const int64_t* col,
                                      const double* As_val, const double* Msp_val, int memspace, int device, const lsfc_blocktri_opts* opts);
int lsfc_precond_create_from_plan_opts(lsfc_precond** out, lsfc_plan* plan, const lsfc_blocktri_opts* opts);
int lsfc_precond_blocktri_get_pivots(const lsfc_precond* pc, int64_t k, int64_t* perm, int64_t capacity);
int lsfc_precond_blocktri_info(const lsfc_precond* pc, int64_t out[6], double* min_pivot_ratio);
int lsfc_precond_blocktri_get_block(const lsfc_precond* pc, int64_t k, double* out, int64_t capacity_complex);



int lsfc_sparsify_pattern(int64_t n, int64_t m, int64_t l, int64_t* nnz, int64_t* rowptr, int64_t* col, int64_t* row_class);

int lsfc_sparsify_build(lsfc_plan* plan, int64_t* rowptr, int64_t* col, double* As_val, double* AG_val,
                        double* Msp_val, double* sigma, int memspace);


int lsfc_plan_set_stream(lsfc_plan* plan, void* hip_stream);
int lsfc_plan_synchronize(lsfc_plan* plan);
int lsfc_time_apply(lsfc_plan* plan, const double* x_dev, double* y_dev, int reps, double* ms_total);
int lsfc_profile_apply(lsfc_plan* plan, const double* x_dev, double* y_dev, int reps,
                       int max_stages, const char** names, double* ms, double* bytes, int* nstages);

int lsfc_plan_set_tuning(lsfc_plan* plan, const char* key, int value);

int lsfc_device_count(int* count);
int lsfc_malloc(void** dptr, size_t bytes, int device);
int lsfc_free(void* dptr);
int lsfc_memcpy_h2d(void* dst_dev, const void* src_host, size_t bytes);
int lsfc_memcpy_d2h(void* dst_host, const void* src_dev, size_t bytes);
int lsfc_host_register(void* ptr, size_t bytes);
int lsfc_host_unregister(void* ptr);
int lsfc_host_alloc(void** ptr, size_t bytes);
int lsfc_host_free(void* ptr);


#define LSFC_UNIQUE_ID_BYTES 128
int lsfc_dist_unique_id(unsigned char id[LSFC_UNIQUE_ID_BYTES]);

int lsfc_dist_plan_create_gv3d(lsfc_plan** out, int64_t n, int64_t m, int64_t l, double box, double omega,
                               const double* nu_local, unsigned flags, int device,
                               int rank, int nranks, const unsigned char id[LSFC_UNIQUE_ID_BYTES]);

int lsfc_dist_sim_plan_create_gv3d(lsfc_plan** out, int64_t n, int64_t m, int64_t l, double box, double omega,
                                   const double* nu_local, unsigned flags, int device, int rank, int nranks);
int lsfc_dist_sim_apply(lsfc_plan** plans, int nranks, const double* const* x, double* const* y, int mode);


int lsfc_plan_create_gv3d_multi(lsfc_plan** out, int64_t n, int64_t m, int64_t l, double box, double omega,
                                const double* nu, unsigned flags, const int* devices, int ndev);
int lsfc_multi_info(const lsfc_plan* plan, int* ndev, int* devices, int64_t* local_n, const char** transport);
int lsfc_multi_apply_dev(lsfc_plan* plan, const double* const* x_dev, double* const* y_dev, int mode);

int lsfc_padded_length(int64_t n);

const char* lsfc_last_error(void);
const char* lsfc_version(void);

#ifdef __cplusplus
}
#endif
#endif
```

Before: 81.04 applies/s.

## Store only x-mirror-representative symbol tiles and reorder tickets to pair mirror chunks

The 3D symbol is even in x, so the plan now stores only representative 8-wide x chunks and builds an x-mirror table that maps each data chunk to a stored symbol tile plus a lane permutation. The fused z kernels index the symbol through this table. The persistent ticket order is changed so mirrored chunk pairs are processed back to back, letting the second one hit the same symbol tile in cache. This roughly halves symbol storage and HBM traffic for the multiply. The cost is an extra table lookup and per-lane index arithmetic, plus a dependence on the evenness check.

```diff
diff --git a/fast_solver_lippmann_schwinger_amd/_lib.py b/fast_solver_lippmann_schwinger_amd/_lib.py
--- a/fast_solver_lippmann_schwinger_amd/_lib.py
+++ b/fast_solver_lippmann_schwinger_amd/_lib.py
@@ -109,6 +109,8 @@
     "lsfc_multi_apply_dev": (_I, [_P, _PP, _PP, _I]),
     "lsfc_last_error": (C.c_char_p, []),
     "lsfc_padded_length": (_I, [C.c_int64]),
+    "lsfc_xmirror_table": (_I, [_L, _P, _P, _P]),
+    "lsfc_plan_symbol_bytes": (_L, [_P]),
     "lsfc_version": (C.c_char_p, []),
 }
 
diff --git a/fast_solver_lippmann_schwinger_amd/csrc/fft_kernels.hip b/fast_solver_lippmann_schwinger_amd/csrc/fft_kernels.hip
--- a/fast_solver_lippmann_schwinger_amd/csrc/fft_kernels.hip
+++ b/fast_solver_lippmann_schwinger_amd/csrc/fft_kernels.hip
@@ -145,7 +145,8 @@
 __global__ __launch_bounds__(C::T * LINES, WPE)
 void k_zfused(cplx* __restrict__ data, const cplx* __restrict__ sym, const cplx* __restrict__ tw,
               int nouter, int64_t dGrp, int64_t dOuter, int64_t dLine, int64_t sGrp, int64_t sOuter, int64_t sLine,
-              const int2* __restrict__ ytab, const int* __restrict__ zm, int nin, int nrhs, int64_t dBatch, int sibling_pairs) {
+              const int2* __restrict__ ytab, const int* __restrict__ zm, int nin, int nrhs, int64_t dBatch, int sibling_pairs,
+              const int4* __restrict__ xtab) {
     using LL = LdsLayout<LINES, 3, SPLIT>;
     extern __shared__ __attribute__((aligned(16))) char smem[];
     constexpr int T = C::T, E = C::E;
@@ -163,8 +164,10 @@
     const int o = tile % nouter, g = tile / nouter;
     int outer = o, srow = o;
     if (ytab) { const int2 e = ytab[o]; outer = e.x; srow = e.y; }
-    cplx* d = data + g * dGrp + outer * dOuter + xi;
-    const cplx* s = sym + g * sGrp + srow * sOuter + xi;
+    int gd = g, gs = g, sxi = xi;
+    if (xtab) { const int4 x4 = xtab[g]; gd = x4.x; gs = x4.y; sxi = (int)(((unsigned)x4.z >> (4 * xi)) & 7u); }
+    cplx* d = data + gd * dGrp + outer * dOuter + xi;
+    const cplx* s = sym + gs * sGrp + srow * sOuter + sxi;
     const int li = threadIdx.x % LINES;
     if constexpr (TWL) {
         cplx* tl = reinterpret_cast<cplx*>(smem + (size_t)LL::line_elems(C::L) * LINES * LL::elem_bytes());
@@ -296,7 +299,8 @@
 __global__ __launch_bounds__(C::T * LINES, (HALF && 2 * persist_lds_bytes<C, LINES, SPLIT, TWL, HALF>() <= (size_t)160 * 1024) ? 2 : 1)
 void k_zfused_persist(cplx* __restrict__ data, const cplx* __restrict__ sym, const cplx* __restrict__ tw,
                       int nouter, int64_t dGrp, int64_t dOuter, int64_t dLine, int64_t sGrp, int64_t sOuter, int64_t sLine,
-                      const int2* __restrict__ ytab, const int* __restrict__ zm, int nin, unsigned ntiles, unsigned* __restrict__ tickets) {
+                      const int2* __restrict__ ytab, const int* __restrict__ zm, int nin, unsigned ntiles, unsigned* __restrict__ tickets,
+                      const int4* __restrict__ xtab, int xgroup) {
     using LL = LdsLayout<LINES, HALF ? -1 : 3, SPLIT>;
     extern __shared__ __attribute__((aligned(16))) char smem[];
     constexpr int T = C::T, E = C::E, H = E / 2;
@@ -341,33 +345,41 @@
         __syncthreads();
         tw = tl;
     }
-    auto locate = [&](unsigned w, cplx*& dbase, const cplx*& sbase, unsigned sub = 0) {
+    auto locate = [&](unsigned w, cplx*& dbase, const cplx*& sbase, unsigned& smap, unsigned sub = 0) {
         unsigned tl_ = w; int half = 0;
         if constexpr (PAIR) tl_ = ticket_decode_pair(w, sub);
         else if constexpr (TICKETS) { unsigned hf; ticket_decode<HALF>(w, tl_, hf); half = (int)hf * LINES; }
-        const int o = (int)(tl_ % (unsigned)nouter), g = (int)(tl_ / (unsigned)nouter);
-        int outer = o, srow = o;
+        int o, g;
+        if (TICKETS && xgroup) {
+            const unsigned u = (tl_ & 15u) | ((tl_ >> 5) << 4);
+            o = (int)(u % (unsigned)nouter); g = (int)(2u * (u / (unsigned)nouter) + ((tl_ >> 4) & 1u));
+        } else { o = (int)(tl_ % (unsigned)nouter); g = (int)(tl_ / (unsigned)nouter); }
+        int outer = o, srow = o, gs = g;
+        unsigned lm = 0x76543210u;
         if (ytab) { const int2 e2 = ytab[o]; outer = e2.x; srow = e2.y; }
+        if (xtab) { const int4 x4 = xtab[g]; g = x4.x; gs = x4.y; lm = (unsigned)x4.z; }
         dbase = data + g * dGrp + outer * dOuter + half;
-        sbase = sym + g * sGrp + srow * sOuter + half;
+        sbase = sym + gs * sGrp + srow * sOuter;
+        smap = lm >> (4 * half);
     };
     const unsigned doff = (unsigned)(li + (int)dLine * t), dstep = (unsigned)((int)dLine * T);
-    const unsigned soff = (unsigned)(li + (int)sLine * t), sstep = (unsigned)((int)sLine * T);
+    const unsigned soff = (unsigned)((int)sLine * t), sstep = (unsigned)((int)sLine * T);
     constexpr bool MIRG = (XL & 2) != 0;
     [[maybe_unused]] unsigned moff[MIRG ? H : 1];
     if constexpr (MIRG) {
 #pragma unroll
-        for (int e = 0; e < H; ++e) moff[e] = (unsigned)(li + (int)sLine * zm[t + T * e]);
+        for (int e = 0; e < H; ++e) moff[e] = (unsigned)((int)sLine * zm[t + T * e]);
     }
     cplx nd[H];
     {
-        cplx* d; const cplx* s;
-        locate(cur, d, s);
+        cplx* d; const cplx* s; unsigned m;
+        locate(cur, d, s, m);
 #pragma unroll
         for (int e = 0; e < H; ++e) nd[e] = (EXACT || t + T * e < nin) ? d[doff + dstep * e] : make_double2(0.0, 0.0);
     }
     [[maybe_unused]] unsigned sub = 0;
     [[maybe_unused]] const cplx* sheld = nullptr;
+    [[maybe_unused]] unsigned mheld = 0;
     [[maybe_unused]] cplx sv_pair[PAIR ? H : 1];
     [[maybe_unused]] cplx smid_pair = make_double2(0.0, 0.0);
     for (;;) {
@@ -382,20 +394,21 @@
         cplx smid_tile = make_double2(0.0, 0.0);
         cplx& smid = PAIR ? smid_pair : smid_tile;
         auto load_symbol = [&] {
-            cplx* d; const cplx* s;
-            locate(cur, d, s, sub);
+            cplx* d; const cplx* s; unsigned m;
+            locate(cur, d, s, m, sub);
             if constexpr (PAIR) {
-                if (s == sheld) return;
-                sheld = s;
+                if (s == sheld && m == mheld) return;
+                sheld = s; mheld = m;
             }
-            const unsigned so = launder_v(soff);
+            const unsigned sl = (m >> (4 * li)) & 7u;
+            const unsigned so = launder_v(soff) + sl;
 #pragma unroll
             for (int e = 0; e < H; ++e) sv[e] = s[so + sstep * e];
             if constexpr (MIRG) {
 #pragma unroll
-                for (int e = 0; e < H; ++e) smr[e] = s[moff[e]];
+                for (int e = 0; e < H; ++e) smr[e] = s[moff[e] + sl];
             } else {
-                if (t == 0) smid = s[so - (unsigned)((int)sLine * t) + (unsigned)((int)sLine * (C::L / 2))];
+                if (t == 0) smid = s[sl + (unsigned)((int)sLine * (C::L / 2))];
             }
         };
         if constexpr (!SPLIT && WS) {
@@ -443,8 +456,8 @@
         }
         const bool more = PAIR ? (sub == 0 || next != DONE) : (TICKETS ? next != DONE : next < nwork);
         if (more) {
-            cplx* dn; const cplx* sn;
-            if (PAIR && sub == 0) locate(cur, dn, sn, 1u); else locate(next, dn, sn, 0u);
+            cplx* dn; const cplx* sn; unsigned mn;
+            if (PAIR && sub == 0) locate(cur, dn, sn, mn, 1u); else locate(next, dn, sn, mn, 0u);
             const unsigned dof = launder_v(doff);
 #pragma unroll
             for (int e = 0; e < H; ++e) nd[e] = (EXACT || t + T * e < nin) ? dn[dof + dstep * e] : make_double2(0.0, 0.0);
@@ -452,8 +465,8 @@
         if constexpr (!SPLIT && WS) fft_inverse_ws<C, LL, true, TWL, DEFER, (XL > 0)>(v, t, tw, smem, 0, li);
         else fft_inverse<C, LL, true, TWL>(v, t, tw, smem, 0, li);
         {
-            cplx* d; const cplx* s;
-            locate(cur, d, s, sub);
+            cplx* d; const cplx* s; unsigned m;
+            locate(cur, d, s, m, sub);
             const unsigned dof = launder_v(doff);
 #pragma unroll
             for (int e = 0; e < H; ++e) if (EXACT || t + T * e < nin) d[dof + dstep * e] = v[e];
@@ -477,6 +490,8 @@
 }
 
 static bool env_flag_no_sibling_pairs() { static const bool v = getenv("LSFC_NO_SIBLING_PAIRS") != nullptr; return v; }
+static bool env_flag_xmirror_group() { static const bool v = [] { const char* e = getenv("LSFC_XMIRROR_GROUP"); return !(e && e[0] == '0'); }(); return v; }
+static int xmirror_group(const FusedGeom& g) { return (g.xtab && g.nouter % 16 == 0 && (g.Lx / XB) % 2 == 0 && env_flag_xmirror_group()) ? 1 : 0; }
 static bool env_flag_z_quarter() { static const bool v = [] { const char* e = getenv("LSFC_Z_QUARTER"); return e && e[0] == '1'; }(); return v; }
 
 template <class C> struct Tune {
@@ -549,12 +564,12 @@
     if (LINES == XB) {
         hipLaunchKernelGGL(k, dim3((unsigned)((g.Lx / XB) * g.nouter)), dim3(C::T * LINES), lds, st, data, sym, tw, g.nouter,
                            g.dTile, g.dOuter, g.dLine, g.sTile, g.sOuter, g.sLine, g.ytab, g.zm, g.nin, nrhs, dBatch,
-                           0);
+                           0, g.xtab);
     } else {
-        LSFC_REQUIRE(g.dTile == XB && g.sTile == XB, "sub-tile groups need the natural (2D) layout");
+        LSFC_REQUIRE(g.dTile == XB && g.sTile == XB && !g.xtab, "sub-tile groups need the natural (2D) layout");
         hipLaunchKernelGGL(k, dim3((unsigned)((g.Lx / LINES) * g.nouter)), dim3(C::T * LINES), lds, st, data, sym, tw, g.nouter,
                            (int64_t)LINES, g.dOuter, g.dLine, (int64_t)LINES, g.sOuter, g.sLine, g.ytab, g.zm, g.nin, nrhs, dBatch,
-                           (XB / LINES == 2 && g.nouter == 1 && (g.Lx / LINES) % 16 == 0 && !env_flag_no_sibling_pairs()) ? 1 : 0);
+                           (XB / LINES == 2 && g.nouter == 1 && (g.Lx / LINES) % 16 == 0 && !env_flag_no_sibling_pairs()) ? 1 : 0, (const int4*)nullptr);
     }
 }
 
@@ -580,7 +595,9 @@
         if (xl == 1) {
             if (twl) k = (g.nin == C::L / 2) ? k_zfused_persist<C, LINES, SPLIT, true, true, LATE_SYM, false, TICKETS, 1> : k_zfused_persist<C, LINES, SPLIT, false, true, LATE_SYM, false, TICKETS, 1>;
             else     k = (g.nin == C::L / 2) ? k_zfused_persist<C, LINES, SPLIT, true, false, LATE_SYM, false, TICKETS, 1> : k_zfused_persist<C, LINES, SPLIT, false, false, LATE_SYM, false, TICKETS, 1>;
-        } else if (xl >= 2 && twl) {
+        } else if (xl >= 2 && !twl) {
+            k = (g.nin == C::L / 2) ? k_zfused_persist<C, LINES, SPLIT, true, false, LATE_SYM, false, TICKETS, 1> : k_zfused_persist<C, LINES, SPLIT, false, false, LATE_SYM, false, TICKETS, 1>;
+        } else if (xl >= 2) {
             if (xl == 5 && TICKETS) k = (g.nin == C::L / 2) ? k_zfused_persist<C, LINES, SPLIT, true, true, LATE_SYM, false, TICKETS, 5> : k_zfused_persist<C, LINES, SPLIT, false, true, LATE_SYM, false, TICKETS, 5>;
             else if (xl == 3) k = (g.nin == C::L / 2) ? k_zfused_persist<C, LINES, SPLIT, true, true, LATE_SYM, false, TICKETS, 3> : k_zfused_persist<C, LINES, SPLIT, false, true, LATE_SYM, false, TICKETS, 3>;
             else k = (g.nin == C::L / 2) ? k_zfused_persist<C, LINES, SPLIT, true, true, LATE_SYM, false, TICKETS, 1> : k_zfused_persist<C, LINES, SPLIT, false, true, LATE_SYM, false, TICKETS, 1>;
@@ -592,8 +609,10 @@
     const unsigned ntiles = (unsigned)((g.Lx / XB) * g.nouter);
     const int per_cu = (int)std::max<size_t>(1, std::min<size_t>(4, ((size_t)160 * 1024) / lds));
     const unsigned grid = std::min<unsigned>(ntiles, (unsigned)(cus * per_cu));
+    const int xgroup = TICKETS ? xmirror_group(g) : 0;
     hipLaunchKernelGGL(k, dim3(grid), dim3(C::T * LINES), lds, st, data, sym, tw, g.nouter,
-                       g.dTile, g.dOuter, g.dLine, g.sTile, g.sOuter, g.sLine, g.ytab, g.zm, g.nin, ntiles, TICKETS ? ticket_set(st) : (unsigned*)nullptr);
+                       g.dTile, g.dOuter, g.dLine, g.sTile, g.sOuter, g.sLine, g.ytab, g.zm, g.nin, ntiles, TICKETS ? ticket_set(st) : (unsigned*)nullptr,
+                       g.xtab, xgroup);
 }
 static unsigned* ticket_set(hipStream_t st) {
     static std::mutex mu;
@@ -630,8 +649,9 @@
         const int per_cu = (int)std::max<size_t>(1, std::min<size_t>(2, ((size_t)160 * 1024) / lds));
         const unsigned grid = std::min<unsigned>(2 * ntiles, (unsigned)(cu_count() * per_cu));
         unsigned* tickets = ticket_set(st);
+        const int xgroup = xmirror_group(g);
         hipLaunchKernelGGL(k, dim3(grid), dim3(C::T * LINES), lds, st, data, sym, twl, g.nouter,
-                           g.dTile, g.dOuter, g.dLine, g.sTile, g.sOuter, g.sLine, g.ytab, g.zm, g.nin, ntiles, tickets);
+                           g.dTile, g.dOuter, g.dLine, g.sTile, g.sOuter, g.sLine, g.ytab, g.zm, g.nin, ntiles, tickets, g.xtab, xgroup);
     } else {
         fail(LSFC_EINVAL, "half-tile persistent pass: lines of %d points run as whole tiles", (int)C::L);
     }
@@ -646,7 +666,7 @@
     const int64_t ntiles = (int64_t)(g.Lx / XB) * g.nouter;
     LSFC_REQUIRE(ntiles % 8 == 0, "half-tile z pass needs a multiple of 8 tiles");
     hipLaunchKernelGGL(k, dim3((unsigned)((XB / LINES) * ntiles)), dim3(C::T * LINES), lds, st, data, sym, tw, g.nouter,
-                       g.dTile, g.dOuter, g.dLine, g.sTile, g.sOuter, g.sLine, g.ytab, g.zm, g.nin, 1, (int64_t)0, 0);
+                       g.dTile, g.dOuter, g.dLine, g.sTile, g.sOuter, g.sLine, g.ytab, g.zm, g.nin, 1, (int64_t)0, 0, g.xtab);
 }
 
 #if LSFC_FAMILY == 2
diff --git a/fast_solver_lippmann_schwinger_amd/csrc/plan.hip b/fast_solver_lippmann_schwinger_amd/csrc/plan.hip
--- a/fast_solver_lippmann_schwinger_amd/csrc/plan.hip
+++ b/fast_solver_lippmann_schwinger_amd/csrc/plan.hip
@@ -239,9 +239,49 @@
         if (p->ndim == 3) {
             plan_setup_symbol_rows(p, quarter ? nullptr : G2.p, perm[1], perm[2], pyrow);
             LSFC_REQUIRE(!quarter || (p->sym_rows == p->pads[1] / 2 + 1 && p->sym_hz == p->pads[2] / 2 + 8), "internal: quarter symbol but full storage");
-            p->sym.alloc((size_t)p->pads[0] * p->sym_rows * p->sym_hz);
-            pw_permute_symbol(G2.p, p->sym.p, dperm[0].p, pyrow.p, dperm[2].p, p->pads, p->sym_rows, p->sym_hz, 0, p->pads[0] / 8, scale, p->stream,
-                              quarter ? p->pads[1] / 2 + 1 : 0);
+            const int ntx = p->pads[0] / 8, srcLy = quarter ? p->pads[1] / 2 + 1 : 0;
+            const size_t tile_elems = (size_t)8 * p->sym_rows * p->sym_hz;
+            std::vector<int> rep((size_t)ntx); std::vector<unsigned> lanes((size_t)ntx);
+            bool xeven = false;
+            p->xtab.release(); p->xtab_host.clear(); p->sym_tiles = ntx;
+            if (p->sym_rows == p->pads[1] / 2 + 1 && p->sym_hz == p->pads[2] / 2 + 8 && pruned_xmirror_table(p->pads[0], rep.data(), lanes.data()))
+                xeven = quarter || pw_mirror_deviation(G2.p, p->pads, 0, p->stream) < 1e-13;
+            if (xeven) {
+                std::vector<int> px((size_t)p->pads[0]);
+                for (int xb = 0; xb < ntx; ++xb)
+                    for (int xi = 0; xi < 8; ++xi) px[(size_t)(8 * xb + xi)] = perm[0][(size_t)(8 * rep[(size_t)xb] + (int)((lanes[(size_t)xb] >> (4 * xi)) & 7u))];
+                LSFC_HIP(hipMemcpy(dperm[0].p, px.data(), px.size() * sizeof(int), hipMemcpyHostToDevice));
+            }
+            if (xeven && env_switch("LSFC_SYMBOL_OCTANT") != '0') {
+                std::vector<int> stile((size_t)ntx, -1), mirror_of((size_t)ntx, -1);
+                int ns = 0;
+                for (int xb = 0; xb < ntx; ++xb) { if (rep[(size_t)xb] == xb) stile[(size_t)xb] = ns++; else mirror_of[(size_t)rep[(size_t)xb]] = xb; }
+                for (int xb = 0; xb < ntx; ++xb)
+                    if (rep[(size_t)xb] == xb && mirror_of[(size_t)xb] < 0) p->xtab_host.push_back(make_int4(xb, stile[(size_t)xb], (int)XMIRROR_IDENTITY, 0));
+                LSFC_REQUIRE(p->xtab_host.size() % 2 == 0, "internal: odd number of self-mirrored chunks");
+                for (int xb = 0; xb < ntx; ++xb) {
+                    const int m = mirror_of[(size_t)xb];
+                    if (m < 0) continue;
+                    p->xtab_host.push_back(make_int4(xb, stile[(size_t)xb], (int)XMIRROR_IDENTITY, 0));
+                    p->xtab_host.push_back(make_int4(m, stile[(size_t)xb], (int)lanes[(size_t)m], 0));
+                }
+                LSFC_REQUIRE((int)p->xtab_host.size() == ntx, "internal: x-mirror table has %d entries for %d tiles", (int)p->xtab_host.size(), ntx);
+                p->sym_tiles = ns;
+                p->xtab.alloc(p->xtab_host.size());
+                LSFC_HIP(hipMemcpy(p->xtab.p, p->xtab_host.data(), p->xtab_host.size() * sizeof(int4), hipMemcpyHostToDevice));
+                p->sym.alloc((size_t)ns * tile_elems);
+                for (int xb = 0; xb < ntx;) {
+                    if (stile[(size_t)xb] < 0) { ++xb; continue; }
+                    int e = xb + 1;
+                    while (e < ntx && stile[(size_t)e] >= 0) ++e;
+                    pw_permute_symbol(G2.p, p->sym.p + (size_t)stile[(size_t)xb] * tile_elems, dperm[0].p, pyrow.p, dperm[2].p, p->pads, p->sym_rows, p->sym_hz,
+                                      xb, e - xb, scale, p->stream, srcLy);
+                    xb = e;
+                }
+            } else {
+                p->sym.alloc((size_t)ntx * tile_elems);
+                pw_permute_symbol(G2.p, p->sym.p, dperm[0].p, pyrow.p, dperm[2].p, p->pads, p->sym_rows, p->sym_hz, 0, ntx, scale, p->stream, srcLy);
+            }
         } else {
             const int Ly = p->pads[1];
             std::vector<int> zm;
@@ -362,7 +402,7 @@
 void plan_zfused_3d(lsfc_plan* p, int Wc, int64_t a2_off, int64_t sym_off, int nrhs, hipStream_t st) {
     const int Ly = p->pads[1];
     const FusedGeom g{Wc, Ly, (int64_t)p->pitch2 * Ly, (int64_t)p->pitch2, 8, (int64_t)8 * p->sym_hz * p->sym_rows, (int64_t)8 * p->sym_hz, 8,
-                      p->ytab.p, p->zmirror.p, p->dims[2]};
+                      p->ytab.p, p->zmirror.p, p->dims[2], Wc == p->pads[0] ? p->xtab.p : nullptr};
     pruned_zfused(p->pads[2], p->tuning, p->A2.p + a2_off, p->sym.p + sym_off, p->tw[2].p, p->twl[2].p, g, st, nrhs, p->a2_elems);
 }
 static FusedGeom geom_2d_rows(const lsfc_plan* p) {
@@ -605,6 +645,18 @@
 
 const char* lsfc_last_error(void) { return g_last_error; }
 int lsfc_padded_length(int64_t n) { return (n >= 1 && n <= 1024) ? lsfc::pruned_best_length(n) : 0; }
+int lsfc_xmirror_table(int64_t L, int* perm, int* rep, unsigned* lanes) {
+    int ok = 0;
+    const int rc = guarded([&] {
+        LSFC_REQUIRE(lsfc::pruned_length_supported(L), "unsupported line length %lld", (long long)L);
+        if (perm) lsfc::pruned_perm((int)L, perm);
+        std::vector<int> r((size_t)L / 8 + 1); std::vector<unsigned> m((size_t)L / 8 + 1);
+        ok = lsfc::pruned_xmirror_table((int)L, r.data(), m.data()) ? 1 : 0;
+        if (ok && rep) std::copy(r.begin(), r.begin() + L / 8, rep);
+        if (ok && lanes) std::copy(m.begin(), m.begin() + L / 8, lanes);
+    });
+    return rc ? rc : ok;
+}
 
 const char* lsfc_version(void) { return "lsfc 0.1 (gfx950, rocFFT + hand-written pruned FFT passes)"; }
 
@@ -756,12 +808,38 @@
     return guarded([&] {
         LSFC_REQUIRE(plan && count, "NULL argument");
         LSFC_REQUIRE(!plan->multi, "not available on a multi-device plan");
+        if (!plan->xtab_host.empty()) {
+            const size_t tile = (size_t)8 * plan->sym_rows * plan->sym_hz;
+            *count = (int64_t)(plan->xtab_host.size() * tile);
+            if (out) {
+                LSFC_REQUIRE(capacity_complex >= *count, "buffer too small");
+                std::vector<cplx> stored(plan->sym.n);
+                LSFC_HIP(hipMemcpy(stored.data(), plan->sym.p, plan->sym.bytes(), hipMemcpyDeviceToHost));
+                cplx* o = reinterpret_cast<cplx*>(out);
+                for (const int4& e : plan->xtab_host) {
+                    const cplx* src = stored.data() + (size_t)e.y * tile;
+                    cplx* dst = o + (size_t)e.x * tile;
+                    for (size_t r = 0; r < tile / 8; ++r)
+                        for (int xi = 0; xi < 8; ++xi) dst[8 * r + xi] = src[8 * r + (((unsigned)e.z >> (4 * xi)) & 7u)];
+                }
+            }
+            return;
+        }
         *count = (int64_t)plan->sym.n;
         if (out) {
             LSFC_REQUIRE(capacity_complex >= (int64_t)plan->sym.n, "buffer too small");
             LSFC_HIP(hipMemcpy(out, plan->sym.p, plan->sym.bytes(), hipMemcpyDeviceToHost));
         }
     });
+}
+int64_t lsfc_plan_symbol_bytes(const lsfc_plan* plan) {
+    int64_t bytes = -1;
+    guarded([&] {
+        LSFC_REQUIRE(plan, "NULL argument");
+        LSFC_REQUIRE(!plan->multi, "not available on a multi-device plan");
+        bytes = (int64_t)plan->sym.bytes();
+    });
+    return bytes;
 }
 
 int lsfc_apply(lsfc_plan* plan, const double* x, double* y, int memspace) {
diff --git a/fast_solver_lippmann_schwinger_amd/csrc/plan.hpp b/fast_solver_lippmann_schwinger_amd/csrc/plan.hpp
--- a/fast_solver_lippmann_schwinger_amd/csrc/plan.hpp
+++ b/fast_solver_lippmann_schwinger_amd/csrc/plan.hpp
@@ -104,6 +104,9 @@
     lsfc::DevBuf<int2> ytab;
     int sym_hz = 0;
     lsfc::DevBuf<int> zmirror;
+    int sym_tiles = 0;
+    lsfc::DevBuf<int4> xtab;
+    std::vector<int4> xtab_host;
     int pitch1 = 0, pitch2 = 0;
     int64_t tile2d = 0;
     int64_t a1_elems = 0, a2_elems = 0;
diff --git a/fast_solver_lippmann_schwinger_amd/csrc/pruned.hip b/fast_solver_lippmann_schwinger_amd/csrc/pruned.hip
--- a/fast_solver_lippmann_schwinger_amd/csrc/pruned.hip
+++ b/fast_solver_lippmann_schwinger_amd/csrc/pruned.hip
@@ -3,6 +3,7 @@
 #include <cstdlib>
 #include <mutex>
 #include <set>
+#include <vector>
 
 namespace lsfc {
 
@@ -89,6 +90,35 @@
     case 5: pruned_perm_f5(L, freq_of_storage); break;
     default: fail(LSFC_EINVAL, "pruned pipeline: unsupported padded length %d", L); }
 }
+bool pruned_xmirror_table(int L, int* rep, unsigned* lanes) {
+    if (!family(L) || L % 16) return false;
+    std::vector<int> perm((size_t)L), inv((size_t)L);
+    pruned_perm(L, perm.data());
+    for (int s = 0; s < L; ++s) inv[(size_t)perm[(size_t)s]] = s;
+    unsigned pairmap = 0; bool have = false;
+    int kept = 0;
+    for (int xb = 0; xb < L / 8; ++xb) {
+        int chunk = -1; unsigned map = 0, seen = 0; bool whole = true;
+        for (int xi = 0; xi < 8; ++xi) {
+            const int sm = inv[(size_t)((L - perm[(size_t)(8 * xb + xi)]) % L)];
+            if (chunk < 0) chunk = sm / 8;
+            if (sm / 8 != chunk) whole = false;
+            map |= (unsigned)(sm % 8) << (4 * xi); seen |= 1u << (sm % 8);
+        }
+        if (!whole || seen != 0xFFu || chunk == xb) { rep[xb] = xb; lanes[xb] = XMIRROR_IDENTITY; ++kept; continue; }
+        if (!have) { pairmap = map; have = true; }
+        if (map != pairmap) return false;
+        if (chunk > xb) { rep[xb] = xb; lanes[xb] = XMIRROR_IDENTITY; }
+        else { rep[xb] = chunk; lanes[xb] = map; }
+    }
+    if (!have || kept % 2) return false;
+    if (have) {
+        unsigned lo = 0;
+        for (int xi = 0; xi < 4; ++xi) lo |= 1u << ((pairmap >> (4 * xi)) & 7u);
+        if (lo != 0x0Fu && lo != 0xF0u) return false;
+    }
+    return true;
+}
 int pruned_twfull_len(int L) {
     switch (family(L)) {
     case 2: return pruned_twfull_len_f2(L);
diff --git a/fast_solver_lippmann_schwinger_amd/csrc/pruned.hpp b/fast_solver_lippmann_schwinger_amd/csrc/pruned.hpp
--- a/fast_solver_lippmann_schwinger_amd/csrc/pruned.hpp
+++ b/fast_solver_lippmann_schwinger_amd/csrc/pruned.hpp
@@ -27,6 +27,8 @@
 void pruned_warmup(int device);
 int pruned_best_length(int64_t n);
 void pruned_perm(int L, int* freq_of_storage);
+static constexpr unsigned XMIRROR_IDENTITY = 0x76543210u;
+bool pruned_xmirror_table(int L, int* rep, unsigned* lanes);
 PrunedTuning pruned_default_tuning();
 
 void pruned_xfwd(int L, const PrunedTuning&, const VecBatch& vb, int nrhs, int64_t obatch, const double* nu, cplx* out, const cplx* tw, int64_t nlines, int W, int Wp, int n, hipStream_t,
@@ -47,6 +49,7 @@
     const int2* ytab;
     const int* zm;
     int nin;
+    const int4* xtab = nullptr;
 };
 void pruned_zfused(int L, const PrunedTuning&, cplx* data, const cplx* sym, const cplx* tw, const cplx* twl, const FusedGeom&, hipStream_t,
                    int nrhs = 1, int64_t dBatch = 0);
diff --git a/fast_solver_lippmann_schwinger_amd/operators.py b/fast_solver_lippmann_schwinger_amd/operators.py
--- a/fast_solver_lippmann_schwinger_amd/operators.py
+++ b/fast_solver_lippmann_schwinger_amd/operators.py
@@ -99,6 +99,12 @@
         out = np.empty(cnt.value, dtype=np.complex128)
         L.check(L.load().lsfc_plan_get_symbol(self._plan, out.ctypes.data_as(C.c_void_p), cnt.value, C.byref(cnt)))
         return out
+
+    def symbol_bytes(self):
+        n = L.load().lsfc_plan_symbol_bytes(self._plan)
+        if n < 0:
+            L.check(int(n))
+        return int(n)
 
     def set_tuning(self, **knobs):
         for key, value in knobs.items():
diff --git a/include/lsfc.h b/include/lsfc.h
--- a/include/lsfc.h
+++ b/include/lsfc.h
@@ -60,6 +60,7 @@
 const char* lsfc_plan_pipeline(const lsfc_plan* plan);
 int lsfc_plan_set_nu(lsfc_plan* plan, const double* nu, int memspace);
 int lsfc_plan_get_symbol(const lsfc_plan* plan, double* out, int64_t capacity_complex, int64_t* count);
+int64_t lsfc_plan_symbol_bytes(const lsfc_plan* plan);
 
 
 int lsfc_apply(lsfc_plan* plan, const double* x, double* y, int memspace);
@@ -195,6 +196,8 @@
 
 int lsfc_padded_length(int64_t n);
 
+int lsfc_xmirror_table(int64_t L, int* perm, int* rep, unsigned* lanes);
+
 const char* lsfc_last_error(void);
 const char* lsfc_version(void);
 
```

After: 80.81 applies/s. About the same (-0.3%).
